# Azure/mmlspark

Measured on NVIDIA H100. Metric: boosting_iters_per_sec, higher is better.
Workload: dtype int64 fixed-point histograms over u8 bins (fp32 gradients, fp64 split gains)

## Files before the change

### mmlspark_b200/csrc/engine.cu

```cuda
#include "engine.h"
#include "objective.h"
#include "renew_kernel.cuh"
#include "metric_kernels.cuh"

#include <nvtx3/nvToolsExt.h>

#include <arpa/inet.h>
#include <netdb.h>
#include <netinet/in.h>
#include <netinet/tcp.h>
#include <sys/select.h>
#include <sys/socket.h>
#include <unistd.h>
#include <sys/types.h>

#include <algorithm>
#include <chrono>
#include <functional>
#include <mutex>
#include <omp.h>
#include <cstring>
#include <numeric>
#include <thread>

// ... 365 lines not shown
  UploadMeta();
  rows_stride = static_cast<size_t>(num_data);
  bins.Alloc(static_cast<size_t>(num_tiles) * rows_stride * 32);
  if (nw > 0) bins16.Alloc(static_cast<size_t>(nw) * rows_stride);
}

template <typename T>
static void LaunchBin(const T* X, long long nrow, int ncol, int row_major, long long ld, const Dataset& d, long long row_offset, cudaStream_t s) {
  B200_CUDA(cudaFuncSetAttribute(k_bin_rows<T>, cudaFuncAttributeMaxDynamicSharedMemorySize, 65536));
  const int sms = DeviceSMs();
  dim3 grid(static_cast<unsigned>(std::min<long long>((nrow + 7) / 8, sms * 8)), d.num_tiles);
  if (grid.x == 0) grid.x = 1;
  k_bin_rows<T><<<grid, 256, 65536, s>>>(X, nrow, ncol, row_major, ld, d.meta.p, d.ub.p, d.catbin.p, d.nfn, d.bins.p, static_cast<long long>(d.rows_stride), row_offset);
  if (d.nw > 0)
    k_bin_wide<T><<<sms * 8, 256, 0, s>>>(X, nrow, row_major, ld, d.wide_meta.p, d.nw, d.wide_cats.p, d.wide_catbin.p, d.wide_ub.p, d.bins16.p, d.rows_stride, row_offset);
  B200_CUDA(cudaGetLastError());
}

void Dataset::BinBlock(const void* data, bool on_device, int data_type, int is_row_major, long long n, long long start_row) {
  NvtxRange nvtx("b200gbm:K0 bin rows (H2D + value->bin)");
  const int F = num_total_features;
  const size_t esz = data_type == 0 ? 4 : 8;
  if (start_row < 0 || start_row + n > num_data) Fatal("row block out of range");
  if (on_device) {
    const long long ld = is_row_major ? F : n;
    if (data_type == 0) LaunchBin<float>(static_cast<const float*>(data), n, F, is_row_major, ld, *this, start_row, stream);
    else LaunchBin<double>(static_cast<const double*>(data), n, F, is_row_major, ld, *this, start_row, stream);
    B200_CUDA(cudaStreamSynchronize(stream));
    return;
  }
  const size_t kStageBytes = 256u << 20;
  long long chunk = std::max<long long>(1, std::min<long long>(n, static_cast<long long>(kStageBytes) / (static_cast<long long>(F) * esz)));
  const size_t need = static_cast<size_t>(chunk) * F * esz;
  if (!ingest_copy_stream_) {
    B200_CUDA(cudaStreamCreateWithFlags(&ingest_copy_stream_, cudaStreamNonBlocking));
    for (int i = 0; i < 2; ++i) {
      B200_CUDA(cudaEventCreateWithFlags(&ingest_copied_[i], cudaEventDisableTiming));
      B200_CUDA(cudaEventCreateWithFlags(&ingest_binned_[i], cudaEventDisableTiming));
    }
  }
  for (int i = 0; i < 2; ++i) if (ingest_buf_[i].n < need) ingest_buf_[i].Alloc(std::max(need, std::min(kStageBytes, static_cast<size_t>(num_data) * F * esz)));
  cudaStream_t copy_stream = ingest_copy_stream_;
  int it = 0;
  for (long long r0 = 0; r0 < n; r0 += chunk, ++it) {
    const int b = it & 1;
    const long long rows = std::min(chunk, n - r0);
    if (it >= 2) B200_CUDA(cudaStreamWaitEvent(copy_stream, ingest_binned_[b], 0));
    if (is_row_major) {
      B200_CUDA(cudaMemcpyAsync(ingest_buf_[b].p, static_cast<const unsigned char*>(data) + static_cast<size_t>(r0) * F * esz, static_cast<size_t>(rows) * F * esz,
                                cudaMemcpyHostToDevice, copy_stream));
    } else {
      B200_CUDA(cudaMemcpy2DAsync(ingest_buf_[b].p, static_cast<size_t>(rows) * esz, static_cast<const unsigned char*>(data) + static_cast<size_t>(r0) * esz,
                                  static_cast<size_t>(n) * esz, static_cast<size_t>(rows) * esz, F, cudaMemcpyHostToDevice, copy_stream));
    }
    B200_CUDA(cudaEventRecord(ingest_copied_[b], copy_stream));
    B200_CUDA(cudaStreamWaitEvent(stream, ingest_copied_[b], 0));
    const long long ld = is_row_major ? F : rows;
    if (data_type == 0) LaunchBin<float>(reinterpret_cast<const float*>(ingest_buf_[b].p), rows, F, is_row_major, ld, *this, start_row + r0, stream);
    else LaunchBin<double>(reinterpret_cast<const double*>(ingest_buf_[b].p), rows, F, is_row_major, ld, *this, start_row + r0, stream);
    B200_CUDA(cudaEventRecord(ingest_binned_[b], stream));
  }
  B200_CUDA(cudaStreamSynchronize(stream));
  ingest_rows_done_ += n;
  if (ingest_rows_done_ >= num_data) ReleaseIngestStaging();
}

void Dataset::ReleaseIngestStaging() {
  for (int i = 0; i < 2; ++i) {
    ingest_buf_[i].Free();
    if (ingest_copied_[i]) { cudaEventDestroy(ingest_copied_[i]); ingest_copied_[i] = nullptr; }
    if (ingest_binned_[i]) { cudaEventDestroy(ingest_binned_[i]); ingest_binned_[i] = nullptr; }
  }
  if (ingest_copy_stream_) { cudaStreamDestroy(ingest_copy_stream_); ingest_copy_stream_ = nullptr; }
}

Dataset* Dataset::CreateFromSampledColumn(double** sample_data, int** sample_indices, int ncol, const int* num_per_col, int num_sample_row,
                                          int num_total_row, const char* params) {
  (void)sample_indices;
  EnsureDevice();
  if (num_total_row <= 0 || ncol <= 0) Fatal("Dataset should have at least one row and one column");
  std::unique_ptr<Dataset> d = NewShell(num_total_row, ncol, params);
  d->SetMappers(nullptr, [&](std::vector<std::vector<double>>* nz, int, int) {
    for (int f = 0; f < ncol; ++f) (*nz)[f].assign(sample_data[f], sample_data[f] + num_per_col[f]);
    return num_sample_row;
  });
  d->AllocBins();
  return d.release();
}

void Dataset::PushRows(const void* data, int data_type, int nrow, int ncol, int start_row) {
  EnsureDevice();
  if (ncol != num_total_features) Fatal("PushRows: wrong number of columns");
  if (data_type != 0 && data_type != 1) Fatal("PushRows: unknown data type");
  StreamTimer timer(stream);
  BinBlock(data, IsDevicePointer(data), data_type, 1, nrow, start_row);
  ingest_ms += timer.Ms();
}

template <typename T>
void Dataset::UnpackTiles(T* out) const {
  std::vector<uint8_t> h(bins.n);
  B200_CUDA(cudaMemcpy(h.data(), bins.p, bins.n, cudaMemcpyDeviceToHost));
  std::memset(out, 0, static_cast<size_t>(num_data) * num_total_features * sizeof(T));
  for (int u = 0; u < nfn; ++u) {
    const int f = used[u];
    const uint8_t* src = h.data() + (static_cast<size_t>(u >> 5) * rows_stride) * 32 + (u & 31);
    for (int i = 0; i < num_data; ++i) out[static_cast<size_t>(i) * num_total_features + f] = src[static_cast<size_t>(i) * 32];
  }
}
void Dataset::GetBinsRowMajor(uint8_t* out) const {
  if (nw > 0) Fatal("this dataset has features with more than 256 bins: use B200GBM_DatasetGetBins16");
  UnpackTiles(out);
}
void Dataset::GetBinsRowMajor16(uint16_t* out) const {
  UnpackTiles(out);
  if (nw > 0) {
    std::vector<uint16_t> hw(bins16.n);
    B200_CUDA(cudaMemcpy(hw.data(), bins16.p, bins16.n * sizeof(uint16_t), cudaMemcpyDeviceToHost));
    for (int w = 0; w < nw; ++w) {
      const int f = used[nfn + w];
      const uint16_t* src = hw.data() + static_cast<size_t>(w) * rows_stride;
      for (int i = 0; i < num_data; ++i) out[static_cast<size_t>(i) * num_total_features + f] = src[i];
    }
  }
}

__global__ void k_gather_bin_rows(BinView bv, int nf, const FeatMeta* __restrict__ meta, const int* __restrict__ rows, int nrows, int F,
                                  uint16_t* __restrict__ out) {
  for (long long e = blockIdx.x * static_cast<long long>(blockDim.x) + threadIdx.x; e < static_cast<long long>(nrows) * nf;
       e += static_cast<long long>(gridDim.x) * blockDim.x) {
    const int i = static_cast<int>(e / nf), u = static_cast<int>(e % nf);
    out[static_cast<size_t>(i) * F + meta[u].real_index] = static_cast<uint16_t>(bv.at(u, static_cast<size_t>(rows[i])));
  }
}
void Dataset::GetBinsOfRows(const int32_t* rows, int nrows, uint16_t* out) const {
  if (nrows <= 0) return;
  for (int i = 0; i < nrows; ++i) if (rows[i] < 0 || rows[i] >= num_data) Fatal("GetBinsOfRows: row index out of range");
  DevBuf<int> dr; dr.Alloc(nrows);
  DevBuf<uint16_t> dout; dout.Alloc(static_cast<size_t>(nrows) * num_total_features);
  dr.Upload(rows, nrows, stream);
  dout.Zero(stream);
  if (nf > 0) k_gather_bin_rows<<<DeviceSMs() * 4, 256, 0, stream>>>(View(), nf, meta.p, dr.p, nrows, num_total_features, dout.p);
  B200_CUDA(cudaGetLastError());
  dout.Download(out, dout.n, stream);
  B200_CUDA(cudaStreamSynchronize(stream));
}

void Dataset::Histogram(const float* grad, const float* hess, const int32_t* idx, int cnt, double* out) const {
  EnsureDevice();
  B200_CUDA(set_k4_smem_limit());
  const int n = num_data;
  DevBuf<float> g, h; g.Alloc(n); h.Alloc(n);
  g.Upload(grad, n, stream); h.Upload(hess, n, stream);
  DevBuf<int4> q; q.Alloc(n);
  DevBuf<TreeCtrl> ctrl; ctrl.Alloc(1); ctrl.Zero(stream);
  DevBuf<int> didx; didx.Alloc(std::max(cnt, 1));
  if (idx) didx.Upload(idx, cnt, stream);
  const size_t elems = static_cast<size_t>(num_tiles) * 32 * 512;
  DevBuf<long long> H; H.Alloc(elems); H.Zero(stream);
  DevBuf<double> D; D.Alloc(elems);
  int sms = 0;
  B200_CUDA(cudaDeviceGetAttribute(&sms, cudaDevAttrMultiProcessorCount, device));
  k_absmax<<<sms * 4, 256, 0, stream>>>(g.p, h.p, n, ctrl.p);
  k_set_scale<<<1, 1, 0, stream>>>(ctrl.p, 0, 1.0);
  k_quantize<<<sms * 4, 256, 0, stream>>>(g.p, h.p, n, q.p, ctrl.p, 0, nullptr, 0);
  HistWork w{0, cnt, idx ? 1 : 0, 0};
  B200_CUDA(cudaMemcpyAsync(&ctrl.p->hist_work, &w, sizeof(w), cudaMemcpyHostToDevice, stream));
  DevBuf<int4> qo; qo.Alloc(std::max(cnt, 1));
  k_gather_q<<<sms * 4, 256, 0, stream>>>(&ctrl.p->hist_work, didx.p, didx.p, q.p, qo.p);
  launch_k4(false, bins.p, rows_stride, num_tiles, q.p, qo.p, didx.p, didx.p, &ctrl.p->hist_work,
            reinterpret_cast<unsigned long long*>(H.p), sms, stream);
  k_hist_to_double<<<sms * 4, 256, 0, stream>>>(H.p, D.p, elems, ctrl.p);
  B200_CUDA(cudaGetLastError());
  std::vector<double> hd(elems);
  D.Download(hd.data(), elems, stream);
  B200_CUDA(cudaStreamSynchronize(stream));
  std::memset(out, 0, sizeof(double) * static_cast<size_t>(num_total_features) * 512);
  for (int u = 0; u < nfn; ++u) std::memcpy(out + static_cast<size_t>(used[u]) * 512, hd.data() + static_cast<size_t>(u) * 512, sizeof(double) * 512);
}

Dataset* Dataset::CreateFromMat(const void* data, int data_type, int nrow, int ncol, int is_row_major, const char* params,
                                const Dataset* reference) {
  EnsureDevice();
  if (data_type != 0 && data_type != 1) Fatal("Unknown data type in CreateFromMat (expect C_API_DTYPE_FLOAT32 or FLOAT64)");
  if (nrow <= 0 || ncol <= 0) Fatal("Dataset should have at least one row and one column");
  std::unique_ptr<Dataset> d = NewShell(nrow, ncol, params);
  StreamTimer timer(d->stream);
  const bool on_device = IsDevicePointer(data);
  d->SetMappers(reference, [&](std::vector<std::vector<double>>* nz, int f0, int f1) {
    const int n = nrow, F = ncol;
    const std::vector<int> rows = d->SampleRows();
    const int sample_cnt = static_cast<int>(rows.size());
    std::vector<double> S(static_cast<size_t>(sample_cnt) * F);
    if (on_device) {
      DevBuf<int> d_rows; d_rows.Alloc(sample_cnt);
      DevBuf<double> d_S; d_S.Alloc(S.size());
      d_rows.Upload(rows.data(), sample_cnt, d->stream);
      int grid = static_cast<int>(std::min<size_t>((S.size() + 255) / 256, static_cast<size_t>(DeviceSMs()) * 32));
      if (data_type == 0) k_gather_rows<float><<<grid, 256, 0, d->stream>>>(static_cast<const float*>(data), n, F, is_row_major, d_rows.p, sample_cnt, d_S.p);
      else k_gather_rows<double><<<grid, 256, 0, d->stream>>>(static_cast<const double*>(data), n, F, is_row_major, d_rows.p, sample_cnt, d_S.p);
      B200_CUDA(cudaGetLastError());
      d_S.Download(S.data(), S.size(), d->stream);
      B200_CUDA(cudaStreamSynchronize(d->stream));
    } else {
#pragma omp parallel for schedule(static)
      for (int s = 0; s < sample_cnt; ++s) {
        const long long r = rows[s];
        for (int f = 0; f < F; ++f) {
          double v;
          if (data_type == 0) v = is_row_major ? static_cast<const float*>(data)[r * F + f] : static_cast<const float*>(data)[static_cast<long long>(f) * n + r];
          else v = is_row_major ? static_cast<const double*>(data)[r * F + f] : static_cast<const double*>(data)[static_cast<long long>(f) * n + r];
          S[static_cast<size_t>(s) * F + f] = v;
        }
      }
    }
#pragma omp parallel for schedule(dynamic)
    for (int f = f0; f < f1; ++f) {
      (*nz)[f].reserve(sample_cnt);
      for (int s = 0; s < sample_cnt; ++s) {
        double v = S[static_cast<size_t>(s) * F + f];
        if (std::fabs(v) > kZeroThr || std::isnan(v)) (*nz)[f].push_back(v);
      }
    }
    return sample_cnt;
  });
  d->AllocBins();
  d->BinBlock(data, on_device, data_type, is_row_major, nrow, 0);
  d->ingest_ms = timer.Ms();
  return d.release();
}

__global__ void k_fill_default_wide(const WideMeta* __restrict__ wm, int nw, uint16_t* __restrict__ bins16, size_t rows_stride, long long nrow) {
  for (long long e = blockIdx.x * static_cast<long long>(blockDim.x) + threadIdx.x; e < nrow * nw; e += static_cast<long long>(gridDim.x) * blockDim.x) {
    const int w = static_cast<int>(e / nrow);
    bins16[static_cast<size_t>(w) * rows_stride + (e - static_cast<long long>(w) * nrow)] = static_cast<uint16_t>(wm[w].default_bin);
  }
}
__global__ void k_fill_default_bins(const FeatMeta* __restrict__ meta, int nf, uint8_t* __restrict__ bins, size_t rows_stride, long long nrow, int num_tiles) {
  const long long total = nrow * num_tiles * 32;
  for (long long e = blockIdx.x * static_cast<long long>(blockDim.x) + threadIdx.x; e < total; e += static_cast<long long>(gridDim.x) * blockDim.x) {
    const int lane = static_cast<int>(e & 31);
    const long long rt = e >> 5;
    const int tile = static_cast<int>(rt / nrow);
    const long long r = rt - static_cast<long long>(tile) * nrow;
    const int u = tile * 32 + lane;
    bins[(static_cast<size_t>(tile) * rows_stride + r) * 32 + lane] = u < nf ? static_cast<uint8_t>(meta[u].default_bin) : 0;
  }
}
template <typename TI, typename TV>
__global__ void k_bin_csr(const TI* __restrict__ indptr, const int* __restrict__ indices, const TV* __restrict__ vals, long long nrow, const int* __restrict__ inner_of,
                          const FeatMeta* __restrict__ meta, const double* __restrict__ ub, const uint8_t* __restrict__ catbin, uint8_t* __restrict__ bins,
                          size_t rows_stride, long long elem_base, int nfn, const WideMeta* __restrict__ wm, const int* __restrict__ wcats,
                          const unsigned short* __restrict__ wcatbin, const double* __restrict__ wub, uint16_t* __restrict__ bins16) {
  const int lane = threadIdx.x & 31;
  const long long warp = (blockIdx.x * static_cast<long long>(blockDim.x) + threadIdx.x) >> 5, nwarps = (static_cast<long long>(gridDim.x) * blockDim.x) >> 5;
  for (long long r = warp; r < nrow; r += nwarps) {
    const long long a = static_cast<long long>(indptr[r]) - elem_base, b = static_cast<long long>(indptr[r + 1]) - elem_base;
    for (long long k = a + lane; k < b; k += 32) {
      const int u = inner_of[indices[k]];
      if (u < 0) continue;
      const FeatMeta m = meta[u];
      double v = static_cast<double>(vals[k]);
      if (u >= nfn) {
        bins16[static_cast<size_t>(u - nfn) * rows_stride + r] = static_cast<uint16_t>(d_wide_bin(v, wm[u - nfn], wcats, wcatbin, wub));
        continue;
      }
      const double* myub = ub + static_cast<size_t>(u) * 256;
      unsigned bin = 0;
      if (m.is_categorical) {
        if (!isnan(v)) {
          const int iv = static_cast<int>(v);
          if (iv >= 0) {
            int lo = 0, hi = m.num_sorted_cats;
            while (lo < hi) { int mid = (lo + hi) >> 1; if (static_cast<int>(myub[mid]) < iv) lo = mid + 1; else hi = mid; }
            if (lo < m.num_sorted_cats && static_cast<int>(myub[lo]) == iv) bin = catbin[static_cast<size_t>(u) * 256 + lo];
          }
        }
      } else {
        if (isnan(v)) { if (m.missing_type == 2) bin = m.num_bin - 1; else v = 0.0; }
        if (!isnan(v)) {
          int lo = 0, hi = m.num_bin - 1 - (m.missing_type == 2 ? 1 : 0);
          while (lo < hi) { int mid = (hi + lo - 1) / 2; if (v <= myub[mid]) hi = mid; else lo = mid + 1; }
          bin = lo;
        }
      }
      bins[(static_cast<size_t>(u >> 5) * rows_stride + r) * 32 + (u & 31)] = static_cast<uint8_t>(bin);
    }
  }
}

Dataset* Dataset::CreateFromCSR(const void* indptr, int indptr_type, const int32_t* indices, const void* data, int data_type,
                                int64_t nindptr, int64_t nelem, int64_t num_col, const char* params, const Dataset* reference) {
  EnsureDevice();
  if (num_col <= 0) Fatal("CreateFromCSR: num_col must be given");
  if (num_col > std::numeric_limits<int>::max()) Fatal("CreateFromCSR: too many columns");
  if (indptr_type != 2 && indptr_type != 3) Fatal("CreateFromCSR: indptr must be int32 or int64");
  if (data_type != 0 && data_type != 1) Fatal("Unknown data type in CreateFromCSR (expect C_API_DTYPE_FLOAT32 or FLOAT64)");
  const int64_t nrow = nindptr - 1;
  if (nrow <= 0) Fatal("Dataset should have at least one row and one column");
  if (nrow > std::numeric_limits<int>::max()) Fatal("CreateFromCSR: too many rows for one partition");
  auto ip = [&](int64_t r) -> int64_t { return indptr_type == 2 ? static_cast<const int32_t*>(indptr)[r] : static_cast<const int64_t*>(indptr)[r]; };
  auto val = [&](int64_t k) -> double { return data_type == 0 ? static_cast<double>(static_cast<const float*>(data)[k]) : static_cast<const double*>(data)[k]; };
  if (ip(0) < 0 || ip(nrow) > nelem) Fatal("CreateFromCSR: indptr does not match the number of elements");
  {
    int bad = 0;
#pragma omp parallel for schedule(static) reduction(| : bad)
    for (int64_t r = 0; r < nrow; ++r) {
      if (ip(r) > ip(r + 1)) bad |= 1;
      else for (int64_t k = ip(r); k < ip(r + 1); ++k) if (indices[k] < 0 || indices[k] >= num_col) bad |= 2;
    }
    if (bad & 1) Fatal("CreateFromCSR: indptr is not non-decreasing");
    if (bad & 2) Fatal("CreateFromCSR: a column index is negative or >= num_col");
  }
  std::unique_ptr<Dataset> d = NewShell(static_cast<int>(nrow), static_cast<int>(num_col), params);
  StreamTimer timer(d->stream);
  const int F = d->num_total_features;
  d->SetMappers(reference, [&](std::vector<std::vector<double>>* nz, int, int) {
    const std::vector<int> rows = d->SampleRows();
    for (int r : rows)
      for (int64_t k = ip(r); k < ip(r + 1); ++k) {
        const double v = val(k);
        if (std::fabs(v) > kZeroThr || std::isnan(v)) (*nz)[indices[k]].push_back(v);
      }
// ... 63 lines not shown
  } else if (s == "weight" || s == "weights") {
    if (n == 0 || data == nullptr) { weight.clear(); d_weight.Free(); return; }
    if (n != num_data) Fatal("Length of weights is not same with #data");
    to_f32(&weight);
    d_weight.Alloc(n); d_weight.Upload(weight.data(), n, stream);
  } else if (s == "init_score") {
    if (n == 0 || data == nullptr) { init_score.clear(); return; }
    if (n % num_data != 0) Fatal("Initial score size doesn't match data size");
    init_score.resize(n);
    if (type == 1) std::memcpy(init_score.data(), data, sizeof(double) * n);
    else if (type == 0) for (int i = 0; i < n; ++i) init_score[i] = static_cast<const float*>(data)[i];
    else Fatal("Input type error for init_score (expect float64)");
  } else if (s == "group" || s == "query") {
    if (type != 2) Fatal("Input type error for group (expect int32)");
    const int32_t* g = static_cast<const int32_t*>(data);
    group_sizes.assign(g, g + n);
    query_boundaries.assign(1, 0);
    for (int i = 0; i < n; ++i) query_boundaries.push_back(query_boundaries.back() + g[i]);
    if (query_boundaries.back() != num_data) Fatal("Sum of query counts is not same with #data");
    d_qb.Alloc(query_boundaries.size()); d_qb.Upload(query_boundaries.data(), query_boundaries.size(), stream);
  } else {
    Fatal("Unknown field name: " + s);
  }
  B200_CUDA(cudaStreamSynchronize(stream));
}

void Dataset::GetField(const char* name, int* out_len, const void** out_ptr, int* out_type) const {
  std::string s(name);
  if (s == "label" || s == "target") { *out_len = static_cast<int>(label.size()); *out_ptr = label.data(); *out_type = 0; }
  else if (s == "weight" || s == "weights") { *out_len = static_cast<int>(weight.size()); *out_ptr = weight.empty() ? nullptr : weight.data(); *out_type = 0; }
  else if (s == "init_score") { *out_len = static_cast<int>(init_score.size()); *out_ptr = init_score.empty() ? nullptr : init_score.data(); *out_type = 1; }
  else if (s == "group" || s == "query") { *out_len = static_cast<int>(query_boundaries.size()); *out_ptr = query_boundaries.empty() ? nullptr : query_boundaries.data(); *out_type = 2; }
  else Fatal("Unknown field name: " + s);
}

void Dataset::SetFeatureNames(const char** names, int n) {
  if (n != num_total_features) Fatal("Size of feature_names error, should equal with total number of features");
  feature_names.assign(n, "");
  for (int i = 0; i < n; ++i) {
    feature_names[i] = names[i];
    for (auto& c : feature_names[i]) if (c == ' ') c = '_';
  }
}

static size_t Align16(size_t x) { return (x + 15) & ~static_cast<size_t>(15); }
constexpr int kScanSmem = (768 + 64) * 8;

Booster::Booster(const std::string& model_text) {
  std::unique_ptr<HostModel> m = HostModel::FromString(model_text);
  model = std::move(*m);
  K = model.num_tree_per_iteration;
  num_init_iteration = model.NumIterations();
}

Booster::Booster(const Dataset* tr, const char* params) : train(tr) {
  EnsureDevice();
  device_ = CurrentDevice();
  cfg.Parse(params);
  if (cfg.boosting != "gbdt" && cfg.boosting != "rf" && cfg.boosting != "goss" && cfg.boosting != "dart")
    Fatal("Unknown boosting type " + cfg.boosting);
  is_rf_ = cfg.boosting == "rf"; is_goss_ = cfg.boosting == "goss"; is_dart_ = cfg.boosting == "dart";
  drop_rand_ = LcgRandom(cfg.drop_seed);
  obj_.reset(new Objective(cfg, *train));
  balanced_bagging_ = cfg.bagging_freq > 0 && (cfg.pos_bagging_fraction < 1.0 || cfg.neg_bagging_fraction < 1.0) && obj_->kind() == ObjectiveKind::kBinary;
  bagging_ = cfg.bagging_freq > 0 && (cfg.bagging_fraction < 1.0 || balanced_bagging_);
  if (bagging_ && !(cfg.bagging_fraction > 0.0)) Fatal("bagging_fraction should be in (0, 1]");
  if (is_goss_) {
    if (!(cfg.top_rate + cfg.other_rate <= 1.0)) Fatal("Check failed: (config_->top_rate + config_->other_rate) <= (1.0f)");
    if (!(cfg.top_rate > 0.0 && cfg.other_rate > 0.0)) Fatal("Check failed: config_->top_rate > 0.0f && config_->other_rate > 0.0f");
    if (bagging_) Fatal("Cannot use bagging in GOSS");
  }
  if (is_rf_) {
    const bool ff = cfg.feature_fraction < 1.0 && cfg.feature_fraction > 0.0;
    if (!(bagging_ || ff)) Fatal("Check failed: (config->bagging_freq > 0 && config->bagging_fraction < 1.0f && config->bagging_fraction > 0.0f) || (config->feature_fraction < 1.0f && config->feature_fraction > 0.0f)");
  }
  if (cfg.num_leaves < 2) Fatal("num_leaves should be >= 2");
  ValidateMetrics();
  if (train->label.empty()) Fatal("label should not be empty for training");
  K = obj_->NumTreePerIteration();
  parallel_ = Net().active && Net().world > 1;
  cfg.num_machines = parallel_ ? Net().world : 1;
  if (balanced_bagging_) {
    double npos = static_cast<double>(std::count_if(train->label.begin(), train->label.end(), [](float v) { return v > 0; }));
    if (parallel_) {
      cudaStream_t ts;
      B200_CUDA(cudaStreamCreateWithFlags(&ts, cudaStreamNonBlocking));
      AllReduceHost(&npos, 1, ncclSum, ts);
      B200_CUDA(cudaStreamDestroy(ts));
    }
    if (!(npos > 0)) { balanced_bagging_ = false; bagging_ = cfg.bagging_freq > 0 && cfg.bagging_fraction < 1.0; }
  }
  shrinkage_ = is_rf_ ? 1.0 : cfg.learning_rate;
  model.average_output = is_rf_;
  model.num_class = K;
  model.num_tree_per_iteration = K;
  model.label_index = 0;
  model.max_feature_idx = train->num_total_features - 1;
  model.feature_names = train->feature_names;
  for (int f = 0; f < train->num_total_features; ++f) model.feature_infos.push_back(train->mappers[f].InfoString());
  InitTraining();
  model.objective_str = obj_->ToString();
}

Booster::~Booster() {
  if (split_op_trees_ > 0) {
    double tot = 0; for (auto& kv : split_op_ms_) tot += kv.second;
    fprintf(stderr, "[b200gbm split timing] %d trees, %.3f ms per tree in split operations:", split_op_trees_, tot / split_op_trees_);
    for (auto& kv : split_op_ms_) fprintf(stderr, " %s=%.1fus", kv.first.c_str(), 1000.0 * kv.second / split_op_trees_ / std::max(cfg.num_leaves - 1, 1));
    fprintf(stderr, " (per split)\n");
  }
  for (auto* v : valids_) delete v;
  for (void* p : ipc_opened_) cudaIpcCloseMemHandle(p);
  if (tree_host_) cudaFreeHost(tree_host_);
  if (ctrl_host_) cudaFreeHost(ctrl_host_);
  if (leaves_host_) cudaFreeHost(leaves_host_);
  if (ev_a_) cudaEventDestroy(ev_a_);
  if (ev_b_) cudaEventDestroy(ev_b_);
  if (stream_) cudaStreamDestroy(stream_);
}

void Booster::InitTraining() {
  const int n = train->num_data;
  const int L = cfg.num_leaves;
  cudaDeviceProp prop;
  B200_CUDA(cudaGetDeviceProperties(&prop, device_));
  num_sms_ = prop.multiProcessorCount;
  B200_CUDA(cudaStreamCreateWithFlags(&stream_, cudaStreamNonBlocking));
  B200_CUDA(cudaEventCreate(&ev_a_)); B200_CUDA(cudaEventCreate(&ev_b_));
  cudaDeviceSetLimit(cudaLimitMaxL2FetchGranularity, 32);
  cudaGetLastError();
  B200_CUDA(set_k4_smem_limit());
  B200_CUDA(cudaFuncSetAttribute(k_scan, cudaFuncAttributeMaxDynamicSharedMemorySize, kScanSmem));

  sp_.l1 = cfg.lambda_l1; sp_.l2 = cfg.lambda_l2; sp_.max_delta_step = cfg.max_delta_step;
  sp_.min_gain_to_split = cfg.min_gain_to_split; sp_.min_sum_hessian = cfg.min_sum_hessian_in_leaf;
  sp_.min_data_in_leaf = cfg.min_data_in_leaf; sp_.max_depth = cfg.max_depth; sp_.num_leaves = L; sp_.parallel = parallel_ ? 1 : 0;
  sp_.nf = train->nf; sp_.nf_pad = train->nf_pad; sp_.num_tiles = train->num_tiles; sp_.nfn = train->nfn;
  {
    auto gd = [&](const char* k, double d) { auto it = cfg.raw.find(k); return (it != cfg.raw.end() && !it->second.empty()) ? std::atof(it->second.c_str()) : d; };
    sp_.cat_l2 = gd("cat_l2", 10.0); sp_.cat_smooth = gd("cat_smooth", 10.0);
    sp_.max_cat_threshold = static_cast<int>(gd("max_cat_threshold", 32)); sp_.max_cat_to_onehot = static_cast<int>(gd("max_cat_to_onehot", 4));
    sp_.min_data_per_group = static_cast<int>(gd("min_data_per_group", 100)); sp_.pad3 = 0;
    if (train->nw > 0) {
      if (sp_.max_cat_threshold > kCatListMax) Fatal("max_cat_threshold > " + std::to_string(kCatListMax) + " is not supported together with categorical features of more than 256 bins");
      if (sp_.max_cat_to_onehot > 256) Fatal("max_cat_to_onehot > 256 is not supported together with categorical features of more than 256 bins");
      B200_CUDA(cudaFuncSetAttribute(k4_hist_wide<4>, cudaFuncAttributeMaxDynamicSharedMemorySize, 4 * kWideHistSeg * 4));
      B200_CUDA(cudaFuncSetAttribute(k4_hist_wide<3>, cudaFuncAttributeMaxDynamicSharedMemorySize, 4 * kWideHistSeg * 4));
      B200_CUDA(cudaFuncSetAttribute(k_scan_wide, cudaFuncAttributeMaxDynamicSharedMemorySize, kWideMaxBins * 8));
    }
  }

  score_.Alloc(static_cast<size_t>(K) * n); score_.Zero(stream_);
  grad_.Alloc(static_cast<size_t>(K) * n); hess_.Alloc(static_cast<size_t>(K) * n);
  qgh_.Alloc(n); qord_.Alloc(n); idx0_.Alloc(n); idx1_.Alloc(n);
  slot_elems_ = train->hist_pairs * 2;
  H_.Alloc(slot_elems_); H_.Zero(stream_); pool_.Alloc(slot_elems_ * L);
  {
    int per_sm = 0;
    B200_CUDA(cudaOccupancyMaxActiveBlocksPerMultiprocessor(&per_sm, k_partition, 256, 0));
    int coop = 0;
    cudaDeviceGetAttribute(&coop, cudaDevAttrCooperativeLaunch, device_);
    if (!coop || per_sm < 1) Fatal("this device cannot launch the cooperative partition kernel");
    part_max_blocks_ = per_sm * num_sms_;
  }
  flags_.Alloc(static_cast<size_t>(L) * train->nf_pad);
  cands_.Alloc(2 * static_cast<size_t>(train->nf_pad));
  leaves_.Alloc(L); ctrl_.Alloc(1); ctrl_.Zero(stream_);
  const int chunks = n / kPartChunk + 2;
  part_bits_.Alloc(static_cast<size_t>(chunks) * (kPartChunk / 32)); part_chunks_.Alloc(static_cast<size_t>(chunks) + chunks / kPartLocalScan + 8); part_chunks_.Zero(stream_);
  {
    size_t off = 0;
    auto take = [&](size_t bytes) { size_t o = off; off += Align16(bytes); return o; };
    size_t o_lc = take(4 * (L - 1)), o_rc = take(4 * (L - 1)), o_sf = take(4 * (L - 1)), o_tb = take(4 * (L - 1)), o_dt = take(4 * (L - 1));
    size_t o_sg = take(4 * (L - 1)), o_lv = take(8 * L), o_lw = take(8 * L), o_lcn = take(4 * L), o_iv = take(8 * (L - 1)), o_iw = take(8 * (L - 1));
    size_t o_ic = take(4 * (L - 1)), o_lp = take(4 * L), o_ld = take(4 * L), o_nl = take(16), o_cb = take(32 * (L - 1));
    size_t o_cl = take(2 * kCatListMax * (L - 1)), o_cn = take(4 * (L - 1));
    tree_blob_bytes_ = off;
    tree_blob_.Alloc(off);
    unsigned char* b = tree_blob_.p;
    tree_dev_.left_child = reinterpret_cast<int*>(b + o_lc); tree_dev_.right_child = reinterpret_cast<int*>(b + o_rc);
    tree_dev_.split_feature_inner = reinterpret_cast<int*>(b + o_sf); tree_dev_.threshold_bin = reinterpret_cast<int*>(b + o_tb);
    tree_dev_.decision_type = reinterpret_cast<int*>(b + o_dt); tree_dev_.split_gain = reinterpret_cast<float*>(b + o_sg);
    tree_dev_.leaf_value = reinterpret_cast<double*>(b + o_lv); tree_dev_.leaf_weight = reinterpret_cast<double*>(b + o_lw);
    tree_dev_.leaf_count = reinterpret_cast<int*>(b + o_lcn); tree_dev_.internal_value = reinterpret_cast<double*>(b + o_iv);
    tree_dev_.internal_weight = reinterpret_cast<double*>(b + o_iw); tree_dev_.internal_count = reinterpret_cast<int*>(b + o_ic);
    tree_dev_.leaf_parent = reinterpret_cast<int*>(b + o_lp); tree_dev_.leaf_depth = reinterpret_cast<int*>(b + o_ld);
    tree_dev_.num_leaves = reinterpret_cast<int*>(b + o_nl);
    tree_dev_.cat_bits = reinterpret_cast<unsigned*>(b + o_cb);
    tree_dev_.cat_list = reinterpret_cast<unsigned short*>(b + o_cl);
    tree_dev_.cat_list_len = reinterpret_cast<int*>(b + o_cn);
    B200_CUDA(cudaMemsetAsync(b, 0, off, stream_));
    B200_CUDA(cudaMallocHost(reinterpret_cast<void**>(&tree_host_), off));
    B200_CUDA(cudaMallocHost(reinterpret_cast<void**>(&ctrl_host_), sizeof(TreeCtrl)));
    B200_CUDA(cudaMallocHost(reinterpret_cast<void**>(&leaves_host_), sizeof(LeafState) * L));
  }
  if (!train->init_score.empty()) {
    if (train->init_score.size() != static_cast<size_t>(K) * n) Fatal("Initial score size doesn't match data size");
    has_init_score_ = true;
    score_.Upload(train->init_score.data(), train->init_score.size(), stream_);
  }
  obj_->Init(stream_);
  const_hessian_ = obj_->ConstHessian() && !is_goss_;
  if (obj_->RenewsLeaves()) {
    rn_keys_a_.Alloc(n); rn_keys_b_.Alloc(n); rn_pos_a_.Alloc(n); rn_pos_b_.Alloc(n); rn_leaf_of_pos_.Alloc(n); rn_leaf_a_.Alloc(n); rn_leaf_b_.Alloc(n);
    rn_res_.Alloc(n); rn_row_.Alloc(n); rn_seg_.Alloc(L + 1); rn_out_.Alloc(2 * static_cast<size_t>(L));
    if (obj_->RenewWeights()) rn_cdf_.Alloc(n);
    size_t t1 = 0, t2 = 0;
    cub::DeviceRadixSort::SortPairs(nullptr, t1, rn_keys_a_.p, rn_keys_b_.p, rn_pos_a_.p, rn_pos_b_.p, n, 0, 64, stream_);
    cub::DeviceRadixSort::SortPairs(nullptr, t2, rn_leaf_a_.p, rn_leaf_b_.p, rn_pos_b_.p, rn_pos_a_.p, n, 0, 32, stream_);
    rn_tmp_bytes_ = std::max(t1, t2);
    rn_tmp_.Alloc(rn_tmp_bytes_ + 16);
  }
  if (parallel_) SetupPeerReduce();
  col_rand_ = LcgRandom(cfg.feature_fraction_seed);
  feature_used_host_.assign(train->nf_pad, 0);
  for (int u = 0; u < train->nf; ++u) feature_used_host_[u] = 1;
  feature_used_.Alloc(train->nf_pad);
  feature_used_.Upload(feature_used_host_.data(), train->nf_pad, stream_);
  ResetFeaturesByTree();
  if (bagging_ || is_goss_) {
    bag_blocks_ = (n + kBagBlock - 1) / kBagBlock;
    std::vector<unsigned> st(bag_blocks_);
    for (int i = 0; i < bag_blocks_; ++i) st[i] = static_cast<unsigned>(cfg.bagging_seed + i);
    bag_lcg_.Alloc(bag_blocks_); bag_lcg_.Upload(st.data(), st.size(), stream_);
    std::unique_ptr<LcgJump> jt(new LcgJump());
    unsigned a = 1, c = 0;
    for (int j = 0; j < kBagBlock; ++j) { a = a * 214013u; c = c * 214013u + 2531011u; jt->mul[j] = a; jt->add[j] = c; }
    bag_jump_.Alloc(1); bag_jump_.Upload(jt.get(), 1, stream_);
    in_bag_.Alloc(n); bag_block_cnt_.Alloc(bag_blocks_); bag_idx_.Alloc(n); bag_total_.Alloc(1);
    need_re_bagging_ = bagging_;
    B200_CUDA(cudaStreamSynchronize(stream_));
  }
  if (is_rf_) {
    if (!train->init_score.empty()) Fatal("Check failed: train_data->metadata().init_score() == nullptr");
    rf_init_scores_.assign(K, 0.0);
    DevBuf<double> tmp;
    tmp.Alloc(static_cast<size_t>(K) * n); tmp.Zero(stream_);
    for (int k = 0; k < K; ++k) {
      double init = (cfg.boost_from_average && !has_init_score_) ? obj_->BoostFromScore(k) : 0.0;
      if (!(std::fabs(init) > kEps)) init = 0.0;
      rf_init_scores_[k] = init;
      if (init != 0.0) k_add_const<<<num_sms_ * 4, 256, 0, stream_>>>(tmp.p + static_cast<size_t>(k) * n, n, init);
    }
    ComputeGradientsAt(tmp.p);
    B200_CUDA(cudaStreamSynchronize(stream_));
  }
  B200_CUDA(cudaStreamSynchronize(stream_));
}

TreeDev Booster::RebasedTree(unsigned char* base) const {
  TreeDev t = tree_dev_;
  auto mv = [&](auto*& p) { p = reinterpret_cast<std::remove_reference_t<decltype(p)>>(base + (reinterpret_cast<unsigned char*>(p) - tree_blob_.p)); };
  mv(t.left_child); mv(t.right_child); mv(t.split_feature_inner); mv(t.threshold_bin); mv(t.decision_type); mv(t.split_gain);
  mv(t.leaf_value); mv(t.leaf_weight); mv(t.leaf_count); mv(t.internal_value); mv(t.internal_weight); mv(t.internal_count);
  mv(t.leaf_parent); mv(t.leaf_depth); mv(t.num_leaves); mv(t.cat_bits); mv(t.cat_list); mv(t.cat_list_len);
  return t;
}
void Booster::AddStoredTree(int iter_index, int k, bool to_train, bool to_valid) {
  const size_t ti = static_cast<size_t>(num_init_iteration + iter_index) * K + k;
  const HostTree& ht = *model.trees[ti];
  cudaStream_t s = stream_;
  const int n = train->num_data;
  if (ht.num_leaves <= 1) {
    const double v = ht.leaf_value[0];
    if (v != 0.0) {
      if (to_train) k_add_const<<<num_sms_ * 4, 256, 0, s>>>(score_.p + static_cast<size_t>(k) * n, n, v);
      if (to_valid) for (auto* vs : valids_) k_add_const<<<num_sms_ * 4, 256, 0, s>>>(vs->score.p + static_cast<size_t>(k) * vs->ds->num_data, vs->ds->num_data, v);
    }
    return;
  }
  DevBuf<unsigned char>& blob = *tree_store_.at(static_cast<size_t>(iter_index) * K + k);
  TreeDev td = RebasedTree(blob.p);
  B200_CUDA(cudaMemcpyAsync(td.leaf_value, ht.leaf_value.data(), sizeof(double) * ht.num_leaves, cudaMemcpyHostToDevice, s));
  const int egrid = num_sms_ * 8;
  if (to_train) k_add_tree_binned<<<egrid, 256, 0, s>>>(td, train->meta.p, train->View(), n, score_.p + static_cast<size_t>(k) * n, 1.0);
  if (to_valid)
    for (auto* vs : valids_)
      k_add_tree_binned<<<egrid, 256, 0, s>>>(td, vs->ds->meta.p, vs->ds->View(), vs->ds->num_data,
                                              vs->score.p + static_cast<size_t>(k) * vs->ds->num_data, 1.0);
  B200_CUDA(cudaGetLastError());
  B200_CUDA(cudaStreamSynchronize(s));
  timing.launches += (to_train ? 1 : 0) + (to_valid ? static_cast<long long>(valids_.size()) : 0);
}
void Booster::DroppingTrees() {
  drop_index_.clear();
  const bool is_skip = drop_rand_.NextFloat() < cfg.skip_drop;
  if (!is_skip) {
    double drop_rate = cfg.drop_rate;
    if (!cfg.uniform_drop) {
      const double inv_average_weight = static_cast<double>(tree_weight_.size()) / sum_weight_;
      if (cfg.max_drop > 0) drop_rate = std::min(drop_rate, cfg.max_drop * inv_average_weight / sum_weight_);
      for (int i = 0; i < iter; ++i)
        if (drop_rand_.NextFloat() < drop_rate * tree_weight_[i] * inv_average_weight) {
          drop_index_.push_back(i);
          if (drop_index_.size() >= static_cast<size_t>(cfg.max_drop)) break;
        }
    } else {
      if (cfg.max_drop > 0) drop_rate = std::min(drop_rate, cfg.max_drop / static_cast<double>(iter));
      for (int i = 0; i < iter; ++i)
        if (drop_rand_.NextFloat() < drop_rate) {
          drop_index_.push_back(i);
          if (drop_index_.size() >= static_cast<size_t>(cfg.max_drop)) break;
        }
    }
  }
  for (int i : drop_index_)
    for (int k = 0; k < K; ++k) {
// ... 77 lines not shown
  {
    DevBuf<unsigned char> ds, dr; ds.Alloc(sizeof(PeerInfo)); dr.Alloc(sizeof(PeerInfo) * R);
    B200_CUDA(cudaMemcpyAsync(ds.p, &mine, sizeof(PeerInfo), cudaMemcpyHostToDevice, stream_));
    B200_NCCL(ncclAllGather(ds.p, dr.p, sizeof(PeerInfo), ncclChar, Net().comm, stream_));
    B200_CUDA(cudaMemcpyAsync(all.data(), dr.p, sizeof(PeerInfo) * R, cudaMemcpyDeviceToHost, stream_));
    B200_CUDA(cudaStreamSynchronize(stream_));
  }
  int ok = 1;
  for (int r = 0; r < R; ++r) ok &= all[r].ok;
  PeerTables pt{};
  if (ok) {
    for (int r = 0; r < R && ok; ++r) {
      void* p3[3];
      if (r == me) { for (int i = 0; i < 3; ++i) p3[i] = bufs[i]; }
      else if (all[r].pid == mine.pid) {
        int can = 0;
        cudaDeviceCanAccessPeer(&can, device_, all[r].device);
        if (!can) { ok = 0; break; }
        cudaError_t e = cudaDeviceEnablePeerAccess(all[r].device, 0);
        if (e != cudaSuccess && e != cudaErrorPeerAccessAlreadyEnabled) { cudaGetLastError(); ok = 0; break; }
        cudaGetLastError();
        for (int i = 0; i < 3; ++i) p3[i] = reinterpret_cast<void*>(all[r].ptr[i]);
      } else {
        for (int i = 0; i < 3; ++i) {
          if (cudaIpcOpenMemHandle(&p3[i], all[r].ipc[i], cudaIpcMemLazyEnablePeerAccess) != cudaSuccess) { cudaGetLastError(); ok = 0; break; }
          ipc_opened_.push_back(p3[i]);
        }
        if (!ok) break;
      }
      pt.H[r] = static_cast<const long long*>(p3[0]); pt.mail[r] = static_cast<SplitCand*>(p3[1]); pt.flags[r] = static_cast<unsigned*>(p3[2]);
    }
  }
  double okd = ok ? 1.0 : 0.0;
  AllReduceHost(&okd, 1, ncclMin, stream_);
  const bool peers_ok = okd > 0.5;
  fused_ = peers_ok && mode == 1;
  p2p_allreduce_ = peers_ok && mode == 2;
  if (p2p_allreduce_) { pt.rank = me; pt.world = R; pt.feat0 = 0; pt.feat1 = 0; pt.error = peer_error_.p; peers_ = pt; return; }
  if (!fused_) return;
  const int tiles_per_rank = (train->num_tiles + R - 1) / R;
  pt.rank = me; pt.world = R;
  pt.feat0 = std::min(train->nf_pad, me * tiles_per_rank * 32);
  pt.feat1 = std::min(train->nf_pad, (me + 1) * tiles_per_rank * 32);
  pt.error = peer_error_.p;
  peers_ = pt;
}

void Booster::ResetFeaturesByTree() {
  if (cfg.feature_fraction >= 1.0) return;
  const int total = train->nf;
  int cnt = std::max(static_cast<int>(total * cfg.feature_fraction + 0.5), std::min(2, total));
  std::fill(feature_used_host_.begin(), feature_used_host_.end(), 0);
  for (int i : col_rand_.Sample(total, cnt)) feature_used_host_[train->sample_order[i]] = 1;
  feature_used_.Upload(feature_used_host_.data(), train->nf_pad, stream_);
}

double Booster::BoostFromAverage(int k) {
  if (model.trees.empty() && !has_init_score_ && cfg.boost_from_average) {
    double init = obj_->BoostFromScore(k);
    if (std::fabs(init) > kEps) {
      const int n = train->num_data;
      k_add_const<<<num_sms_ * 4, 256, 0, stream_>>>(score_.p + static_cast<size_t>(k) * n, n, init);
      for (auto* v : valids_) k_add_const<<<num_sms_ * 4, 256, 0, stream_>>>(v->score.p + static_cast<size_t>(k) * v->ds->num_data, v->ds->num_data, init);
      B200_CUDA(cudaGetLastError());
      return init;
    }
  }
  return 0.0;
}

void Booster::ComputeGradientsAt(const double* score_p) {
  NvtxRange nvtx("b200gbm:K1/K2 gradients");
  obj_->LaunchGradients(score_p, grad_.p, hess_.p, num_sms_);
  B200_CUDA(cudaGetLastError());
  timing.launches += 1;
}

void Booster::RenewTreeOutput(int k, double rf_pred) {
  const int n = train->num_data;
  const int total = use_bag_ ? bag_count_ : n;
  const int L = cfg.num_leaves;
  cudaStream_t s = stream_;
  TreeCtrl* ctrl = ctrl_.p;
  const int egrid = num_sms_ * 8;
  const float* wptr = obj_->RenewWeights();
  k_renew_gather<<<egrid, 256, 0, s>>>(ctrl, leaves_.p, idx0_.p, idx1_.p, train->d_label.p, is_rf_ ? nullptr : score_.p + static_cast<size_t>(k) * n, rf_pred,
                                       rn_keys_a_.p, rn_pos_a_.p, rn_res_.p, rn_leaf_of_pos_.p, rn_row_.p);
  size_t tb = rn_tmp_bytes_;
  B200_CUDA(cub::DeviceRadixSort::SortPairs(rn_tmp_.p, tb, rn_keys_a_.p, rn_keys_b_.p, rn_pos_a_.p, rn_pos_b_.p, total, 0, 64, s));
  k_renew_leaf_keys<<<egrid, 256, 0, s>>>(rn_pos_b_.p, rn_leaf_of_pos_.p, total, rn_leaf_a_.p);
  int leaf_bits = 1;
  while ((1 << leaf_bits) < L) ++leaf_bits;
  tb = rn_tmp_bytes_;
  B200_CUDA(cub::DeviceRadixSort::SortPairs(rn_tmp_.p, tb, rn_leaf_a_.p, rn_leaf_b_.p, rn_pos_b_.p, rn_pos_a_.p, total, 0, leaf_bits, s));
  k_renew_offsets<<<1, 32, 0, s>>>(ctrl, leaves_.p, rn_seg_.p);
  double* out = rn_out_.p;
  double* has = rn_out_.p + L;
  const int lgrid = (L + 127) / 128;
  if (!wptr) {
    k_renew_unweighted<<<lgrid, 128, 0, s>>>(ctrl, rn_seg_.p, rn_pos_a_.p, rn_res_.p, obj_->RenewAlpha(), out, has);
  } else {
    k_renew_cdf<<<L, 1024, 0, s>>>(ctrl, rn_seg_.p, rn_pos_a_.p, rn_row_.p, wptr, rn_cdf_.p);
    k_renew_weighted<<<lgrid, 128, 0, s>>>(ctrl, rn_seg_.p, rn_pos_a_.p, rn_res_.p, rn_cdf_.p, obj_->RenewAlpha(), out, has);
  }
  if (parallel_) B200_NCCL(ncclAllReduce(out, out, 2 * static_cast<size_t>(L), ncclDouble, ncclSum, Net().comm, s));
  k_renew_apply<<<lgrid, 128, 0, s>>>(ctrl, tree_dev_, out, has, parallel_ ? 1 : 0);
  B200_CUDA(cudaGetLastError());
  timing.launches += wptr ? 7 : 6;
}

void Booster::EnsureColumnCopy() {
  if (cols_tried_) return;
  cols_tried_ = true;
  const Dataset& d = *train;
  const char* env = std::getenv("B200GBM_COLUMN_COPY");
  if ((env && std::atoi(env) == 0) || d.nfn == 0 || d.num_data == 0) return;
  const size_t stride = (static_cast<size_t>(d.num_data) + 255) & ~static_cast<size_t>(255);
  const size_t need = static_cast<size_t>(d.num_tiles) * 32 * stride;
  size_t free_b = 0, total_b = 0;
  if (cudaMemGetInfo(&free_b, &total_b) != cudaSuccess) { cudaGetLastError(); return; }
  const size_t reserve = std::max<size_t>(static_cast<size_t>(8) << 30, total_b / 10);
  if (free_b < need + reserve) return;
  uint8_t* p = nullptr;
  if (cudaMalloc(reinterpret_cast<void**>(&p), need) != cudaSuccess) { cudaGetLastError(); return; }
  bins_cols_.p = p; bins_cols_.n = need;
  cols_stride_ = stride;
  const long long work = ((static_cast<long long>(d.num_data) + 255) / 256) * d.num_tiles;
  k_tiles_to_columns<<<static_cast<unsigned>(std::min<long long>(work, static_cast<long long>(num_sms_) * 16)), 256, 0, stream_>>>(
      d.bins.p, d.rows_stride, d.num_tiles, d.num_data, bins_cols_.p, stride);
  B200_CUDA(cudaGetLastError());
}

void Booster::GetMemoryInfo(int64_t* out2) {
  EnsureDevice();
  size_t free_b = 0, total_b = 0;
  if (cudaMemGetInfo(&free_b, &total_b) != cudaSuccess) { cudaGetLastError(); free_b = 0; }
  out2[0] = static_cast<int64_t>(bins_cols_.n);
  out2[1] = static_cast<int64_t>(free_b);
}

void Booster::LaunchPartition(int grid, int last) {
  const Dataset& d = *train;
  TreeCtrl* ctrl = ctrl_.p;
  LeafState* leaves = leaves_.p;
  TreeDev tree = tree_dev_;
  uint8_t* flags = flags_.p;
  const FeatMeta* meta = d.meta.p;
  SplitParams sp = sp_;
  const uint8_t* bins = d.bins.p;
  size_t rows_stride = d.rows_stride;
  int* i0 = idx0_.p; int* i1 = idx1_.p;
  unsigned* bits = part_bits_.p;
  int* chunks = part_chunks_.p;
  const int4* qgh = qgh_.p;
  int4* qord = qord_.p;
  long long* H = H_.p;
  size_t h_elems = slot_elems_;
  const uint16_t* bins16 = d.bins16.p;
  static const int tickets = [] { const char* e = std::getenv("B200GBM_PART_TICKETS"); return e ? std::atoi(e) : 8; }();
  int tickets_per_block = tickets;
  const uint8_t* cols = bins_cols_.p;
  size_t cols_stride = cols_stride_;
  int* super_tot = part_chunks_.p + (train->num_data / kPartChunk + 2);
  void* args[] = {&ctrl, &leaves, &tree, &flags, &meta, &sp, &last, &bins, &rows_stride, &i0, &i1, &bits, &chunks, &qgh, &qord, &H, &h_elems, &bins16, &tickets_per_block,
                  &cols, &cols_stride, &super_tot};
  B200_CUDA(cudaLaunchCooperativeKernel(reinterpret_cast<void*>(k_partition), dim3(grid), dim3(256), args, 0, stream_));
}

void Booster::TrainOneTree(int k, HostTree* out) {
  NvtxRange nvtx_tree("b200gbm:tree");
  EnsureColumnCopy();
  const Dataset& d = *train;
  const int n = d.num_data;
  const int L = cfg.num_leaves;
  const float* g = grad_.p + static_cast<size_t>(k) * n;
  const float* h = hess_.p + static_cast<size_t>(k) * n;
  TreeCtrl* ctrl = ctrl_.p;
  cudaStream_t s = stream_;
  const int egrid = num_sms_ * 8;
  nvtxRangePushA("b200gbm:K3 quantize + C1 root sums");
  B200_CUDA(cudaMemsetAsync(&ctrl->absmax_bits[0], 0, 8, s));
  k_absmax<<<egrid, 256, 0, s>>>(g, h, n, ctrl);
  if (parallel_) B200_NCCL(ncclAllReduce(&ctrl->absmax_bits[0], &ctrl->absmax_bits[0], 2, ncclUint32, ncclMax, Net().comm, s));
  k_set_scale<<<1, 1, 0, s>>>(ctrl, const_hessian_ ? 1 : 0, 1.0);
  k_quantize<<<egrid, 256, 0, s>>>(g, h, n, qgh_.p, ctrl, const_hessian_ ? 1 : 0, use_bag_ ? in_bag_.p : nullptr, bag_count_);
  if (parallel_) B200_NCCL(ncclAllReduce(&ctrl->root_q[0], &ctrl->root_q[0], 3, ncclInt64, ncclSum, Net().comm, s));
  ResetFeaturesByTree();
  if (use_bag_)
    B200_CUDA(cudaMemcpyAsync(idx0_.p, bag_idx_.p, static_cast<size_t>(bag_count_) * sizeof(int), cudaMemcpyDeviceToDevice, s));
  k_tree_init<<<1, 256, 0, s>>>(ctrl, leaves_.p, tree_dev_, flags_.p, sp_, use_bag_ ? bag_count_ : n, feature_used_.p, use_bag_ ? 1 : 0);
  nvtxRangePop();
  timing.launches += 4;
  const int pgrid = std::max(1, std::min(n / kPartChunk + 1, part_max_blocks_));
  const dim3 sgrid(std::max(1, d.nfn), 2);
  std::vector<cudaEvent_t> evs;
  static const bool split_timing = getenv("B200GBM_SPLIT_TIMING") != nullptr;
  std::vector<cudaEvent_t> sev;
  auto mark = [&]() { if (split_timing) { cudaEvent_t e; cudaEventCreate(&e); cudaEventRecord(e, s); sev.push_back(e); } };
  k_round_ctl<<<1, 256, 0, s>>>(ctrl, leaves_.p, tree_dev_, flags_.p, d.meta.p, sp_, 0);
  timing.launches += 1;
  for (int split = 0; split < L - 1; ++split) {
    mark();
    if (profile_hist) { cudaEvent_t a, b; B200_CUDA(cudaEventCreate(&a)); B200_CUDA(cudaEventCreate(&b)); evs.push_back(a); evs.push_back(b); B200_CUDA(cudaEventRecord(a, s)); }
    if (split == 0 && use_bag_) k_gather_q<<<egrid, 256, 0, s>>>(&ctrl->hist_work, idx0_.p, idx1_.p, qgh_.p, qord_.p);
    mark();
    nvtxRangePushA("b200gbm:K4 histogram");
    launch_k4(const_hessian_, d.bins.p, d.rows_stride, d.num_tiles, qgh_.p, qord_.p, idx0_.p, idx1_.p, &ctrl->hist_work,
              reinterpret_cast<unsigned long long*>(H_.p), num_sms_, s);
    if (d.nw > 0) {
      int max_nb = 0;
      for (const WideMeta& wm : d.wide_host) max_nb = std::max(max_nb, wm.num_bin);
      const int segs = (max_nb + kWideHistSeg - 1) / kWideHistSeg;
      int units = 0;
      for (const WideMeta& wm : d.wide_host) units += (wm.num_bin + kWideHistSeg - 1) / kWideHistSeg;
      const dim3 wgrid(static_cast<unsigned>(std::max(1, std::min(64, 4 * num_sms_ / std::max(1, units)))), static_cast<unsigned>(d.nw), static_cast<unsigned>(segs));
      if (const_hessian_)
        k4_hist_wide<3><<<wgrid, kWideThreads, 4 * kWideHistSeg * 4, s>>>(d.bins16.p, d.rows_stride, d.wide_meta.p, qgh_.p, qord_.p, idx0_.p, idx1_.p, &ctrl->hist_work,
                                                                         reinterpret_cast<unsigned long long*>(H_.p));
      else
        k4_hist_wide<4><<<wgrid, kWideThreads, 4 * kWideHistSeg * 4, s>>>(d.bins16.p, d.rows_stride, d.wide_meta.p, qgh_.p, qord_.p, idx0_.p, idx1_.p, &ctrl->hist_work,
                                                                         reinterpret_cast<unsigned long long*>(H_.p));
      timing.launches += 1;
    }
    nvtxRangePop();
    if (profile_hist) B200_CUDA(cudaEventRecord(evs.back(), s));
    mark();
    nvtxRangePushA(parallel_ ? "b200gbm:C2 histogram reduce + K5 scan + pick" : "b200gbm:K5 scan + pick");
    if (fused_) {
      ++epoch_;
      const dim3 dgrid(std::max(1, (peers_.feat1 - peers_.feat0 + 7) / 8), 2);
      k_scan_dp<<<dgrid, 256, 0, s>>>(ctrl, leaves_.p, d.meta.p, peers_, pool_.p, slot_elems_, flags_.p, cands_.p, sp_, epoch_);
      k_pick_dp<<<1, 256, 0, s>>>(ctrl, leaves_.p, d.meta.p, cands_.p, sp_, peers_, epoch_);
      mark();
    } else {
      if (p2p_allreduce_) {
        ++epoch_;
        const int agrid = static_cast<int>(std::max<size_t>(1, std::min<size_t>(64, slot_elems_ / 2 / Net().world / 256 + 1)));
        k_allreduce_p2p<<<agrid, 256, 0, s>>>(ctrl, peers_, slot_elems_, epoch_, peer_flags_.p + 48);
        timing.launches += 1;
      } else if (parallel_) {
        B200_NCCL(ncclAllReduce(H_.p, H_.p, slot_elems_, ncclInt64, ncclSum, Net().comm, s));
      }
      mark();
      if (d.nw > 0) {
        k_scan_wide<<<dim3(d.nw, 2), 256, kWideMaxBins * 8, s>>>(ctrl, leaves_.p, d.wide_meta.p, H_.p, pool_.p, slot_elems_, flags_.p, cands_.p, sp_);
        timing.launches += 1;
      }
      k_scan<<<sgrid, 256, d.has_categorical ? kScanSmem : 0, s>>>(ctrl, leaves_.p, d.meta.p, H_.p, pool_.p, slot_elems_, flags_.p, cands_.p, sp_);
    }
    nvtxRangePop();
    mark();
    nvtxRangePushA("b200gbm:K7 partition + controller");
    LaunchPartition(pgrid, split == L - 2 ? 1 : 0);
    nvtxRangePop();
    mark();
    timing.launches += fused_ ? 4 : 3; timing.hist_launches += 1;
  }
  if (obj_->RenewsLeaves()) RenewTreeOutput(k, is_rf_ ? rf_init_scores_[k] : 0.0);
  const double bias = is_rf_ ? rf_init_scores_[k] : 0.0, pre = is_rf_ ? static_cast<double>(iter + num_init_iteration) : 1.0;
  const double post = is_rf_ ? 1.0 / (iter + num_init_iteration + 1) : 1.0;
  if (use_bag_ || is_rf_)
    k_add_tree_binned<<<egrid, 256, 0, s>>>(tree_dev_, d.meta.p, d.View(), n, score_.p + static_cast<size_t>(k) * n, shrinkage_, bias, pre, post);
  else
    k_add_score<<<egrid, 256, 0, s>>>(ctrl, leaves_.p, tree_dev_, idx0_.p, idx1_.p, score_.p + static_cast<size_t>(k) * n, shrinkage_);
  for (auto* v : valids_)
    k_add_tree_binned<<<egrid, 256, 0, s>>>(tree_dev_, v->ds->meta.p, v->ds->View(), v->ds->num_data,
                                            v->score.p + static_cast<size_t>(k) * v->ds->num_data, shrinkage_, bias, pre, post);
  timing.launches += 2 + static_cast<long long>(valids_.size());
  B200_CUDA(cudaGetLastError());
  B200_CUDA(cudaMemcpyAsync(tree_host_, tree_blob_.p, tree_blob_bytes_, cudaMemcpyDeviceToHost, s));
  B200_CUDA(cudaMemcpyAsync(ctrl_host_, ctrl, sizeof(TreeCtrl), cudaMemcpyDeviceToHost, s));
  B200_CUDA(cudaStreamSynchronize(s));
  if (split_timing && !fused_ && !sev.empty()) {
    static const char* kOps[] = {"gather_q(bagged root)", "K4", "allreduce", "scan+pick", "partition+zeroH+ctl"};
    const int per = 6;
    for (size_t b0 = 0; b0 + per <= sev.size(); b0 += per)
      for (int o = 0; o < per - 1; ++o) { float ms = 0; cudaEventElapsedTime(&ms, sev[b0 + o], sev[b0 + o + 1]); split_op_ms_[kOps[o]] += ms; }
    split_op_trees_ += 1;
    for (auto e : sev) cudaEventDestroy(e);
  }
  if (profile_hist) {
    for (size_t i = 0; i + 1 < evs.size(); i += 2) { float ms = 0; cudaEventElapsedTime(&ms, evs[i], evs[i + 1]); timing.hist_ms += ms; }
    for (auto e : evs) cudaEventDestroy(e);
  }
  timing.hist_rows += ctrl_host_->trace_rows;
  if (fused_ || p2p_allreduce_) {
    int err = 0;
    B200_CUDA(cudaMemcpy(&err, peer_error_.p, sizeof(int), cudaMemcpyDeviceToHost));
    if (err) Fatal("data-parallel training: a peer rank stopped responding (peer-memory barrier timed out)");
  }
  const unsigned char* hb = tree_host_;
  auto at = [&](const void* devp) { return hb + (static_cast<const unsigned char*>(devp) - tree_blob_.p); };
  const int nl = *reinterpret_cast<const int*>(at(tree_dev_.num_leaves));
  out->Resize(nl);
  if (nl > 1) {
    const int* lc = reinterpret_cast<const int*>(at(tree_dev_.left_child));
    const int* rc = reinterpret_cast<const int*>(at(tree_dev_.right_child));
    const int* sf = reinterpret_cast<const int*>(at(tree_dev_.split_feature_inner));
    const int* tb = reinterpret_cast<const int*>(at(tree_dev_.threshold_bin));
    const int* dt = reinterpret_cast<const int*>(at(tree_dev_.decision_type));
    const float* sg = reinterpret_cast<const float*>(at(tree_dev_.split_gain));
    const double* lv = reinterpret_cast<const double*>(at(tree_dev_.leaf_value));
    const double* lw = reinterpret_cast<const double*>(at(tree_dev_.leaf_weight));
    const int* lcn = reinterpret_cast<const int*>(at(tree_dev_.leaf_count));
    const double* iv = reinterpret_cast<const double*>(at(tree_dev_.internal_value));
    const double* iw = reinterpret_cast<const double*>(at(tree_dev_.internal_weight));
    const int* ic = reinterpret_cast<const int*>(at(tree_dev_.internal_count));
    const int* ld = reinterpret_cast<const int*>(at(tree_dev_.leaf_depth));
    const unsigned* cb = reinterpret_cast<const unsigned*>(at(tree_dev_.cat_bits));
    const unsigned short* cl = reinterpret_cast<const unsigned short*>(at(tree_dev_.cat_list));
    const int* cln = reinterpret_cast<const int*>(at(tree_dev_.cat_list_len));
    for (int i = 0; i < nl - 1; ++i) {
      out->left_child[i] = lc[i]; out->right_child[i] = rc[i]; out->split_feature_inner[i] = sf[i];
      out->split_feature[i] = d.used[sf[i]]; out->threshold_in_bin[i] = static_cast<uint32_t>(tb[i]);
      out->decision_type[i] = static_cast<int8_t>(dt[i]); out->split_gain[i] = sg[i];
      const FeatureBins& fbm = d.mappers[d.used[sf[i]]];
      if (dt[i] & 1) {
        std::vector<int> cats;
        if (sf[i] >= d.nfn) { for (int k = 0; k < cln[i]; ++k) cats.push_back(fbm.bin_to_cat[cl[i * kCatListMax + k]]); }
        else for (int b = 0; b < fbm.num_bin; ++b) if ((cb[i * 8 + (b >> 5)] >> (b & 31)) & 1u) cats.push_back(fbm.bin_to_cat[b]);
        out->AddCategoricalNode(i, cats);
      } else {
        double thr = fbm.upper[tb[i]];
        if (std::isnan(thr)) thr = 0.0; else if (thr >= 1e300) thr = 1e300; else if (thr <= -1e300) thr = -1e300;
        out->threshold[i] = thr;
      }
      out->internal_value[i] = iv[i]; out->internal_weight[i] = iw[i]; out->internal_count[i] = ic[i];
    }
    for (int i = 0; i < nl; ++i) { out->leaf_value[i] = lv[i]; out->leaf_weight[i] = lw[i]; out->leaf_count[i] = lcn[i]; out->leaf_depth[i] = ld[i]; }
  } else {
    out->leaf_value[0] = 0.0;
  }
}

bool Booster::TrainTrees(const float* custom_g, const float* custom_h) {
  NvtxRange nvtx("b200gbm:iteration (LGBM_BoosterUpdateOneIter)");
  if (!train) Fatal("this booster was loaded from a model string and cannot be trained");
  EnsureDevice();
  cudaStream_t s = stream_;
  const int n = train->num_data;
  B200_CUDA(cudaEventRecord(ev_a_, s));
  std::vector<double> init_scores(K, 0.0);
  bool saved_const = const_hessian_;
  if (is_rf_) {
    if (custom_g) Fatal("RF mode do not support custom objective function, please use built-in objectives.");
    init_scores = rf_init_scores_;
  } else if (!custom_g) {
    for (int k = 0; k < K; ++k) init_scores[k] = BoostFromAverage(k);
    if (is_dart_ && !dart_dropped_this_iter_) DroppingTrees();
    ComputeGradientsAt(score_.p);
  } else {
    grad_.Upload(custom_g, static_cast<size_t>(K) * n, s);
    hess_.Upload(custom_h, static_cast<size_t>(K) * n, s);
    const_hessian_ = false;
  }
  Bagging(iter);
  bool should_continue = is_rf_;
  for (int k = 0; k < K; ++k) {
    std::unique_ptr<HostTree> t(new HostTree());
    t->Resize(1);
    t->leaf_value[0] = 0;
    if (obj_->NeedTrain(k) && train->nf > 0) TrainOneTree(k, t.get());
    if (t->num_leaves > 1) {
      should_continue = true;
      t->Shrink(shrinkage_);
      if (std::fabs(init_scores[k]) > kEps) t->AddBias(init_scores[k]);
    } else if (static_cast<int>(model.trees.size()) < K) {
      double output = obj_->NeedTrain(k) ? init_scores[k] : obj_->BoostFromScore(k);
      t->MakeConstant(output);
      const double pre = is_rf_ ? static_cast<double>(iter + num_init_iteration) : 1.0, post = is_rf_ ? 1.0 / (iter + num_init_iteration + 1) : 1.0;
      k_scale_add<<<num_sms_ * 4, 256, 0, s>>>(score_.p + static_cast<size_t>(k) * n, n, pre, output, post);
      for (auto* v : valids_) k_scale_add<<<num_sms_ * 4, 256, 0, s>>>(v->score.p + static_cast<size_t>(k) * v->ds->num_data, v->ds->num_data, pre, output, post);
    } else {
// ... 407 lines not shown
```

### mmlspark_b200/csrc/engine.h

```cpp
#pragma once
#include <cuda_runtime.h>
#include <nccl.h>

#include <cstdint>
#include <memory>
#include <stdexcept>
#include <map>
#include <string>
#include <vector>

#include "bin_mapper.h"
#include "config.h"
#include "kernels.cuh"
#include "model.h"

namespace b200gbm {

#define B200_CUDA(x)                                                                                      \
  do {                                                                                                    \
    cudaError_t e__ = (x);                                                                                \
    if (e__ != cudaSuccess)                                                                               \
      throw std::runtime_error(std::string("CUDA error: ") + cudaGetErrorString(e__) + " at " + __FILE__ + ":" + std::to_string(__LINE__)); \
  } while (0)
#define B200_NCCL(x)                                                                                      \
// ... 44 lines not shown
  static Dataset* CreateFromMat(const void* data, int data_type, int nrow, int ncol, int is_row_major, const char* params,
                                const Dataset* reference);
  static Dataset* CreateFromCSR(const void* indptr, int indptr_type, const int32_t* indices, const void* data, int data_type,
                                int64_t nindptr, int64_t nelem, int64_t num_col, const char* params, const Dataset* reference);
  static Dataset* CreateFromSampledColumn(double** sample_data, int** sample_indices, int ncol, const int* num_per_col,
                                          int num_sample_row, int num_total_row, const char* params);
  void PushRows(const void* data, int data_type, int nrow, int ncol, int start_row);
  void GetBinsRowMajor(uint8_t* out) const;
  void GetBinsRowMajor16(uint16_t* out) const;
  void GetBinsOfRows(const int32_t* rows, int nrows, uint16_t* out) const;
  void Histogram(const float* grad, const float* hess, const int32_t* idx, int cnt, double* out) const;
  void SetField(const char* name, const void* data, int n, int type);
  void GetField(const char* name, int* out_len, const void** out_ptr, int* out_type) const;
  void SetFeatureNames(const char** names, int n);

  int device = 0;
  int num_data = 0, num_total_features = 0;
  Config cfg;
  std::vector<FeatureBins> mappers;
  std::vector<int> used;
  std::vector<int> inner_of;
  std::vector<FeatMeta> meta_host;
  int nf = 0, nf_pad = 0, num_tiles = 0;
  int nfn = 0, nw = 0;
  size_t hist_pairs = 0;
  std::vector<int> sample_order;
  size_t rows_stride = 0;
  DevBuf<uint8_t> bins;
  DevBuf<uint16_t> bins16;
  std::vector<WideMeta> wide_host;
  DevBuf<WideMeta> wide_meta;
  DevBuf<int> wide_cats;
  DevBuf<unsigned short> wide_catbin;
  DevBuf<double> wide_ub;
  BinView View() const { return BinView{bins.p, rows_stride, bins16.p, nfn}; }
  DevBuf<FeatMeta> meta;
  DevBuf<double> ub;
  DevBuf<uint8_t> catbin;
  bool has_categorical = false;
  std::vector<float> label, weight;
  std::vector<double> init_score;
  std::vector<int32_t> query_boundaries, group_sizes;
  DevBuf<float> d_label, d_weight;
  DevBuf<int> d_qb;
  std::vector<std::string> feature_names;
  cudaStream_t stream = nullptr;
  double ingest_ms = 0.0;

 private:
  static std::unique_ptr<Dataset> NewShell(int nrow, int ncol, const char* params);
  template <typename Sample> void SetMappers(const Dataset* reference, Sample sample);
  std::vector<int> SampleRows() const;
  void AllocBins();
  template <typename T> void UnpackTiles(T* out) const;
  void BinBlock(const void* data, bool on_device, int data_type, int is_row_major, long long nrow, long long start_row);
  DevBuf<unsigned char> ingest_buf_[2];
  cudaStream_t ingest_copy_stream_ = nullptr;
  cudaEvent_t ingest_copied_[2] = {nullptr, nullptr}, ingest_binned_[2] = {nullptr, nullptr};
  long long ingest_rows_done_ = 0;
  void ReleaseIngestStaging();
  void UploadMeta();
};

struct ValidSet {
  const Dataset* ds = nullptr;
  DevBuf<double> score;
};
class Objective;

class Booster {
 public:
  Booster(const Dataset* train, const char* params);
  explicit Booster(const std::string& model_text);
  ~Booster();

  bool UpdateOneIter();
  bool UpdateOneIterCustom(const float* grad, const float* hess);
  void ResetParameter(const char* params);
  void AddValidData(const Dataset* valid);
  void MergeFrom(const Booster* other);
  std::vector<std::string> EvalNames() const;
  std::vector<double> GetEval(int data_idx);
  void ValidateMetrics() const;
  void GetPredict(int data_idx, int64_t* out_len, double* out);
  int64_t NumPredict(int data_idx) const;
  void GetRawScores(int data_idx, double* out);
  int64_t PredictBatch(const void* data, int data_type, int64_t nrow, int ncol, int predict_type, int start_iteration, int num_iteration, double* out);
  double last_predict_ms = 0.0;
  void GetInfo(int* out4) const { out4[0] = parallel_ ? Net().world : 1; out4[1] = parallel_ ? Net().rank : 0; out4[2] = fused_ ? 1 : (p2p_allreduce_ ? 2 : 0); out4[3] = const_hessian_ ? 1 : 0; }
  std::string SaveModelToString(int start_iteration, int num_iteration, int importance_type) const;
  std::string DumpModelJson(int start_iteration, int num_iteration) const;

  struct Timing { double hist_ms = 0, total_ms = 0; long long hist_rows = 0; long long hist_launches = 0, launches = 0; };
  Timing timing;
  std::map<std::string, double> split_op_ms_; int split_op_trees_ = 0;
  bool profile_hist = false;
  std::vector<double> trace;

  Config cfg;
  HostModel model;
  const Dataset* train = nullptr;
  int K = 1;
  int iter = 0;
  int num_init_iteration = 0;

 private:
  void InitTraining();
  bool TrainTrees(const float* custom_g, const float* custom_h);
  void TrainOneTree(int class_id, HostTree* out);
  void LaunchPartition(int grid, int last);
  int part_max_blocks_ = 0;
  double BoostFromAverage(int class_id);

  std::unique_ptr<Objective> obj_;
  int device_ = 0;
  cudaStream_t stream_ = nullptr;
  bool parallel_ = false;
  bool const_hessian_ = false;
  bool has_init_score_ = false;
  double shrinkage_ = 0.1;
  LcgRandom col_rand_{2};
  std::vector<uint8_t> feature_used_host_;
  DevBuf<uint8_t> feature_used_;
  void ResetFeaturesByTree();
  bool is_rf_ = false, is_goss_ = false, bagging_ = false, balanced_bagging_ = false, use_bag_ = false, need_re_bagging_ = false;
  int bag_count_ = 0, bag_blocks_ = 0;
  DevBuf<unsigned> bag_lcg_;
  DevBuf<LcgJump> bag_jump_;
  DevBuf<uint8_t> in_bag_;
  DevBuf<int> bag_block_cnt_, bag_idx_, bag_total_;
  std::vector<double> rf_init_scores_;
  void Bagging(int it);
  void ComputeGradientsAt(const double* score);
  DevBuf<unsigned long long> rn_keys_a_, rn_keys_b_;
  DevBuf<unsigned> rn_pos_a_, rn_pos_b_, rn_leaf_of_pos_, rn_leaf_a_, rn_leaf_b_;
  DevBuf<double> rn_res_, rn_cdf_, rn_out_;
  DevBuf<int> rn_row_, rn_seg_;
  DevBuf<unsigned char> rn_tmp_;
  size_t rn_tmp_bytes_ = 0;
  void RenewTreeOutput(int class_id, double rf_pred);
  bool is_dart_ = false, dart_dropped_this_iter_ = false;
  LcgRandom drop_rand_{4};
  std::vector<int> drop_index_;
  std::vector<double> tree_weight_;
  double sum_weight_ = 0.0;
  std::vector<std::unique_ptr<DevBuf<unsigned char>>> tree_store_;
  void DroppingTrees();
  void DartNormalize();
  void AddStoredTree(int iter_index, int class_id, bool to_train, bool to_valid);
  TreeDev RebasedTree(unsigned char* base) const;
  SplitParams sp_{};
  DevBuf<double> score_;
  DevBuf<float> grad_, hess_;
  DevBuf<int4> qgh_, qord_;
  DevBuf<int> idx0_, idx1_;
  DevBuf<long long> H_;
  DevBuf<long long> pool_;
  size_t slot_elems_ = 0;
  DevBuf<uint8_t> flags_;
  DevBuf<SplitCand> cands_;
  DevBuf<LeafState> leaves_;
  DevBuf<TreeCtrl> ctrl_;
  DevBuf<unsigned char> tree_blob_;
  TreeDev tree_dev_{};
  size_t tree_blob_bytes_ = 0;
  unsigned char* tree_host_ = nullptr;
  TreeCtrl* ctrl_host_ = nullptr;
  LeafState* leaves_host_ = nullptr;
  DevBuf<uint8_t> bins_cols_;
  size_t cols_stride_ = 0;
  bool cols_tried_ = false;
  void EnsureColumnCopy();
 public:
  void GetMemoryInfo(int64_t* out2);
 private:
  DevBuf<unsigned> part_bits_;
  DevBuf<int> part_chunks_;
  bool fused_ = false;
  bool p2p_allreduce_ = false;
  PeerTables peers_{};
  DevBuf<SplitCand> mailbox_;
  DevBuf<unsigned> peer_flags_;
  DevBuf<int> peer_error_;
  std::vector<void*> ipc_opened_;
  unsigned epoch_ = 0;
  void SetupPeerReduce();
  struct ForestBufs { DevBuf<int> tree_offset, leaf_offset, num_leaves, split_feature, decision_type, left_child, right_child, cat_begin, cat_len; DevBuf<double> threshold, leaf_value, node_count, leaf_count, expected; DevBuf<unsigned> cat_words; size_t trees = 0; int max_depth = 0; };
  std::unique_ptr<ForestBufs> forest_;
  void UploadForest();
  std::vector<ValidSet*> valids_;
  DevBuf<double> met_partial_, met_out_, auc_wpos_, auc_wneg_, auc_ppos_, auc_pneg_;
  DevBuf<unsigned long long> auc_keys_a_, auc_keys_b_;
  DevBuf<int> auc_rows_a_, auc_rows_b_, auc_head_, auc_start_;
  DevBuf<unsigned char> auc_tmp_;
  int num_sms_ = 0;
  cudaEvent_t ev_a_ = nullptr, ev_b_ = nullptr;
};

}
```

### mmlspark_b200/csrc/hist_kernel.cuh

```cuda
#pragma once
#include <cstdint>
#include <cuda_runtime.h>

namespace b200gbm {

constexpr int kTileFeat = 32;
constexpr int kBins = 256;
constexpr int kLoBits = 18;
constexpr int kFlushRows = 1 << (32 - kLoBits);
#ifndef B200GBM_K4_EXPERIMENT
#define B200GBM_K4_EXPERIMENT 0
#endif
constexpr int kPlaneWords = kBins * kTileFeat;

struct HistWork {
  int begin;
  int count;
  int use_idx;
  int buf;
};

__global__ void __launch_bounds__(256)
k_gather_q(const HistWork* __restrict__ work, const int* __restrict__ idx0, const int* __restrict__ idx1, const int4* __restrict__ qgh,
           int4* __restrict__ qord) {
  const HistWork w = *work;
  if (!w.use_idx) return;
  const int* __restrict__ idx = w.buf ? idx1 : idx0;
  for (int i = blockIdx.x * blockDim.x + threadIdx.x; i < w.count; i += gridDim.x * blockDim.x) {
    const int p = w.begin + i;
    qord[p] = qgh[idx[p]];
  }
}


__device__ __forceinline__ void cp_async16(void* smem, const void* gmem, bool valid) {
  unsigned s = static_cast<unsigned>(__cvta_generic_to_shared(smem));
  int sz = valid ? 16 : 0;
  asm volatile("cp.async.cg.shared.global [%0], [%1], 16, %2;\n" ::"r"(s), "l"(gmem), "r"(sz));
}
template <int N>
__device__ __forceinline__ void cp_async_wait() {
  asm volatile("cp.async.wait_group %0;\n" ::"n"(N));
}

constexpr int kWsConsumerWarps = 16;
constexpr int kWsProducerWarps = 2;
constexpr int kWsThreads = (kWsConsumerWarps + kWsProducerWarps) * 32;
constexpr int kWsStageRows = 512;
constexpr int kWsStages = 3;
constexpr int kFlushSlabBins = 32;
constexpr int kFlushRowBytes = kFlushSlabBins * 16;
constexpr int kFlushStageBytes = kTileFeat * kFlushRowBytes;
constexpr int kWsSmemBytes = 4 * kPlaneWords * 4 + kWsStages * (kWsStageRows * 32 + kWsStageRows * 16) + kFlushStageBytes + 64;
static_assert(kWsSmemBytes <= 227 * 1024, "K4 shared memory exceeds the 227 KB per block of sm_90");
static_assert(kFlushSlabBins * kTileFeat == 2 * kWsConsumerWarps * 32, "a flush slab is two (g,h) pairs per consumer thread");

__device__ __forceinline__ unsigned smem_u32(const void* p) { return static_cast<unsigned>(__cvta_generic_to_shared(p)); }
__device__ __forceinline__ void mbar_init(unsigned long long* bar, unsigned count) {
  asm volatile("mbarrier.init.shared::cta.b64 [%0], %1;\n" ::"r"(smem_u32(bar)), "r"(count));
}
__device__ __forceinline__ void mbar_arrive(unsigned long long* bar) {
  asm volatile("mbarrier.arrive.shared::cta.b64 _, [%0];\n" ::"r"(smem_u32(bar)) : "memory");
}
__device__ __forceinline__ void mbar_arrive_expect_tx(unsigned long long* bar, unsigned bytes) {
  asm volatile("mbarrier.arrive.expect_tx.shared::cta.b64 _, [%0], %1;\n" ::"r"(smem_u32(bar)), "r"(bytes) : "memory");
}
__device__ __forceinline__ void mbar_expect_tx(unsigned long long* bar, unsigned bytes) {
  asm volatile("mbarrier.expect_tx.relaxed.cta.shared::cta.b64 [%0], %1;\n" ::"r"(smem_u32(bar)), "r"(bytes) : "memory");
}
__device__ __forceinline__ void mbar_wait(unsigned long long* bar, unsigned parity) {
  asm volatile(
      "{\n"
      ".reg .pred p;\n"
      "WAIT_LOOP:\n"
      "mbarrier.try_wait.parity.shared::cta.b64 p, [%0], %1;\n"
      "@p bra DONE;\n"
      "bra WAIT_LOOP;\n"
      "DONE:\n"
      "}\n" ::"r"(smem_u32(bar)), "r"(parity) : "memory");
}
__device__ __forceinline__ void tma_bulk_g2s(void* smem_dst, const void* gmem_src, unsigned bytes, unsigned long long* bar) {
  asm volatile("cp.async.bulk.shared::cluster.global.mbarrier::complete_tx::bytes [%0], [%1], %2, [%3];\n" ::"r"(smem_u32(smem_dst)),
               "l"(gmem_src), "r"(bytes), "r"(smem_u32(bar))
               : "memory");
}
__device__ __forceinline__ void cp_async_mbar_arrive_noinc(unsigned long long* bar) {
  asm volatile("cp.async.mbarrier.arrive.noinc.shared::cta.b64 [%0];\n" ::"r"(smem_u32(bar)) : "memory");
}
__device__ __forceinline__ void bulk_reduce_add_u64(unsigned long long* gmem_dst, const void* smem_src, unsigned bytes) {
  asm volatile("cp.reduce.async.bulk.global.shared::cta.bulk_group.add.u64 [%0], [%1], %2;\n" ::"l"(gmem_dst), "r"(smem_u32(smem_src)),
               "r"(bytes)
               : "memory");
}
__device__ __forceinline__ void bulk_commit() { asm volatile("cp.async.bulk.commit_group;\n" ::: "memory"); }
__device__ __forceinline__ void bulk_wait_read_all() { asm volatile("cp.async.bulk.wait_group.read 0;\n" ::: "memory"); }
__device__ __forceinline__ void bulk_wait_all() { asm volatile("cp.async.bulk.wait_group 0;\n" ::: "memory"); }
__device__ __forceinline__ void fence_proxy_async_smem() { asm volatile("fence.proxy.async.shared::cta;\n" ::: "memory"); }

template <int NATOM>
__global__ void __launch_bounds__(kWsThreads, 1)
k4_hist_build_ws(const uint8_t* __restrict__ bins, size_t rows_stride, int num_tiles, const int4* __restrict__ qgh,
                 const int4* __restrict__ qord, const int* __restrict__ idx0, const int* __restrict__ idx1,
                 const HistWork* __restrict__ work, unsigned long long* __restrict__ hist) {
  extern __shared__ __align__(128) unsigned char smem_raw[];
  unsigned* plane = reinterpret_cast<unsigned*>(smem_raw);
  unsigned char* stage_bins = smem_raw + 4 * kPlaneWords * 4;
  int4* stage_q = reinterpret_cast<int4*>(stage_bins + kWsStages * kWsStageRows * 32);
  unsigned char* flush_stage = reinterpret_cast<unsigned char*>(stage_q) + kWsStages * kWsStageRows * 16;
  unsigned long long* full_bar = reinterpret_cast<unsigned long long*>(flush_stage + kFlushStageBytes);
  unsigned long long* empty_bar = full_bar + kWsStages;

  const HistWork w = *work;
  const int n = w.count;
  if (n <= 0) return;
  const int tid = threadIdx.x, lane = tid & 31, warp = tid >> 5;
  const int* __restrict__ idx = w.buf ? idx1 : idx0;

  long long cells_rows = static_cast<long long>(n) * num_tiles;
  int rpi = static_cast<int>((cells_rows + 4LL * gridDim.x - 1) / (4LL * gridDim.x));
  rpi = (rpi + kWsStageRows - 1) / kWsStageRows * kWsStageRows;
  rpi = max(rpi, kWsStageRows);
  rpi = min(rpi, kFlushRows);
  const int chunks = (n + rpi - 1) / rpi;
  const long long items = static_cast<long long>(chunks) * num_tiles;
  const int i0 = static_cast<int>(items * blockIdx.x / gridDim.x);
  const int i1 = static_cast<int>(items * (blockIdx.x + 1) / gridDim.x);
  if (i0 >= i1) return;

  if (tid == 0) {
    for (int i = 0; i < kWsStages; ++i) { mbar_init(&full_bar[i], kWsProducerWarps * 32); mbar_init(&empty_bar[i], kWsConsumerWarps); }
    asm volatile("fence.mbarrier_init.release.cluster;\n" ::: "memory");
  }
  for (int e = tid; e < 4 * kPlaneWords; e += kWsThreads) plane[e] = 0u;
  __syncthreads();

  unsigned gs = 0;
  if (warp >= kWsConsumerWarps) {
    const int ptid = tid - kWsConsumerWarps * 32;
    constexpr int kPT = kWsProducerWarps * 32;
    constexpr int kPerLane = kWsStageRows / kPT;
    for (int item = i0; item < i1; ++item) {
      const int tile = item / chunks, chunk = item - tile * chunks;
      const int row0 = chunk * rpi;
      const int nrows = min(rpi, n - row0);
      const int nst = (nrows + kWsStageRows - 1) / kWsStageRows;
      const uint8_t* tbins = bins + static_cast<size_t>(tile) * rows_stride * 32;
      for (int s = 0; s < nst; ++s, ++gs) {
        const int slot = gs % kWsStages;
        mbar_wait(&empty_bar[slot], ((gs / kWsStages) & 1u) ^ 1u);
        const int p0 = row0 + s * kWsStageRows;
        const int rows = min(kWsStageRows, row0 + nrows - p0);
        unsigned char* db = stage_bins + slot * kWsStageRows * 32;
        int4* dq = stage_q + slot * kWsStageRows;
        if (!w.use_idx) {
          if (ptid == 0) {
            mbar_arrive_expect_tx(&full_bar[slot], static_cast<unsigned>(rows) * 48u);
            const size_t r = static_cast<size_t>(w.begin + p0);
            tma_bulk_g2s(db, tbins + r * 32, static_cast<unsigned>(rows) * 32u, &full_bar[slot]);
            tma_bulk_g2s(dq, qgh + r, static_cast<unsigned>(rows) * 16u, &full_bar[slot]);
          } else {
            mbar_arrive(&full_bar[slot]);
          }
        } else {
          const int* ip = idx + w.begin + p0;
          if (ptid == 0) {
            mbar_expect_tx(&full_bar[slot], static_cast<unsigned>(rows) * 16u);
            tma_bulk_g2s(dq, qord + static_cast<size_t>(w.begin + p0), static_cast<unsigned>(rows) * 16u, &full_bar[slot]);
          }
          int rr[2 * kPerLane];
#pragma unroll
          for (int k = 0; k < 2 * kPerLane; ++k) { const int j = (ptid + k * kPT) >> 1; rr[k] = j < rows ? ip[j] : -1; }
#pragma unroll
          for (int k = 0; k < 2 * kPerLane; ++k) {
            const int hh = ptid + k * kPT, j = hh >> 1, half = (hh & 1) * 16;
            if (rr[k] >= 0) cp_async16(db + j * 32 + half, tbins + static_cast<size_t>(rr[k]) * 32 + half, true);
          }
          cp_async_mbar_arrive_noinc(&full_bar[slot]);
        }
      }
    }
    cp_async_wait<0>();
  } else {
#if B200GBM_K4_EXPERIMENT >= 1 && B200GBM_K4_EXPERIMENT <= 3
    unsigned exp_sink = 0;
#endif
    const int sub = lane >> 2, rot = lane & 3;
    int acc_rows = 0;
    for (int item = i0; item < i1; ++item) {
      const int tile = item / chunks, chunk = item - tile * chunks;
      const int row0 = chunk * rpi;
      const int nrows = min(rpi, n - row0);
      const int nst = (nrows + kWsStageRows - 1) / kWsStageRows;
      for (int s = 0; s < nst; ++s, ++gs) {
        const int slot = gs % kWsStages;
        mbar_wait(&full_bar[slot], (gs / kWsStages) & 1u);
        const int rows = min(kWsStageRows, nrows - s * kWsStageRows);
        const unsigned* sw = reinterpret_cast<const unsigned*>(stage_bins + slot * kWsStageRows * 32);
        const int4* sq = stage_q + slot * kWsStageRows;
        const int groups = (rows + 31) >> 5;
        for (int g = warp; g < groups; g += kWsConsumerWarps) {
          const int r = g * 32 + lane;
          if (r < rows) {
            const int4 q = sq[r];
            const unsigned* rw = sw + r * 8;
#pragma unroll
            for (int k = 0; k < 8; ++k) {
              const int w8 = (sub + k) & 7;
              const unsigned word = rw[w8];
#pragma unroll
              for (int j = 0; j < 4; ++j) {
                const int kk = (j + rot) & 3;
                const unsigned b = (word >> (8 * kk)) & 0xFFu;
                const unsigned a = b * 32u + static_cast<unsigned>(w8 * 4 + kk);
#if B200GBM_K4_EXPERIMENT == 0 || B200GBM_K4_EXPERIMENT == 4
                atomicAdd(&plane[a], static_cast<unsigned>(q.x));
                atomicAdd(&plane[kPlaneWords + a], static_cast<unsigned>(q.y));
                atomicAdd(&plane[2 * kPlaneWords + a], static_cast<unsigned>(q.z));
                if (NATOM == 4) atomicAdd(&plane[3 * kPlaneWords + a], static_cast<unsigned>(q.w));
#else
                if (B200GBM_K4_EXPERIMENT >= 2) atomicAdd(&plane[a], static_cast<unsigned>(q.x));
                if (B200GBM_K4_EXPERIMENT >= 3) atomicAdd(&plane[kPlaneWords + a], static_cast<unsigned>(q.y));
                if (B200GBM_K4_EXPERIMENT == 1) exp_sink ^= a + static_cast<unsigned>(q.x ^ q.y ^ q.z ^ q.w);
#endif
              }
            }
          }
        }
#if B200GBM_K4_EXPERIMENT >= 1 && B200GBM_K4_EXPERIMENT <= 3
        if (exp_sink == 0x12345679u) plane[lane] = exp_sink;
#endif
        __syncwarp();
        if (lane == 0) mbar_arrive(&empty_bar[slot]);
      }
      acc_rows += nrows;
      bool flush = (item + 1 == i1);
      if (!flush) {
        const int ntile = (item + 1) / chunks, nchunk = (item + 1) - ntile * chunks;
        const int nnext = min(rpi, n - nchunk * rpi);
        flush = (ntile != tile) || (acc_rows + nnext > kFlushRows);
      }
      if (!flush) continue;
      acc_rows = 0;
      asm volatile("bar.sync 1, %0;\n" ::"n"(kWsConsumerWarps * 32) : "memory");
      unsigned long long* htile = hist + static_cast<size_t>(tile) * kTileFeat * kBins * 2;
      int sbin[2];
#pragma unroll
      for (int i = 0; i < 2; ++i) sbin[i] = (warp + i * kWsConsumerWarps + lane) & (kFlushSlabBins - 1);
      for (int b0 = 0; b0 < kBins; b0 += kFlushSlabBins) {
        long long g[2], h[2];
        bool nz = false;
#pragma unroll
        for (int i = 0; i < 2; ++i) {
          const int e = (b0 + sbin[i]) * kTileFeat + lane;
          const unsigned ghi = plane[e], glo = plane[kPlaneWords + e], hhi = plane[2 * kPlaneWords + e];
          const unsigned hlo = (NATOM == 4) ? plane[3 * kPlaneWords + e] : 0u;
          plane[e] = 0u;
          plane[kPlaneWords + e] = 0u;
          plane[2 * kPlaneWords + e] = 0u;
          if (NATOM == 4) plane[3 * kPlaneWords + e] = 0u;
          nz |= (ghi | glo | hhi | hlo) != 0u;
          g[i] = (static_cast<long long>(static_cast<int>(ghi)) << kLoBits) + static_cast<long long>(glo);
          h[i] = (NATOM == 4) ? (static_cast<long long>(static_cast<int>(hhi)) << kLoBits) + static_cast<long long>(hlo)
                              : static_cast<long long>(hhi);
        }
        if (tid == 0) bulk_wait_read_all();
        asm volatile("bar.sync 1, %0;\n" ::"n"(kWsConsumerWarps * 32) : "memory");
#pragma unroll
        for (int i = 0; i < 2; ++i)
          *reinterpret_cast<longlong2*>(flush_stage + lane * kFlushRowBytes + sbin[i] * 16) = make_longlong2(g[i], h[i]);
        fence_proxy_async_smem();
        int any;
        asm volatile(
            "{\n"
            ".reg .pred p, q;\n"
            "setp.ne.u32 p, %1, 0;\n"
            "bar.red.or.pred q, 1, %2, p;\n"
            "selp.s32 %0, 1, 0, q;\n"
            "}\n"
            : "=r"(any)
            : "r"(static_cast<unsigned>(nz)), "n"(kWsConsumerWarps * 32)
            : "memory");
#if B200GBM_K4_EXPERIMENT != 4
        if (tid == 0 && any) {
          for (int f = 0; f < kTileFeat; ++f)
            bulk_reduce_add_u64(htile + (static_cast<size_t>(f) * kBins + b0) * 2, flush_stage + f * kFlushRowBytes, kFlushSlabBins * 16);
          bulk_commit();
        }
#else
        (void)any; (void)htile;
#endif
      }
    }
    if (tid == 0) bulk_wait_all();
  }
}

inline cudaError_t set_k4_smem_limit() {
  const cudaError_t e = cudaFuncSetAttribute(k4_hist_build_ws<4>, cudaFuncAttributeMaxDynamicSharedMemorySize, kWsSmemBytes);
  if (e != cudaSuccess) return e;
  return cudaFuncSetAttribute(k4_hist_build_ws<3>, cudaFuncAttributeMaxDynamicSharedMemorySize, kWsSmemBytes);
}

inline void launch_k4(bool const_hessian, const uint8_t* bins, size_t rows_stride, int num_tiles, const int4* qgh, const int4* qord,
                      const int* idx0, const int* idx1, const HistWork* work, unsigned long long* hist, int grid, cudaStream_t stream) {
  if (const_hessian)
    k4_hist_build_ws<3><<<grid, kWsThreads, kWsSmemBytes, stream>>>(bins, rows_stride, num_tiles, qgh, qord, idx0, idx1, work, hist);
  else
    k4_hist_build_ws<4><<<grid, kWsThreads, kWsSmemBytes, stream>>>(bins, rows_stride, num_tiles, qgh, qord, idx0, idx1, work, hist);
}

}
```

### mmlspark_b200/csrc/kernels.cuh

```cuda
#pragma once
#include <cstdint>
#include <cuda_runtime.h>
#include "hist_kernel.cuh"

namespace b200gbm {

constexpr double kEpsD = 1e-15;
#define kNegInf (-__longlong_as_double(0x7ff0000000000000LL))

struct FeatMeta {
  int num_bin;
  int missing_type;
  int default_bin;
  int offset;
  int real_index;
  int is_categorical;
  int num_sorted_cats;
  int hist_off;
};

constexpr int kWideHistSeg = 8192;
constexpr int kWideMaxBins = 16384;
constexpr int kCatListMax = 64;
struct WideMeta {
  int num_bin, hist_off, cat_off, num_cats;
  int default_bin, missing_type, real_index, is_cat;
  int offset, pad0, pad1, pad2;
};
struct BinView {
  const uint8_t* bins; size_t rows_stride; const uint16_t* bins16; int nfn;
  __device__ __forceinline__ unsigned at(int u, size_t row) const {
    return u < nfn ? bins[(static_cast<size_t>(u >> 5) * rows_stride + row) * 32 + (u & 31)] : bins16[static_cast<size_t>(u - nfn) * rows_stride + row];
  }
};

struct SplitParams {
  double l1, l2, max_delta_step, min_gain_to_split, min_sum_hessian;
  int min_data_in_leaf, max_depth, num_leaves, parallel;
  int nf, nf_pad, num_tiles, nfn;
  double cat_l2, cat_smooth;
  int max_cat_threshold, max_cat_to_onehot, min_data_per_group, pad3;
};

struct SplitCand {
  double gain;
  double left_g, left_h;
  int threshold, left_count, default_left, feature;
  double l2_extra;
  unsigned cat_bits[8];
  int is_cat, cat_list_len;
  unsigned short cat_list[kCatListMax];
};

struct LeafBest {
  double gain;
  double left_g, left_h, right_g, right_h;
  double left_out, right_out;
  int feature, threshold, default_left, left_count, right_count, is_cat;
  unsigned cat_bits[8];
  int cat_list_len, pad;
  unsigned short cat_list[kCatListMax];
};

struct LeafState {
  int begin, count, buf, depth;
  int global_count, identity, hist_slot, parent_node;
  double sum_g, sum_h;
  LeafBest best;
};

struct TreeCtrl {
  int num_leaves, left_leaf, right_leaf, smaller, larger, go, finished, split_leaf;
  int split_feature, split_threshold, split_default_left, split_missing_type, split_num_bin, new_leaf, pending, pad;
  int part_begin, part_count, part_buf, part_identity, part_left_total, smaller_rows, round, split_is_cat;
  unsigned split_cat_bits[8];
  HistWork hist_work;
  unsigned absmax_bits[2];
  int exp_g, exp_h;
  double inv_g, inv_h;
  long long root_q[4];
  long long trace_rows;
  unsigned scan_ticket;
  int q_side;
  unsigned part_barrier;
  unsigned part_ticket;
  unsigned part_next[2];
  int split_wide;
  int split_cat_list_len;
  unsigned short split_cat_list[kCatListMax];
};

struct TreeDev {
  int* left_child; int* right_child; int* split_feature_inner; int* threshold_bin; int* decision_type;
  float* split_gain; double* leaf_value; double* leaf_weight; int* leaf_count; double* internal_value;
  double* internal_weight; int* internal_count; int* leaf_parent; int* leaf_depth; int* num_leaves;
  unsigned* cat_bits;
  unsigned short* cat_list;
  int* cat_list_len;
};

__device__ __forceinline__ double d_sign(double x) { return (x > 0.0) - (x < 0.0); }
__device__ __forceinline__ double d_threshold_l1(double s, double l1) {
  double r = fmax(0.0, fabs(s) - l1);
  return d_sign(s) * r;
}
__device__ __forceinline__ double d_calc_output(double g, double h, const SplitParams& p) {
  double ret = (p.l1 > 0) ? -d_threshold_l1(g, p.l1) / (h + p.l2) : -g / (h + p.l2);
  if (p.max_delta_step > 0 && fabs(ret) > p.max_delta_step) ret = d_sign(ret) * p.max_delta_step;
  return ret;
}
__device__ __noinline__ double d_leaf_gain(double g, double h, const SplitParams& p) {
  if (!(p.max_delta_step > 0)) {
    if (p.l1 > 0) { double sg = d_threshold_l1(g, p.l1); return (sg * sg) / (h + p.l2); }
    return (g * g) / (h + p.l2);
  }
  double out = d_calc_output(g, h, p);
  double sg = (p.l1 > 0) ? d_threshold_l1(g, p.l1) : g;
  return -(2.0 * sg * out + (h + p.l2) * out * out);
}

template <typename T>
__global__ void __launch_bounds__(256)
k_bin_rows(const T* __restrict__ X, long long nrow, int ncol, int row_major, long long ld, const FeatMeta* __restrict__ meta,
           const double* __restrict__ ub, const uint8_t* __restrict__ catbin, int nf, uint8_t* __restrict__ bins, long long rows_stride,
           long long row_offset) {
  extern __shared__ double s_ub[];
  const int tile = blockIdx.y;
  for (int e = threadIdx.x; e < 32 * 256; e += blockDim.x) {
    int f = tile * 32 + (e >> 8);
    s_ub[(e & 255) * 32 + (e >> 8)] = f < nf ? ub[static_cast<size_t>(f) * 256 + (e & 255)] : 0.0;
  }
  __syncthreads();
  const int lane = threadIdx.x & 31, warp = threadIdx.x >> 5;
  const int u = tile * 32 + lane;
  FeatMeta m;
  m.num_bin = 1; m.missing_type = 0; m.real_index = 0; m.is_categorical = 0; m.num_sorted_cats = 0;
  if (u < nf) m = meta[u];
  const double* myub = s_ub + lane;
  for (long long r = blockIdx.x * 8LL + warp; r < nrow; r += gridDim.x * 8LL) {
    unsigned bin = 0;
    if (u < nf) {
      double v = row_major ? static_cast<double>(X[r * ld + m.real_index]) : static_cast<double>(X[static_cast<long long>(m.real_index) * ld + r]);
      if (m.is_categorical) {
        if (!isnan(v)) {
          const int iv = static_cast<int>(v);
          if (iv >= 0) {
            int lo = 0, hi = m.num_sorted_cats;
            while (lo < hi) { int mid = (lo + hi) >> 1; if (static_cast<int>(myub[mid * 32]) < iv) lo = mid + 1; else hi = mid; }
            if (lo < m.num_sorted_cats && static_cast<int>(myub[lo * 32]) == iv) bin = catbin[static_cast<size_t>(u) * 256 + lo];
          }
        }
      } else {
        if (isnan(v)) {
          if (m.missing_type == 2) bin = m.num_bin - 1; else v = 0.0;
        }
        if (!isnan(v)) {
          int lo = 0, hi = m.num_bin - 1 - (m.missing_type == 2 ? 1 : 0);
          while (lo < hi) {
            int mid = (hi + lo - 1) / 2;
            if (v <= myub[mid * 32]) hi = mid; else lo = mid + 1;
          }
          bin = lo;
        }
      }
    }
    bins[(static_cast<size_t>(tile) * rows_stride + row_offset + r) * 32 + lane] = static_cast<uint8_t>(bin);
  }
}

__global__ void k_grad_l2(const double* __restrict__ score, const float* __restrict__ label, const float* __restrict__ weight,
                          float* __restrict__ g, float* __restrict__ h, int n) {
  for (int i = blockIdx.x * blockDim.x + threadIdx.x; i < n; i += gridDim.x * blockDim.x) {
    if (weight) { g[i] = static_cast<float>((score[i] - label[i]) * weight[i]); h[i] = weight[i]; }
    else { g[i] = static_cast<float>(score[i] - label[i]); h[i] = 1.0f; }
  }
}
__global__ void k_grad_regvar(const double* __restrict__ score, const float* __restrict__ label, const float* __restrict__ weight,
                              float* __restrict__ g, float* __restrict__ h, int n, int kind, double alpha, double c, double mds, double rho) {
  for (int i = blockIdx.x * blockDim.x + threadIdx.x; i < n; i += gridDim.x * blockDim.x) {
    const double s = score[i], lab = label[i];
    double gg, hh;
    if (kind == 1) { const double diff = s - lab; gg = fabs(diff) <= alpha ? diff : d_sign(diff) * alpha; hh = 1.0; }
    else if (kind == 2) { const double x = s - lab; gg = c * x / (fabs(x) + c); hh = c * c / ((fabs(x) + c) * (fabs(x) + c)); }
    else if (kind == 3) { gg = exp(s) - lab; hh = exp(s + mds); }
    else if (kind == 4) { gg = 1.0 - lab * exp(-s); hh = lab * exp(-s); }
    else { gg = -lab * exp((1 - rho) * s) + exp((2 - rho) * s); hh = -lab * (1 - rho) * exp((1 - rho) * s) + (2 - rho) * exp((2 - rho) * s); }
    if (weight) { gg *= weight[i]; hh *= weight[i]; }
    g[i] = static_cast<float>(gg); h[i] = static_cast<float>(hh);
  }
}
__global__ void k_grad_percentile(const double* __restrict__ score, const float* __restrict__ label, const float* __restrict__ weight,
                                  const float* __restrict__ label_weight, float* __restrict__ g, float* __restrict__ h, int n, int kind, float alpha) {
  for (int i = blockIdx.x * blockDim.x + threadIdx.x; i < n; i += gridDim.x * blockDim.x) {
    if (kind == 2) {
      const float delta = static_cast<float>(score[i] - label[i]);
      const float gg = delta >= 0 ? (1.0f - alpha) : -alpha;
      g[i] = weight ? __fmul_rn(gg, weight[i]) : gg;
    } else {
      const double diff = score[i] - label[i];
      const int sgn = (diff > 0.0) - (diff < 0.0);
      if (kind == 1) g[i] = weight ? static_cast<float>(sgn * static_cast<double>(weight[i])) : static_cast<float>(sgn);
      else g[i] = static_cast<float>(sgn * static_cast<double>(label_weight[i]));
    }
    h[i] = weight ? weight[i] : 1.0f;
  }
}
__global__ void k_grad_binary(const double* __restrict__ score, const float* __restrict__ label, const float* __restrict__ weight,
                              float* __restrict__ g, float* __restrict__ h, int n, double sigmoid, double w_neg, double w_pos) {
  for (int i = blockIdx.x * blockDim.x + threadIdx.x; i < n; i += gridDim.x * blockDim.x) {
    const int is_pos = label[i] > 0;
    const double lab = is_pos ? 1.0 : -1.0;
    const double lw = is_pos ? w_pos : w_neg;
    const double response = -lab * sigmoid / (1.0 + exp(lab * sigmoid * score[i]));
    const double abs_response = fabs(response);
    double gg = response * lw, hh = abs_response * (sigmoid - abs_response) * lw;
    if (weight) { gg *= weight[i]; hh *= weight[i]; }
    g[i] = static_cast<float>(gg); h[i] = static_cast<float>(hh);
  }
}
__global__ void k_grad_ova(const double* __restrict__ score, const float* __restrict__ label, const float* __restrict__ weight, float* __restrict__ g,
                           float* __restrict__ h, int n, int K, double sigmoid, const double* __restrict__ cw, const uint8_t* __restrict__ need) {
  for (int i = blockIdx.x * blockDim.x + threadIdx.x; i < n; i += gridDim.x * blockDim.x) {
    const int li = static_cast<int>(label[i]);
    for (int k = 0; k < K; ++k) {
      if (!need[k]) continue;
      const size_t id = static_cast<size_t>(n) * k + i;
      const int is_pos = li == k;
      const double lab = is_pos ? 1.0 : -1.0;
      const double lw = cw[2 * k + is_pos];
      const double response = -lab * sigmoid / (1.0 + exp(lab * sigmoid * score[id]));
      const double abs_response = fabs(response);
// ... 5 lines not shown
}
__global__ void k_grad_xent(const double* __restrict__ score, const float* __restrict__ label, const float* __restrict__ weight, float* __restrict__ g,
                            float* __restrict__ h, int n) {
  for (int i = blockIdx.x * blockDim.x + threadIdx.x; i < n; i += gridDim.x * blockDim.x) {
    const double z = 1.0 / (1.0 + exp(-score[i]));
    double gg = z - label[i], hh = z * (1.0 - z);
    if (weight) { gg *= weight[i]; hh *= weight[i]; }
    g[i] = static_cast<float>(gg); h[i] = static_cast<float>(hh);
  }
}
__global__ void k_grad_softmax(const double* __restrict__ score, const float* __restrict__ label, const float* __restrict__ weight,
                               float* __restrict__ g, float* __restrict__ h, int n, int K, double factor) {
  for (int i = blockIdx.x * blockDim.x + threadIdx.x; i < n; i += gridDim.x * blockDim.x) {
    double wmax = score[i];
    for (int k = 1; k < K; ++k) wmax = fmax(wmax, score[static_cast<size_t>(n) * k + i]);
    double wsum = 0;
    for (int k = 0; k < K; ++k) wsum += exp(score[static_cast<size_t>(n) * k + i] - wmax);
    const int lab = static_cast<int>(label[i]);
    const double w = weight ? weight[i] : 1.0;
    for (int k = 0; k < K; ++k) {
      double p = exp(score[static_cast<size_t>(n) * k + i] - wmax) / wsum;
      double gg = (lab == k) ? p - 1.0 : p, hh = factor * p * (1.0 - p);
      if (weight) { gg *= w; hh *= w; }
      g[static_cast<size_t>(n) * k + i] = static_cast<float>(gg);
      h[static_cast<size_t>(n) * k + i] = static_cast<float>(hh);
    }
  }
}

constexpr int kLrThreads = 128;
__host__ __device__ inline int lr_tile(int truncation) {
  int t = (48 * 1024 / 8) / max(truncation, 1) - 1;
  t = min(t, 128);
  return max(t & ~31, 32);
}
__global__ void __launch_bounds__(kLrThreads)
k_grad_lambdarank(const double* __restrict__ score, const float* __restrict__ label, const float* __restrict__ weight,
                  const int* __restrict__ qb, int nq, const double* __restrict__ inv_max_dcg, const double* __restrict__ label_gain,
                  const double* __restrict__ discount, const float* __restrict__ sig_table, int sig_bins, double min_in, double max_in,
                  double idx_factor, double sigmoid, int truncation, int norm, float* __restrict__ g, float* __restrict__ h, int max_q) {
  extern __shared__ unsigned char lr_smem[];
  double* r_score = reinterpret_cast<double*>(lr_smem);
  double* s_score = r_score + max_q;
  int* s_lab = reinterpret_cast<int*>(s_score + max_q);
  int* s_orig = s_lab + max_q;
  float* s_lam = reinterpret_cast<float*>(s_orig + max_q);
  float* s_hes = s_lam + max_q;
  float2* M = reinterpret_cast<float2*>(s_hes + max_q);
  __shared__ double s_part[kLrThreads];
  const int T = lr_tile(truncation), TS = T + 1;
  for (int q = blockIdx.x; q < nq; q += gridDim.x) {
    const int start = qb[q], cnt = qb[q + 1] - start;
    __syncthreads();
    for (int i = threadIdx.x; i < cnt; i += blockDim.x) r_score[i] = score[start + i];
    __syncthreads();
    for (int i = threadIdx.x; i < cnt; i += blockDim.x) {
      const double si = r_score[i];
      int rank = 0;
      for (int j = 0; j < cnt; ++j) {
        const double sj = r_score[j];
        rank += (sj > si) || (sj == si && j < i);
      }
      s_score[rank] = si; s_lab[rank] = static_cast<int>(label[start + i]); s_orig[rank] = i;
      s_lam[rank] = 0.f; s_hes[rank] = 0.f;
    }
    __syncthreads();
    const double imd = inv_max_dcg[q];
    const double best_score = s_score[0];
    int worst_idx = cnt - 1;
    if (worst_idx > 0 && s_score[worst_idx] == kNegInf) worst_idx -= 1;
    const double worst_score = s_score[worst_idx];
    const bool do_div = norm && best_score != worst_score;
    const int teff = min(truncation, cnt - 1);
    double local_sum = 0.0;
    for (int j0 = 0; j0 < cnt; j0 += T) {
      const int tcnt = min(T, cnt - j0);
      for (int e = threadIdx.x; e < teff * tcnt; e += blockDim.x) {
        const int i = e / tcnt, jj = e - i * tcnt, j = j0 + jj;
        float2 m = make_float2(0.f, 0.f);
        if (j > i) {
          const double sci = s_score[i], scj = s_score[j];
          const int li = s_lab[i], lj = s_lab[j];
          if (sci != kNegInf && scj != kNegInf && li != lj) {
            const bool ih = li > lj;
            const int hr = ih ? i : j, lr = ih ? j : i;
            const double delta_score = ih ? sci - scj : scj - sci;
            const double dcg_gap = label_gain[ih ? li : lj] - label_gain[ih ? lj : li];
            const double paired_discount = fabs(discount[hr] - discount[lr]);
            double delta = dcg_gap * paired_discount * imd;
            if (do_div) delta /= (0.01f + fabs(delta_score));
            double pl;
            if (delta_score <= min_in) pl = sig_table[0];
            else if (delta_score >= max_in) pl = sig_table[sig_bins - 1];
            else pl = sig_table[static_cast<size_t>((delta_score - min_in) * idx_factor)];
            double ph = pl * (1.0f - pl);
            pl *= -sigmoid * delta;
            ph *= sigmoid * sigmoid * delta;
            local_sum -= 2 * pl;
            const float fl = static_cast<float>(pl);
            m = make_float2(ih ? fl : -fl, static_cast<float>(ph));
          }
        }
        M[i * TS + jj] = m;
      }
      __syncthreads();
      for (int p = threadIdx.x; p < cnt; p += blockDim.x) {
        const bool as_j = p >= j0 && p < j0 + tcnt, as_i = p < teff && p + 1 < j0 + tcnt;
        if (!as_j && !as_i) continue;
        float lam = s_lam[p], hes = s_hes[p];
        if (as_j) {
          const int ilim = min(p, teff);
          for (int i = 0; i < ilim; ++i) { const float2 m = M[i * TS + (p - j0)]; lam = __fsub_rn(lam, m.x); hes = __fadd_rn(hes, m.y); }
        }
        if (as_i) {
          for (int j = max(j0, p + 1); j < j0 + tcnt; ++j) { const float2 m = M[p * TS + (j - j0)]; lam = __fadd_rn(lam, m.x); hes = __fadd_rn(hes, m.y); }
        }
        s_lam[p] = lam; s_hes[p] = hes;
      }
      __syncthreads();
    }
    s_part[threadIdx.x] = local_sum;
    __syncthreads();
    double sum_lambdas = 0.0;
    if (norm) for (int t = 0; t < static_cast<int>(blockDim.x); ++t) sum_lambdas += s_part[t];
    double nf = 1.0;
    const bool do_norm = norm && sum_lambdas > 0;
    if (do_norm) nf = log2(1 + sum_lambdas) / sum_lambdas;
    for (int r = threadIdx.x; r < cnt; r += blockDim.x) {
      float lam = s_lam[r], hes = s_hes[r];
      if (do_norm) { lam = static_cast<float>(lam * nf); hes = static_cast<float>(hes * nf); }
      const int o = start + s_orig[r];
      if (weight) { lam = static_cast<float>(lam * weight[o]); hes = static_cast<float>(hes * weight[o]); }
      g[o] = lam; h[o] = hes;
    }
  }
}

__global__ void k_absmax(const float* __restrict__ g, const float* __restrict__ h, int n, TreeCtrl* ctrl) {
  float mg = 0.f, mh = 0.f;
  for (int i = blockIdx.x * blockDim.x + threadIdx.x; i < n; i += gridDim.x * blockDim.x) {
    mg = fmaxf(mg, fabsf(g[i])); mh = fmaxf(mh, fabsf(h[i]));
  }
  for (int o = 16; o; o >>= 1) { mg = fmaxf(mg, __shfl_xor_sync(0xffffffffu, mg, o)); mh = fmaxf(mh, __shfl_xor_sync(0xffffffffu, mh, o)); }
  if ((threadIdx.x & 31) == 0) {
    atomicMax(&ctrl->absmax_bits[0], __float_as_uint(mg));
    atomicMax(&ctrl->absmax_bits[1], __float_as_uint(mh));
  }
}
__global__ void k_set_scale(TreeCtrl* ctrl, int const_hessian, double hess_const) {
  float mg = __uint_as_float(ctrl->absmax_bits[0]), mh = __uint_as_float(ctrl->absmax_bits[1]);
  int eg = (mg > 0.f && isfinite(mg)) ? 34 - ilogbf(mg) : 0;
  int eh = (mh > 0.f && isfinite(mh)) ? 34 - ilogbf(mh) : 0;
  eg = max(min(eg, 1000), -1000); eh = max(min(eh, 1000), -1000);
  ctrl->exp_g = eg; ctrl->exp_h = eh;
  ctrl->inv_g = ldexp(1.0, -eg);
  ctrl->inv_h = const_hessian ? hess_const : ldexp(1.0, -eh);
  ctrl->root_q[0] = 0; ctrl->root_q[1] = 0; ctrl->root_q[2] = 0; ctrl->root_q[3] = 0;
}
__global__ void __launch_bounds__(256)
k_quantize(const float* __restrict__ g, const float* __restrict__ h, int n, int4* __restrict__ qgh, TreeCtrl* ctrl, int const_hessian,
           const uint8_t* __restrict__ in_bag, int bag_count) {
  const int eg = ctrl->exp_g, eh = ctrl->exp_h;
  long long sg = 0, sh = 0;
  for (int i = blockIdx.x * blockDim.x + threadIdx.x; i < n; i += gridDim.x * blockDim.x) {
    long long qg = __double2ll_rn(ldexp(static_cast<double>(g[i]), eg));
    int4 q;
    q.x = static_cast<int>(qg >> kLoBits); q.y = static_cast<int>(qg & ((1LL << kLoBits) - 1));
    long long qh;
    if (const_hessian) { qh = 1; q.z = 1; q.w = 0; }
    else { qh = __double2ll_rn(ldexp(static_cast<double>(h[i]), eh)); q.z = static_cast<int>(qh >> kLoBits); q.w = static_cast<int>(qh & ((1LL << kLoBits) - 1)); }
    qgh[i] = q;
    if (!in_bag || in_bag[i]) { sg += qg; sh += qh; }
  }
  for (int o = 16; o; o >>= 1) { sg += __shfl_xor_sync(0xffffffffu, sg, o); sh += __shfl_xor_sync(0xffffffffu, sh, o); }
  __shared__ long long s_g[8], s_h[8];
  int lane = threadIdx.x & 31, warp = threadIdx.x >> 5;
  if (lane == 0) { s_g[warp] = sg; s_h[warp] = sh; }
  __syncthreads();
  if (threadIdx.x == 0) {
    long long a = 0, b = 0;
    for (int w = 0; w < 8; ++w) { a += s_g[w]; b += s_h[w]; }
    atomicAdd(reinterpret_cast<unsigned long long*>(&ctrl->root_q[0]), static_cast<unsigned long long>(a));
    atomicAdd(reinterpret_cast<unsigned long long*>(&ctrl->root_q[1]), static_cast<unsigned long long>(b));
    if (blockIdx.x == 0) atomicAdd(reinterpret_cast<unsigned long long*>(&ctrl->root_q[2]), static_cast<unsigned long long>(in_bag ? bag_count : n));
  }
}

__global__ void __launch_bounds__(256)
k_tree_init(TreeCtrl* ctrl, LeafState* leaves, TreeDev tree, uint8_t* flags, SplitParams p, int n_local, const uint8_t* feature_used,
            int root_is_bag) {
  for (int u = threadIdx.x; u < p.nf_pad; u += blockDim.x) flags[u] = (u < p.nf && (!feature_used || feature_used[u])) ? 1 : 0;
  for (int l = threadIdx.x; l < p.num_leaves; l += blockDim.x) {
    leaves[l].best.gain = kNegInf; leaves[l].best.feature = -1;
    tree.leaf_parent[l] = -1; tree.leaf_depth[l] = 0; tree.leaf_value[l] = 0; tree.leaf_weight[l] = 0; tree.leaf_count[l] = 0;
  }
  if (threadIdx.x == 0) {
    LeafState& r = leaves[0];
    r.begin = 0; r.count = n_local; r.buf = 0; r.depth = 0; r.identity = root_is_bag ? 0 : 1; r.hist_slot = 0; r.parent_node = -1;
    r.global_count = static_cast<int>(ctrl->root_q[2]);
    r.sum_g = static_cast<double>(ctrl->root_q[0]) * ctrl->inv_g;
    r.sum_h = static_cast<double>(ctrl->root_q[1]) * ctrl->inv_h;
    ctrl->num_leaves = 1; ctrl->left_leaf = 0; ctrl->right_leaf = -1; ctrl->smaller = 0; ctrl->larger = -1;
    ctrl->go = 0; ctrl->finished = 0; ctrl->split_leaf = -1; ctrl->pending = 0; ctrl->round = 0; ctrl->trace_rows = 0;
    *tree.num_leaves = 1;
  }
}

__device__ __forceinline__ void
d_round_ctl(TreeCtrl* ctrl, LeafState* leaves, const TreeDev& tree, uint8_t* flags, const FeatMeta* __restrict__ meta, const SplitParams& p, int last,
            int* s_copy) {
  if (threadIdx.x == 0) {
    s_copy[0] = -1; s_copy[1] = -1;
    if (ctrl->pending) {
      ctrl->pending = 0;
      const int leaf = ctrl->split_leaf, nl = ctrl->new_leaf;
      LeafState& L = leaves[leaf];
      LeafState& R = leaves[nl];
      LeafBest b = L.best;
      const int true_left = __ldcg(&ctrl->part_left_total), true_right = ctrl->part_count - true_left;
      if (!p.parallel) { b.left_count = true_left; b.right_count = true_right; }
      const int node = ctrl->num_leaves - 1;
      const int parent = tree.leaf_parent[leaf];
      if (parent >= 0) {
        if (tree.left_child[parent] == ~leaf) tree.left_child[parent] = node; else tree.right_child[parent] = node;
      }
      tree.split_feature_inner[node] = b.feature;
      tree.split_gain[node] = static_cast<float>(b.gain + p.min_gain_to_split);
      tree.left_child[node] = ~leaf; tree.right_child[node] = ~nl;
      tree.leaf_parent[leaf] = node; tree.leaf_parent[nl] = node;
      tree.internal_weight[node] = tree.leaf_weight[leaf];
      tree.internal_value[node] = tree.leaf_value[leaf];
      tree.internal_count[node] = b.left_count + b.right_count;
      tree.leaf_value[leaf] = isnan(b.left_out) ? 0.0 : b.left_out;
      tree.leaf_weight[leaf] = b.left_h; tree.leaf_count[leaf] = b.left_count;
      tree.leaf_value[nl] = isnan(b.right_out) ? 0.0 : b.right_out;
      tree.leaf_weight[nl] = b.right_h; tree.leaf_count[nl] = b.right_count;
      tree.leaf_depth[nl] = tree.leaf_depth[leaf] + 1; tree.leaf_depth[leaf] += 1;
      const FeatMeta fm = meta[b.feature];
      if (b.is_cat) {
        tree.decision_type[node] = 1 | (fm.missing_type << 2);
        tree.threshold_bin[node] = 0;
      } else {
        tree.decision_type[node] = (b.default_left ? 2 : 0) | (fm.missing_type << 2);
        tree.threshold_bin[node] = b.threshold;
      }
      for (int wd = 0; wd < 8; ++wd) tree.cat_bits[node * 8 + wd] = b.is_cat ? b.cat_bits[wd] : 0u;
      tree.cat_list_len[node] = b.is_cat ? b.cat_list_len : 0;
      if (b.is_cat) for (int k = 0; k < b.cat_list_len && k < kCatListMax; ++k) tree.cat_list[node * kCatListMax + k] = b.cat_list[k];
      ctrl->num_leaves += 1; *tree.num_leaves = ctrl->num_leaves;
      const int dst_buf = L.identity ? 0 : (L.buf ^ 1);
      R.begin = L.begin + true_left; R.count = true_right; R.buf = dst_buf; R.identity = 0; R.depth = L.depth + 1;
      L.count = true_left; L.buf = dst_buf; L.identity = 0; L.depth += 1;
      L.global_count = b.left_count; R.global_count = b.right_count;
      L.sum_g = b.left_g; L.sum_h = b.left_h; R.sum_g = b.right_g; R.sum_h = b.right_h;
      R.hist_slot = nl;
      L.best.gain = kNegInf; L.best.feature = -1; R.best.gain = kNegInf; R.best.feature = -1;
      ctrl->left_leaf = leaf; ctrl->right_leaf = nl;
    }
    ctrl->go = 0; ctrl->smaller = -1; ctrl->larger = -1; ctrl->split_leaf = -1;
    ctrl->hist_work.count = 0; ctrl->part_count = 0;
    if (!ctrl->finished && !last && ctrl->num_leaves < p.num_leaves) {
      const int ll = ctrl->left_leaf, rl = ctrl->right_leaf;
      bool go = true;
      if (p.max_depth > 0 && tree.leaf_depth[ll] >= p.max_depth) go = false;
      const int nl_cnt = leaves[ll].global_count, nr_cnt = rl >= 0 ? leaves[rl].global_count : 0;
      if (go && nr_cnt < p.min_data_in_leaf * 2 && nl_cnt < p.min_data_in_leaf * 2) go = false;
      if (!go) {
        leaves[ll].best.gain = kNegInf;
        if (rl >= 0) leaves[rl].best.gain = kNegInf;
      } else {
        int smaller = ll, larger = -1;
        if (rl >= 0) {
          if (nl_cnt < nr_cnt) { smaller = ll; larger = rl; } else { smaller = rl; larger = ll; }
          if (larger == rl) { int t = leaves[ll].hist_slot; leaves[ll].hist_slot = leaves[rl].hist_slot; leaves[rl].hist_slot = t; }
          s_copy[0] = ll; s_copy[1] = rl;
        }
        ctrl->smaller = smaller; ctrl->larger = larger; ctrl->go = 1;
        const LeafState& S = leaves[smaller];
        ctrl->hist_work.begin = S.begin; ctrl->hist_work.count = S.count; ctrl->hist_work.use_idx = S.identity ? 0 : 1;
        ctrl->hist_work.buf = S.buf;
        ctrl->smaller_rows = S.count;
        ctrl->trace_rows += S.count;
      }
    }
    ctrl->round += 1;
  }
  __syncthreads();
  if (s_copy[0] >= 0)
    for (int u = threadIdx.x; u < p.nf_pad; u += blockDim.x) flags[static_cast<size_t>(s_copy[1]) * p.nf_pad + u] = flags[static_cast<size_t>(s_copy[0]) * p.nf_pad + u];
}
__global__ void __launch_bounds__(256)
k_round_ctl(TreeCtrl* ctrl, LeafState* leaves, TreeDev tree, uint8_t* flags, const FeatMeta* __restrict__ meta, SplitParams p,
            int last) {
  __shared__ int s_copy[2];
  d_round_ctl(ctrl, leaves, tree, flags, meta, p, last, s_copy);
}

__device__ __forceinline__ long long warp_suffix_excl(long long v, int lane) {
  long long inc = v;
  for (int o = 1; o < 32; o <<= 1) { long long t = __shfl_down_sync(0xffffffffu, inc, o); if (lane + o < 32) inc += t; }
  return inc - v;
}
__device__ __forceinline__ long long warp_prefix_excl(long long v, int lane) {
  long long inc = v;
  for (int o = 1; o < 32; o <<= 1) { long long t = __shfl_up_sync(0xffffffffu, inc, o); if (lane >= o) inc += t; }
  return inc - v;
}

__device__ __forceinline__ void d_scan_feature(const long long (&qg)[8], const long long (&qh)[8], int lane, const FeatMeta m, const LeafState& L,
                                               double inv_g, double inv_h, const SplitParams& p, uint8_t* flag, SplitCand* outp) {
  SplitCand& out = *outp;
  const double sum_g = L.sum_g, sum_h = L.sum_h + 2 * kEpsD;
  const int num_data = L.global_count;
  const double cnt_factor = num_data / sum_h;
  const double min_gain_shift = d_leaf_gain(sum_g, sum_h, p) + p.min_gain_to_split;
  const bool two_way = (m.num_bin > 2 && m.missing_type == 2);
  const int na = two_way ? 1 : 0;

  int cnt[8];
#pragma unroll 1
  for (int j = 0; j < 8; ++j) cnt[j] = static_cast<int>(static_cast<double>(qh[j]) * inv_h * cnt_factor + 0.5);

  double best_gain = kNegInf, best_lg = 0, best_lh = 0;
  int best_thr = -1, best_lc = 0, best_dl = 1;
  bool any_valid = false;
// ... 425 lines not shown
#pragma unroll
      for (int rr = 0; rr < 4; ++rr) if (r0 + rr < pt.world) { sx += vx[rr]; sy += vy[rr]; }
    }
    for (int r = 0; r < pt.world; ++r)
      asm volatile("st.volatile.global.v2.s64 [%0], {%1, %2};\n" ::"l"(const_cast<long long*>(pt.H[r]) + i * 2), "l"(sx), "l"(sy) : "memory");
  }
  __threadfence_system();
  __syncthreads();
  if (threadIdx.x == 0) s_last = (atomicAdd(ticket, 1u) == gridDim.x - 1) ? 1 : 0;
  __syncthreads();
  if (!s_last) return;
  if (threadIdx.x == 0) *ticket = 0u;
  __threadfence_system();
  if (threadIdx.x < pt.world) *reinterpret_cast<volatile unsigned*>(&pt.flags[threadIdx.x][16 + pt.rank]) = epoch;
  if (threadIdx.x == 0) peer_wait(pt.flags[pt.rank] + 16, pt.world, epoch, pt.error);
  __syncthreads();
}




__global__ void __launch_bounds__(256)
k_pick_dp(TreeCtrl* ctrl, LeafState* leaves, const FeatMeta* __restrict__ meta, const SplitCand* __restrict__ cands, SplitParams p,
          PeerTables pt, unsigned epoch) {
  __shared__ double s_gain[256];
  __shared__ int s_feat[256], s_idx[256];
  const bool go = ctrl->go != 0;
  if (go) {
    for (int which = 0; which < 2; ++which) {
      const int leaf = which ? ctrl->larger : ctrl->smaller;
      double bg = kNegInf; int bf = 0x7fffffff, bi = -1;
      if (leaf >= 0) {
        for (int u = pt.feat0 + threadIdx.x; u < pt.feat1 && u < p.nf; u += blockDim.x) {
          const SplitCand& c = cands[which * p.nf_pad + u];
          const int rf = meta[u].real_index;
          if (c.gain > bg || (c.gain == bg && rf < bf)) { bg = c.gain; bf = rf; bi = u; }
        }
      }
      s_gain[threadIdx.x] = bg; s_feat[threadIdx.x] = bf; s_idx[threadIdx.x] = bi;
      __syncthreads();
      for (int s = 128; s; s >>= 1) {
        if (threadIdx.x < s) {
          double og = s_gain[threadIdx.x + s]; int of = s_feat[threadIdx.x + s];
          if (og > s_gain[threadIdx.x] || (og == s_gain[threadIdx.x] && of < s_feat[threadIdx.x])) {
            s_gain[threadIdx.x] = og; s_feat[threadIdx.x] = of; s_idx[threadIdx.x] = s_idx[threadIdx.x + s];
          }
        }
        __syncthreads();
      }
      if (threadIdx.x < pt.world) {
        SplitCand c;
        c.gain = kNegInf; c.left_g = 0; c.left_h = 0; c.threshold = 0; c.left_count = 0; c.default_left = 1; c.feature = -1;
        if (s_idx[0] >= 0 && s_gain[0] > kNegInf) c = cands[which * p.nf_pad + s_idx[0]];
        SplitCand* dst = pt.mail[threadIdx.x] + pt.rank * 2 + which;
        volatile double* dd = reinterpret_cast<volatile double*>(dst);
        dd[0] = c.gain; dd[1] = c.left_g; dd[2] = c.left_h;
        volatile int* di = reinterpret_cast<volatile int*>(dd + 3);
        di[0] = c.threshold; di[1] = c.left_count; di[2] = c.default_left; di[3] = c.feature;
      }
      __syncthreads();
    }
  }
  __threadfence_system();
  __syncthreads();
  if (threadIdx.x < pt.world) *reinterpret_cast<volatile unsigned*>(&pt.flags[threadIdx.x][16 + pt.rank]) = epoch;
  if (threadIdx.x == 0) peer_wait(pt.flags[pt.rank] + 16, pt.world, epoch, pt.error);
  __syncthreads();
  if (threadIdx.x == 0 && go) {
    for (int which = 0; which < 2; ++which) {
      const int leaf = which ? ctrl->larger : ctrl->smaller;
      if (leaf < 0) continue;
      SplitCand best;
      best.gain = kNegInf; best.feature = -1; best.left_g = best.left_h = 0; best.threshold = 0; best.left_count = 0; best.default_left = 1;
      int best_rf = 0x7fffffff;
      const SplitCand* mb = pt.mail[pt.rank];
      for (int r = 0; r < pt.world; ++r) {
        SplitCand c;
        const volatile double* dd = reinterpret_cast<const volatile double*>(mb + r * 2 + which);
        c.gain = dd[0]; c.left_g = dd[1]; c.left_h = dd[2];
        const volatile int* di = reinterpret_cast<const volatile int*>(dd + 3);
        c.threshold = di[0]; c.left_count = di[1]; c.default_left = di[2]; c.feature = di[3];
        const int rf = c.feature < 0 ? 0x7fffffff : meta[c.feature].real_index;
        if (c.gain > best.gain || (c.gain == best.gain && rf < best_rf)) { best = c; best_rf = rf; }
      }
      LeafState& L = leaves[leaf];
      LeafBest b;
      b.gain = kNegInf; b.feature = -1; b.threshold = 0; b.default_left = 1; b.left_count = 0; b.right_count = 0;
      b.left_g = b.left_h = b.right_g = b.right_h = b.left_out = b.right_out = 0; b.is_cat = 0; b.cat_list_len = 0; b.pad = 0;
      for (int wd = 0; wd < 8; ++wd) b.cat_bits[wd] = 0u;
      if (best.feature >= 0 && best.gain > kNegInf) {
        const double sum_h = L.sum_h + 2 * kEpsD;
        b.gain = best.gain; b.feature = best.feature; b.threshold = best.threshold; b.default_left = best.default_left;
        b.left_count = best.left_count; b.right_count = L.global_count - best.left_count;
        b.left_g = best.left_g; b.left_h = best.left_h - kEpsD;
        b.right_g = L.sum_g - best.left_g; b.right_h = sum_h - best.left_h - kEpsD;
        b.left_out = d_calc_output(best.left_g, best.left_h, p);
        b.right_out = d_calc_output(L.sum_g - best.left_g, sum_h - best.left_h, p);
      }
      L.best = b;
    }
  }
  __syncthreads();
  if (threadIdx.x < 32 && !ctrl->finished) d_choose_leaf(ctrl, leaves, meta, p, threadIdx.x);
}

__global__ void __launch_bounds__(256)
k_tiles_to_columns(const uint8_t* __restrict__ bins, size_t rows_stride, int num_tiles, long long nrow, uint8_t* __restrict__ cols, size_t cols_stride) {
  __shared__ uint4 s_t[256 * 2 + 16];
  const long long per_tile = (nrow + 255) / 256;
  for (long long w = blockIdx.x; w < per_tile * num_tiles; w += gridDim.x) {
    const int tile = static_cast<int>(w / per_tile);
    const long long r0 = (w % per_tile) * 256;
    const int rows = static_cast<int>(min(256LL, nrow - r0));
    const uint4* src = reinterpret_cast<const uint4*>(bins + (static_cast<size_t>(tile) * rows_stride + static_cast<size_t>(r0)) * 32);
    __syncthreads();
    for (int i = threadIdx.x; i < rows * 2; i += 256) s_t[i] = src[i];
    __syncthreads();
    const uint8_t* sb = reinterpret_cast<const uint8_t*>(s_t);
    const int f = threadIdx.x >> 3, g = threadIdx.x & 7;
    unsigned wv[8];
#pragma unroll
    for (int k = 0; k < 8; ++k) {
      unsigned v = 0;
#pragma unroll
      for (int j = 0; j < 4; ++j) { const int r = g * 32 + k * 4 + j; v |= (r < rows ? static_cast<unsigned>(sb[r * 32 + f]) : 0u) << (8 * j); }
      wv[k] = v;
    }
    uint4* dst = reinterpret_cast<uint4*>(cols + (static_cast<size_t>(tile) * 32 + f) * cols_stride + static_cast<size_t>(r0) + g * 32);
    dst[0] = make_uint4(wv[0], wv[1], wv[2], wv[3]);
    dst[1] = make_uint4(wv[4], wv[5], wv[6], wv[7]);
  }
}

constexpr int kPartChunk = 2048;
constexpr int kPartLocalScan = 2048;
__device__ __forceinline__ bool d_goes_left(unsigned bin, const TreeCtrl* c) {
  if (c->split_is_cat) return (c->split_cat_bits[bin >> 5] >> (bin & 31u)) & 1u;
  if (c->split_missing_type == 2 && bin == static_cast<unsigned>(c->split_num_bin - 1)) return c->split_default_left != 0;
  return bin <= static_cast<unsigned>(c->split_threshold);
}
__device__ __forceinline__ void d_grid_barrier(unsigned* counter, unsigned target) {
  __syncthreads();
  if (threadIdx.x == 0) {
    __threadfence();
    atomicAdd(counter, 1u);
    while (*reinterpret_cast<volatile unsigned*>(counter) < target) __nanosleep(32);
    __threadfence();
  }
  __syncthreads();
}
__global__ void __launch_bounds__(256, 3)
k_partition(TreeCtrl* ctrl, LeafState* leaves, TreeDev tree, uint8_t* flags, const FeatMeta* __restrict__ meta, SplitParams p, int last,
            const uint8_t* __restrict__ bins, size_t rows_stride, int* __restrict__ idx0, int* __restrict__ idx1, unsigned* __restrict__ bits,
            int* __restrict__ chunk_left, const int4* __restrict__ qgh, int4* __restrict__ qord, long long* __restrict__ H, size_t h_elems,
            const uint16_t* __restrict__ bins16, int tickets_per_block, const uint8_t* __restrict__ cols, size_t cols_stride, int* __restrict__ super_tot) {
  __shared__ int s_pref[kPartLocalScan + 1];
  __shared__ unsigned short s_list[kCatListMax];
  __shared__ int s_wl[64];
  __shared__ int s_cnt[8];
  __shared__ int s_copy[2];
  __shared__ int s_last;
  __shared__ int s_chunk;
  const int lane = threadIdx.x & 31, warp = threadIdx.x >> 5;
  {
    longlong2* h2 = reinterpret_cast<longlong2*>(H);
    const size_t n2 = h_elems / 2;
    const longlong2 z = make_longlong2(0, 0);
    for (size_t i = blockIdx.x * static_cast<size_t>(blockDim.x) + threadIdx.x; i < n2; i += static_cast<size_t>(gridDim.x) * blockDim.x) h2[i] = z;
  }
  const int n = ctrl->part_count;
  if (n > 0) {
    const int* src = ctrl->part_buf ? idx1 : idx0;
    int* dst = ctrl->part_identity ? idx0 : (ctrl->part_buf ? idx0 : idx1);
    const int begin = ctrl->part_begin, identity = ctrl->part_identity;
    const int f = ctrl->split_feature;
    const int wide = ctrl->split_wide;
    const uint8_t* col = bins + (static_cast<size_t>((wide >= 0 ? 0 : f) >> 5) * rows_stride) * 32 + ((wide >= 0 ? 0 : f) & 31);
    const uint16_t* wcol = wide >= 0 ? bins16 + static_cast<size_t>(wide) * rows_stride : nullptr;
    const uint8_t* ccol = (cols != nullptr && wide < 0) ? cols + static_cast<size_t>(f) * cols_stride : nullptr;
    const bool wide_cat = wide >= 0 && ctrl->split_is_cat;
    const int list_len = wide_cat ? ctrl->split_cat_list_len : 0;
    if (threadIdx.x < list_len) s_list[threadIdx.x] = ctrl->split_cat_list[threadIdx.x];
    __syncthreads();
    const int chunks = (n + kPartChunk - 1) / kPartChunk;
    const int grp = tickets_per_block > 0 ? max(1, chunks / (static_cast<int>(gridDim.x) * tickets_per_block)) : 1;
    for (;;) {
      __syncthreads();
      if (threadIdx.x == 0) s_chunk = static_cast<int>(atomicAdd(&ctrl->part_next[0], 1u));
      __syncthreads();
      const int cbase = s_chunk * grp;
      if (cbase >= chunks) break;
      for (int c = cbase; c < min(cbase + grp, chunks); ++c) {
      int local = 0;
      int rr[8]; unsigned bb[8];
#pragma unroll
      for (int k = 0; k < 8; ++k) {
        const int i = c * kPartChunk + k * 256 + threadIdx.x;
        rr[k] = i < n ? (identity ? (begin + i) : src[begin + i]) : -1;
      }
#pragma unroll
      for (int k = 0; k < 8; ++k) {
        bb[k] = 0u;
        if (rr[k] >= 0)
          bb[k] = wide >= 0 ? static_cast<unsigned>(wcol[rr[k]]) : (ccol ? static_cast<unsigned>(ccol[rr[k]]) : static_cast<unsigned>(col[static_cast<size_t>(rr[k]) * 32]));
      }
#pragma unroll
      for (int k = 0; k < 8; ++k) {
        bool left = false;
        if (rr[k] >= 0) {
          const unsigned bin = bb[k];
          if (wide_cat) { for (int kk = 0; kk < list_len; ++kk) left |= (bin == s_list[kk]); }
          else left = d_goes_left(bin, ctrl);
        }
        const unsigned bal = __ballot_sync(0xffffffffu, left);
        if (lane == 0) { bits[(c * kPartChunk + k * 256 + threadIdx.x) >> 5] = bal; local += __popc(bal); }
      }
      if (lane == 0 && local) atomicAdd(&chunk_left[c], local);
      }
    }
    d_grid_barrier(&ctrl->part_barrier, gridDim.x);
    int total_left;
    const bool local_scan = chunks <= kPartLocalScan;
    if (local_scan) {
      int v[8], sum = 0;
#pragma unroll
      for (int k = 0; k < 8; ++k) { const int i = threadIdx.x * 8 + k; v[k] = i < chunks ? __ldcg(chunk_left + i) : 0; sum += v[k]; }
      int inc = sum;
      for (int o = 1; o < 32; o <<= 1) { const int t = __shfl_up_sync(0xffffffffu, inc, o); if (lane >= o) inc += t; }
      if (lane == 31) s_cnt[warp] = inc;
      __syncthreads();
      int woff = 0;
      for (int w = 0; w < warp; ++w) woff += s_cnt[w];
      int run = woff + inc - sum;
#pragma unroll
      for (int k = 0; k < 8; ++k) { s_pref[threadIdx.x * 8 + k] = run; run += v[k]; }
      if (threadIdx.x == 255) s_pref[kPartLocalScan] = run;
      __syncthreads();
      total_left = s_pref[kPartLocalScan];
    } else {
      const int supers = (chunks + kPartLocalScan - 1) / kPartLocalScan;
      for (int sp = blockIdx.x; sp < supers; sp += gridDim.x) {
        int v[8], sum = 0;
#pragma unroll
        for (int k = 0; k < 8; ++k) { const int i = sp * kPartLocalScan + threadIdx.x * 8 + k; v[k] = i < chunks ? __ldcg(chunk_left + i) : 0; sum += v[k]; }
        int inc = sum;
        for (int o = 1; o < 32; o <<= 1) { const int t = __shfl_up_sync(0xffffffffu, inc, o); if (lane >= o) inc += t; }
        __syncthreads();
        if (lane == 31) s_cnt[warp] = inc;
        __syncthreads();
        int woff = 0;
        for (int w = 0; w < warp; ++w) woff += s_cnt[w];
        int run = woff + inc - sum;
#pragma unroll
        for (int k = 0; k < 8; ++k) { const int i = sp * kPartLocalScan + threadIdx.x * 8 + k; if (i < chunks) chunk_left[i] = run; run += v[k]; }
        if (threadIdx.x == 255) super_tot[sp] = run;
      }
      d_grid_barrier(&ctrl->part_barrier, 2 * gridDim.x);
      {
        int v[8], sum = 0;
#pragma unroll
        for (int k = 0; k < 8; ++k) { const int i = threadIdx.x * 8 + k; v[k] = i < supers ? __ldcg(super_tot + i) : 0; sum += v[k]; }
        int inc = sum;
        for (int o = 1; o < 32; o <<= 1) { const int t = __shfl_up_sync(0xffffffffu, inc, o); if (lane >= o) inc += t; }
        __syncthreads();
        if (lane == 31) s_cnt[warp] = inc;
        __syncthreads();
        int woff = 0;
        for (int w = 0; w < warp; ++w) woff += s_cnt[w];
        int run = woff + inc - sum;
#pragma unroll
        for (int k = 0; k < 8; ++k) { s_pref[threadIdx.x * 8 + k] = run; run += v[k]; }
        if (threadIdx.x == 255) s_pref[kPartLocalScan] = run;
        __syncthreads();
        total_left = s_pref[kPartLocalScan];
      }
    }
    const LeafBest& bsp = leaves[ctrl->split_leaf].best;
    const int lc = p.parallel ? bsp.left_count : total_left, rc = p.parallel ? bsp.right_count : n - total_left;
    const bool q_left = lc < rc;
    for (;;) {
      __syncthreads();
      if (threadIdx.x == 0) s_chunk = static_cast<int>(atomicAdd(&ctrl->part_next[1], 1u));
      __syncthreads();
      const int cbase = s_chunk * grp;
      if (cbase >= chunks) break;
      for (int c = cbase; c < min(cbase + grp, chunks); ++c) {
      const int wbase = c * (kPartChunk / 32);
      if (threadIdx.x < 64) {
        const int i0 = c * kPartChunk + threadIdx.x * 32;
        s_wl[threadIdx.x] = i0 < n ? __popc(__ldcg(bits + wbase + threadIdx.x)) : 0;
      }
      __syncthreads();
      if (warp == 0) {
        const int a = s_wl[lane * 2], b = s_wl[lane * 2 + 1];
        const int sum = a + b;
        int inc = sum;
        for (int o = 1; o < 32; o <<= 1) { const int t = __shfl_up_sync(0xffffffffu, inc, o); if (lane >= o) inc += t; }
        const int ex = inc - sum;
        s_wl[lane * 2] = ex; s_wl[lane * 2 + 1] = ex + a;
      }
      __syncthreads();
      const int left_base = local_scan ? s_pref[c] : s_pref[c / kPartLocalScan] + __ldcg(chunk_left + c);
      const int right_base = c * kPartChunk - left_base;
      int rr[8], pp[8]; bool qq[8]; int4 qv[8];
#pragma unroll
      for (int k = 0; k < 8; ++k) {
        const int w = k * 8 + warp;
        const int i = c * kPartChunk + w * 32 + lane;
        rr[k] = -1; pp[k] = 0; qq[k] = false;
        if (i < n) {
          const unsigned word = __ldcg(bits + wbase + w);
          const bool left = (word >> lane) & 1u;
          const int lefts_before = s_wl[w] + __popc(word & ((1u << lane) - 1u));
          rr[k] = identity ? (begin + i) : src[begin + i];
          pp[k] = left ? begin + left_base + lefts_before : begin + total_left + right_base + (w * 32 + lane - lefts_before);
          qq[k] = (left == q_left);
        }
      }
#pragma unroll
      for (int k = 0; k < 8; ++k) if (qq[k]) qv[k] = qgh[rr[k]];
#pragma unroll
      for (int k = 0; k < 8; ++k) {
        if (rr[k] < 0) continue;
        dst[pp[k]] = rr[k];
        if (qq[k]) qord[pp[k]] = qv[k];
      }
      __syncthreads();
      }
    }
    if (blockIdx.x == 0 && threadIdx.x == 0) ctrl->part_left_total = total_left;
  }
  __syncthreads();
  if (threadIdx.x == 0) {
    __threadfence();
    const unsigned t = atomicAdd(&ctrl->part_ticket, 1u);
    s_last = (t == gridDim.x - 1) ? 1 : 0;
  }
  __syncthreads();
  if (s_last) {
    __threadfence();
    if (threadIdx.x == 0) { ctrl->part_ticket = 0u; ctrl->part_barrier = 0u; ctrl->part_next[0] = 0u; ctrl->part_next[1] = 0u; }
    if (n > 0) for (int c = threadIdx.x; c < (n + kPartChunk - 1) / kPartChunk; c += blockDim.x) chunk_left[c] = 0;
    d_round_ctl(ctrl, leaves, tree, flags, meta, p, last, s_copy);
  }
}

__device__ __forceinline__ unsigned d_wide_bin(double v, const WideMeta& m, const int* __restrict__ cats, const unsigned short* __restrict__ catbin,
                                               const double* __restrict__ wub) {
  unsigned bin = 0;
  if (m.is_cat) {
    if (!isnan(v)) {
      const int iv = static_cast<int>(v);
      if (iv >= 0) {
        const int* c = cats + m.cat_off;
        int lo = 0, hi = m.num_cats;
        while (lo < hi) { const int mid = (lo + hi) >> 1; if (c[mid] < iv) lo = mid + 1; else hi = mid; }
        if (lo < m.num_cats && c[lo] == iv) bin = catbin[m.cat_off + lo];
      }
    }
    return bin;
  }
  if (isnan(v)) { if (m.missing_type == 2) return static_cast<unsigned>(m.num_bin - 1); v = 0.0; }
  const double* ub = wub + m.cat_off;
  int lo = 0, hi = m.num_bin - 1 - (m.missing_type == 2 ? 1 : 0);
  while (lo < hi) { const int mid = (hi + lo - 1) / 2; if (v <= ub[mid]) hi = mid; else lo = mid + 1; }
  return static_cast<unsigned>(lo);
}
template <typename T>
__global__ void k_bin_wide(const T* __restrict__ X, long long nrow, int row_major, long long ld, const WideMeta* __restrict__ wm, int nw,
                           const int* __restrict__ cats, const unsigned short* __restrict__ catbin, const double* __restrict__ wub,
                           uint16_t* __restrict__ bins16, size_t rows_stride, long long row_offset) {
  const long long total = nrow * nw;
  for (long long e = blockIdx.x * static_cast<long long>(blockDim.x) + threadIdx.x; e < total; e += static_cast<long long>(gridDim.x) * blockDim.x) {
    const int w = static_cast<int>(e / nrow);
    const long long r = e - static_cast<long long>(w) * nrow;
    const WideMeta m = wm[w];
    const double v = row_major ? static_cast<double>(X[r * ld + m.real_index]) : static_cast<double>(X[static_cast<long long>(m.real_index) * ld + r]);
    bins16[static_cast<size_t>(w) * rows_stride + row_offset + r] = static_cast<uint16_t>(d_wide_bin(v, m, cats, catbin, wub));
  }
}

constexpr int kWideThreads = 1024;
template <int NATOM>
__global__ void __launch_bounds__(kWideThreads, 1)
k4_hist_wide(const uint16_t* __restrict__ bins16, size_t rows_stride, const WideMeta* __restrict__ wm, const int4* __restrict__ qgh,
             const int4* __restrict__ qord, const int* __restrict__ idx0, const int* __restrict__ idx1, const HistWork* __restrict__ work,
             unsigned long long* __restrict__ hist) {
  extern __shared__ __align__(16) unsigned wplane[];
  const HistWork w = *work;
  const int n = w.count;
  if (n <= 0) return;
  const int active = min(static_cast<int>(gridDim.x), (n + 4095) / 4096);
  if (static_cast<int>(blockIdx.x) >= active) return;
  const WideMeta m = wm[blockIdx.y];
  const unsigned lo = blockIdx.z * kWideHistSeg;
  if (static_cast<int>(lo) >= m.num_bin) return;
  const int nb = min(kWideHistSeg, m.num_bin - static_cast<int>(lo));
  const int p0 = static_cast<int>(static_cast<long long>(n) * blockIdx.x / active), p1 = static_cast<int>(static_cast<long long>(n) * (blockIdx.x + 1) / active);
  const int* __restrict__ idx = w.buf ? idx1 : idx0;
  const uint16_t* __restrict__ col = bins16 + static_cast<size_t>(blockIdx.y) * rows_stride;
  unsigned* pl0 = wplane; unsigned* pl1 = wplane + kWideHistSeg; unsigned* pl2 = wplane + 2 * kWideHistSeg; unsigned* pl3 = wplane + 3 * kWideHistSeg;
  for (int e = threadIdx.x; e < nb; e += kWideThreads) { pl0[e] = 0u; pl1[e] = 0u; pl2[e] = 0u; if (NATOM == 4) pl3[e] = 0u; }
  __syncthreads();
  for (int c0 = p0; c0 < p1; c0 += kFlushRows) {
    const int c1 = min(c0 + kFlushRows, p1);
    for (int p = c0 + threadIdx.x; p < c1; p += 4 * kWideThreads) {
      int4 q[4]; unsigned b[4]; size_t r[4];
#pragma unroll
      for (int j = 0; j < 4; ++j) {
        const int pj = p + j * kWideThreads;
        r[j] = 0;
        if (pj < c1) {
          if (w.use_idx) { r[j] = static_cast<size_t>(idx[w.begin + pj]); q[j] = qord[w.begin + pj]; }
          else { r[j] = static_cast<size_t>(w.begin + pj); q[j] = qgh[r[j]]; }
        }
      }
#pragma unroll
      for (int j = 0; j < 4; ++j) b[j] = (p + j * kWideThreads < c1) ? static_cast<unsigned>(col[r[j]]) - lo : 0xffffffffu;
#pragma unroll
      for (int j = 0; j < 4; ++j) {
        if (b[j] >= static_cast<unsigned>(nb)) continue;
        atomicAdd(&pl0[b[j]], static_cast<unsigned>(q[j].x));
        atomicAdd(&pl1[b[j]], static_cast<unsigned>(q[j].y));
        atomicAdd(&pl2[b[j]], static_cast<unsigned>(q[j].z));
        if (NATOM == 4) atomicAdd(&pl3[b[j]], static_cast<unsigned>(q[j].w));
      }
    }
    __syncthreads();
    for (int e = threadIdx.x; e < nb; e += kWideThreads) {
      const unsigned ghi = pl0[e], glo = pl1[e], hhi = pl2[e], hlo = (NATOM == 4) ? pl3[e] : 0u;
      if (ghi | glo | hhi | hlo) {
        const long long g = (static_cast<long long>(static_cast<int>(ghi)) << kLoBits) + static_cast<long long>(glo);
        const long long h = (NATOM == 4) ? (static_cast<long long>(static_cast<int>(hhi)) << kLoBits) + static_cast<long long>(hlo) : static_cast<long long>(hhi);
        const size_t o = (static_cast<size_t>(m.hist_off) + lo + e) * 2;
        if (g) atomicAdd(&hist[o], static_cast<unsigned long long>(g));
        if (h) atomicAdd(&hist[o + 1], static_cast<unsigned long long>(h));
        pl0[e] = 0u; pl1[e] = 0u; pl2[e] = 0u; if (NATOM == 4) pl3[e] = 0u;
      }
    }
    __syncthreads();
  }
}

__device__ __forceinline__ void d_block_excl3(long long& a, long long& b, long long& c, int reverse, long long* sm) {
  const int lane = threadIdx.x & 31, warp = threadIdx.x >> 5;
  long long ia = a, ib = b, ic = c;
  for (int o = 1; o < 32; o <<= 1) {
    long long ta, tb, tc;
    if (reverse) { ta = __shfl_down_sync(0xffffffffu, ia, o); tb = __shfl_down_sync(0xffffffffu, ib, o); tc = __shfl_down_sync(0xffffffffu, ic, o); if (lane + o < 32) { ia += ta; ib += tb; ic += tc; } }
    else { ta = __shfl_up_sync(0xffffffffu, ia, o); tb = __shfl_up_sync(0xffffffffu, ib, o); tc = __shfl_up_sync(0xffffffffu, ic, o); if (lane >= o) { ia += ta; ib += tb; ic += tc; } }
  }
  __syncthreads();
  if (lane == (reverse ? 0 : 31)) { sm[warp] = ia; sm[8 + warp] = ib; sm[16 + warp] = ic; }
  __syncthreads();
  long long oa = 0, ob = 0, oc = 0;
  for (int w2 = 0; w2 < 8; ++w2) if (reverse ? w2 > warp : w2 < warp) { oa += sm[w2]; ob += sm[8 + w2]; oc += sm[16 + w2]; }
  a = oa + ia - a; b = ob + ib - b; c = oc + ic - c;
  __syncthreads();
}

__device__ __noinline__ void d_scan_wide_numeric(const long long* __restrict__ hist, const WideMeta m, const LeafState& L, double inv_g, double inv_h,
                                                  const SplitParams& p, uint8_t* flag, SplitCand* outp) {
  __shared__ long long s_sc[24];
  __shared__ double s_bg[8], s_blg[8], s_blh[8];
  __shared__ int s_bt[8], s_blc[8], s_any;
  __shared__ long long s_tot[3];
  const int lane = threadIdx.x & 31, warp = threadIdx.x >> 5;
  const double sum_g = L.sum_g, sum_h = L.sum_h + 2 * kEpsD;
  const int num_data = L.global_count;
  const double cnt_factor = num_data / sum_h;
  const double min_gain_shift = d_leaf_gain(sum_g, sum_h, p) + p.min_gain_to_split;
  const bool two_way = (m.num_bin > 2 && m.missing_type == 2);
  const int na = two_way ? 1 : 0;
  const int S = (m.num_bin + 255) / 256;
  const int b0 = threadIdx.x * S, b1 = min(b0 + S, m.num_bin);
  if (threadIdx.x == 0) s_any = 0;
  bool any_valid = false;
  double best_gain = kNegInf, best_lg = 0, best_lh = 0;
  int best_thr = -1, best_lc = 0, best_dl = 1;
  {
    const int hi = m.num_bin - 1 - na;
    long long lg = 0, lh = 0, lc = 0;
    for (int b = b0; b < b1; ++b)
      if (b >= 1 && b <= hi) { const long long qh = hist[b * 2 + 1]; lg += hist[b * 2]; lh += qh; lc += static_cast<int>(static_cast<double>(qh) * inv_h * cnt_factor + 0.5); }
    long long rg = lg, rh = lh, rc = lc;
    d_block_excl3(rg, rh, rc, 1, s_sc);
    for (int b = b1 - 1; b >= b0; --b) {
      if (b < 1 || b > hi) continue;
      const long long qg = hist[b * 2], qh = hist[b * 2 + 1];
      rg += qg; rh += qh; rc += static_cast<int>(static_cast<double>(qh) * inv_h * cnt_factor + 0.5);
      const double srg = static_cast<double>(rg) * inv_g;
      const double srh = kEpsD + static_cast<double>(rh) * inv_h;
      const int right_count = static_cast<int>(rc);
      if (right_count < p.min_data_in_leaf || srh < p.min_sum_hessian) continue;
      const int left_count = num_data - right_count;
      if (left_count < p.min_data_in_leaf) continue;
      const double slh = sum_h - srh;
      if (slh < p.min_sum_hessian) continue;
      const double slg = sum_g - srg;
      const double gain = d_leaf_gain(slg, slh, p) + d_leaf_gain(srg, srh, p);
      if (gain <= min_gain_shift) continue;
      any_valid = true;
      if (gain > best_gain) { best_gain = gain; best_lg = slg; best_lh = slh; best_thr = b - 1; best_lc = left_count; }
    }
    for (int o = 16; o; o >>= 1) {
      const double og = __shfl_xor_sync(0xffffffffu, best_gain, o);
      const int ot = __shfl_xor_sync(0xffffffffu, best_thr, o);
      const double olg = __shfl_xor_sync(0xffffffffu, best_lg, o), olh = __shfl_xor_sync(0xffffffffu, best_lh, o);
      const int olc = __shfl_xor_sync(0xffffffffu, best_lc, o);
      if (og > best_gain || (og == best_gain && ot > best_thr)) { best_gain = og; best_thr = ot; best_lg = olg; best_lh = olh; best_lc = olc; }
    }
    if (lane == 0) { s_bg[warp] = best_gain; s_bt[warp] = best_thr; s_blg[warp] = best_lg; s_blh[warp] = best_lh; s_blc[warp] = best_lc; }
    __syncthreads();
    for (int w2 = 0; w2 < 8; ++w2)
      if (s_bg[w2] > best_gain || (s_bg[w2] == best_gain && s_bt[w2] > best_thr)) { best_gain = s_bg[w2]; best_thr = s_bt[w2]; best_lg = s_blg[w2]; best_lh = s_blh[w2]; best_lc = s_blc[w2]; }
    __syncthreads();
  }
  if (two_way) {
    const int hi = m.num_bin - 2;
    long long ag = 0, ah = 0, ac = 0, lg = 0, lh = 0, lc = 0;
    for (int b = b0; b < b1; ++b) {
      const long long qg = hist[b * 2], qh = hist[b * 2 + 1];
      const int c = static_cast<int>(static_cast<double>(qh) * inv_h * cnt_factor + 0.5);
      if (b >= 1 && b < m.num_bin) { ag += qg; ah += qh; ac += c; }
      if (b >= m.offset && b <= hi) { lg += qg; lh += qh; lc += c; }
    }
    {
      long long ta = ag, tb = ah, tc = ac;
      for (int o = 16; o; o >>= 1) { ta += __shfl_xor_sync(0xffffffffu, ta, o); tb += __shfl_xor_sync(0xffffffffu, tb, o); tc += __shfl_xor_sync(0xffffffffu, tc, o); }
      if (lane == 0) { s_sc[warp] = ta; s_sc[8 + warp] = tb; s_sc[16 + warp] = tc; }
      __syncthreads();
      if (threadIdx.x == 0) { long long x = 0, y = 0, z = 0; for (int w2 = 0; w2 < 8; ++w2) { x += s_sc[w2]; y += s_sc[8 + w2]; z += s_sc[16 + w2]; } s_tot[0] = x; s_tot[1] = y; s_tot[2] = z; }
      __syncthreads();
      ag = s_tot[0]; ah = s_tot[1]; ac = s_tot[2];
    }
    long long pg = lg, ph = lh, pc = lc;
    d_block_excl3(pg, ph, pc, 0, s_sc);
    double base_g = 0.0, base_h = kEpsD; int base_c = 0;
    if (m.offset == 1) {
      base_g = sum_g - static_cast<double>(ag) * inv_g;
      base_h = (sum_h - kEpsD) - static_cast<double>(ah) * inv_h;
      base_c = num_data - static_cast<int>(ac);
    }
    double f_gain = kNegInf, f_lg = 0, f_lh = 0; int f_thr = 1 << 30, f_lc = 0;
    for (int b = b0; b < b1; ++b) {
      if (b > hi) continue;
      if (b >= m.offset) { const long long qh = hist[b * 2 + 1]; pg += hist[b * 2]; ph += qh; pc += static_cast<int>(static_cast<double>(qh) * inv_h * cnt_factor + 0.5); }
      const double slg = base_g + static_cast<double>(pg) * inv_g;
      const double slh = base_h + static_cast<double>(ph) * inv_h;
      const int left_count = base_c + static_cast<int>(pc);
      if (left_count < p.min_data_in_leaf || slh < p.min_sum_hessian) continue;
      const int right_count = num_data - left_count;
      if (right_count < p.min_data_in_leaf) continue;
      const double srh = sum_h - slh;
      if (srh < p.min_sum_hessian) continue;
      const double srg = sum_g - slg;
      const double gain = d_leaf_gain(slg, slh, p) + d_leaf_gain(srg, srh, p);
      if (gain <= min_gain_shift) continue;
      any_valid = true;
      if (gain > f_gain) { f_gain = gain; f_lg = slg; f_lh = slh; f_thr = b; f_lc = left_count; }
    }
    for (int o = 16; o; o >>= 1) {
      const double og = __shfl_xor_sync(0xffffffffu, f_gain, o);
      const int ot = __shfl_xor_sync(0xffffffffu, f_thr, o);
      const double olg = __shfl_xor_sync(0xffffffffu, f_lg, o), olh = __shfl_xor_sync(0xffffffffu, f_lh, o);
      const int olc = __shfl_xor_sync(0xffffffffu, f_lc, o);
      if (og > f_gain || (og == f_gain && ot < f_thr)) { f_gain = og; f_thr = ot; f_lg = olg; f_lh = olh; f_lc = olc; }
    }
    if (lane == 0) { s_bg[warp] = f_gain; s_bt[warp] = f_thr; s_blg[warp] = f_lg; s_blh[warp] = f_lh; s_blc[warp] = f_lc; }
    __syncthreads();
    for (int w2 = 0; w2 < 8; ++w2)
      if (s_bg[w2] > f_gain || (s_bg[w2] == f_gain && s_bt[w2] < f_thr)) { f_gain = s_bg[w2]; f_thr = s_bt[w2]; f_lg = s_blg[w2]; f_lh = s_blh[w2]; f_lc = s_blc[w2]; }
    __syncthreads();
    if (f_gain > best_gain) { best_gain = f_gain; best_thr = f_thr; best_lg = f_lg; best_lh = f_lh; best_lc = f_lc; best_dl = 0; }
  } else if (m.missing_type == 2) {
    best_dl = 0;
  }
  if (any_valid) atomicOr(&s_any, 1);
// ... 662 lines not shown
```

Baseline: 5.598.

## Stream fp32 (g,h) pairs instead of int4 quantized rows into histogram kernels

Gradients and hessians are stored as float2 (8 bytes per row) instead of pre-quantized int4 (16 bytes), and the histogram kernels convert them to fixed-point on the fly using the per-tree exponents. This halves the per-row gradient traffic in the partition gather, the ordered copy and the TMA stage loads, at the cost of double-precision multiply and round work inside the consumer warps. The change also raises the pipeline stages from 3 to 4 and prefetches the next stage's row indices before waiting on the empty barrier.

```diff
diff --git a/mmlspark_b200/csrc/engine.cu b/mmlspark_b200/csrc/engine.cu
--- a/mmlspark_b200/csrc/engine.cu
+++ b/mmlspark_b200/csrc/engine.cu
@@ -541,7 +541,7 @@
   const int n = num_data;
   DevBuf<float> g, h; g.Alloc(n); h.Alloc(n);
   g.Upload(grad, n, stream); h.Upload(hess, n, stream);
-  DevBuf<int4> q; q.Alloc(n);
+  DevBuf<float2> q; q.Alloc(static_cast<size_t>(n) + kGhPad);
   DevBuf<TreeCtrl> ctrl; ctrl.Alloc(1); ctrl.Zero(stream);
   DevBuf<int> didx; didx.Alloc(std::max(cnt, 1));
   if (idx) didx.Upload(idx, cnt, stream);
@@ -552,12 +552,12 @@
   B200_CUDA(cudaDeviceGetAttribute(&sms, cudaDevAttrMultiProcessorCount, device));
   k_absmax<<<sms * 4, 256, 0, stream>>>(g.p, h.p, n, ctrl.p);
   k_set_scale<<<1, 1, 0, stream>>>(ctrl.p, 0, 1.0);
-  k_quantize<<<sms * 4, 256, 0, stream>>>(g.p, h.p, n, q.p, ctrl.p, 0, nullptr, 0);
+  k_pack_gh<<<sms * 4, 256, 0, stream>>>(g.p, h.p, n, q.p, ctrl.p, 0, nullptr, 0);
   HistWork w{0, cnt, idx ? 1 : 0, 0};
   B200_CUDA(cudaMemcpyAsync(&ctrl.p->hist_work, &w, sizeof(w), cudaMemcpyHostToDevice, stream));
-  DevBuf<int4> qo; qo.Alloc(std::max(cnt, 1));
-  k_gather_q<<<sms * 4, 256, 0, stream>>>(&ctrl.p->hist_work, didx.p, didx.p, q.p, qo.p);
-  launch_k4(false, bins.p, rows_stride, num_tiles, q.p, qo.p, didx.p, didx.p, &ctrl.p->hist_work,
+  DevBuf<float2> qo; qo.Alloc(static_cast<size_t>(std::max(cnt, 1)) + kGhPad);
+  k_gather_gh<<<sms * 4, 256, 0, stream>>>(&ctrl.p->hist_work, didx.p, didx.p, q.p, qo.p);
+  launch_k4(false, bins.p, rows_stride, num_tiles, q.p, qo.p, ctrl.p->exp_gh, didx.p, didx.p, &ctrl.p->hist_work,
             reinterpret_cast<unsigned long long*>(H.p), sms, stream);
   k_hist_to_double<<<sms * 4, 256, 0, stream>>>(H.p, D.p, elems, ctrl.p);
   B200_CUDA(cudaGetLastError());
@@ -927,7 +927,7 @@
 
   score_.Alloc(static_cast<size_t>(K) * n); score_.Zero(stream_);
   grad_.Alloc(static_cast<size_t>(K) * n); hess_.Alloc(static_cast<size_t>(K) * n);
-  qgh_.Alloc(n); qord_.Alloc(n); idx0_.Alloc(n); idx1_.Alloc(n);
+  gh_.Alloc(static_cast<size_t>(n) + kGhPad); ghord_.Alloc(static_cast<size_t>(n) + kGhPad); idx0_.Alloc(n); idx1_.Alloc(n);
   slot_elems_ = train->hist_pairs * 2;
   H_.Alloc(slot_elems_); H_.Zero(stream_); pool_.Alloc(slot_elems_ * L);
   {
@@ -1311,8 +1311,8 @@
   int* i0 = idx0_.p; int* i1 = idx1_.p;
   unsigned* bits = part_bits_.p;
   int* chunks = part_chunks_.p;
-  const int4* qgh = qgh_.p;
-  int4* qord = qord_.p;
+  const float2* gh = gh_.p;
+  float2* ghord = ghord_.p;
   long long* H = H_.p;
   size_t h_elems = slot_elems_;
   const uint16_t* bins16 = d.bins16.p;
@@ -1321,7 +1321,7 @@
   const uint8_t* cols = bins_cols_.p;
   size_t cols_stride = cols_stride_;
   int* super_tot = part_chunks_.p + (train->num_data / kPartChunk + 2);
-  void* args[] = {&ctrl, &leaves, &tree, &flags, &meta, &sp, &last, &bins, &rows_stride, &i0, &i1, &bits, &chunks, &qgh, &qord, &H, &h_elems, &bins16, &tickets_per_block,
+  void* args[] = {&ctrl, &leaves, &tree, &flags, &meta, &sp, &last, &bins, &rows_stride, &i0, &i1, &bits, &chunks, &gh, &ghord, &H, &h_elems, &bins16, &tickets_per_block,
                   &cols, &cols_stride, &super_tot};
   B200_CUDA(cudaLaunchCooperativeKernel(reinterpret_cast<void*>(k_partition), dim3(grid), dim3(256), args, 0, stream_));
 }
@@ -1342,7 +1342,7 @@
   k_absmax<<<egrid, 256, 0, s>>>(g, h, n, ctrl);
   if (parallel_) B200_NCCL(ncclAllReduce(&ctrl->absmax_bits[0], &ctrl->absmax_bits[0], 2, ncclUint32, ncclMax, Net().comm, s));
   k_set_scale<<<1, 1, 0, s>>>(ctrl, const_hessian_ ? 1 : 0, 1.0);
-  k_quantize<<<egrid, 256, 0, s>>>(g, h, n, qgh_.p, ctrl, const_hessian_ ? 1 : 0, use_bag_ ? in_bag_.p : nullptr, bag_count_);
+  k_pack_gh<<<egrid, 256, 0, s>>>(g, h, n, gh_.p, ctrl, const_hessian_ ? 1 : 0, use_bag_ ? in_bag_.p : nullptr, bag_count_);
   if (parallel_) B200_NCCL(ncclAllReduce(&ctrl->root_q[0], &ctrl->root_q[0], 3, ncclInt64, ncclSum, Net().comm, s));
   ResetFeaturesByTree();
   if (use_bag_)
@@ -1361,10 +1361,10 @@
   for (int split = 0; split < L - 1; ++split) {
     mark();
     if (profile_hist) { cudaEvent_t a, b; B200_CUDA(cudaEventCreate(&a)); B200_CUDA(cudaEventCreate(&b)); evs.push_back(a); evs.push_back(b); B200_CUDA(cudaEventRecord(a, s)); }
-    if (split == 0 && use_bag_) k_gather_q<<<egrid, 256, 0, s>>>(&ctrl->hist_work, idx0_.p, idx1_.p, qgh_.p, qord_.p);
+    if (split == 0 && use_bag_) k_gather_gh<<<egrid, 256, 0, s>>>(&ctrl->hist_work, idx0_.p, idx1_.p, gh_.p, ghord_.p);
     mark();
     nvtxRangePushA("b200gbm:K4 histogram");
-    launch_k4(const_hessian_, d.bins.p, d.rows_stride, d.num_tiles, qgh_.p, qord_.p, idx0_.p, idx1_.p, &ctrl->hist_work,
+    launch_k4(const_hessian_, d.bins.p, d.rows_stride, d.num_tiles, gh_.p, ghord_.p, ctrl->exp_gh, idx0_.p, idx1_.p, &ctrl->hist_work,
               reinterpret_cast<unsigned long long*>(H_.p), num_sms_, s);
     if (d.nw > 0) {
       int max_nb = 0;
@@ -1374,10 +1374,10 @@
       for (const WideMeta& wm : d.wide_host) units += (wm.num_bin + kWideHistSeg - 1) / kWideHistSeg;
       const dim3 wgrid(static_cast<unsigned>(std::max(1, std::min(64, 4 * num_sms_ / std::max(1, units)))), static_cast<unsigned>(d.nw), static_cast<unsigned>(segs));
       if (const_hessian_)
-        k4_hist_wide<3><<<wgrid, kWideThreads, 4 * kWideHistSeg * 4, s>>>(d.bins16.p, d.rows_stride, d.wide_meta.p, qgh_.p, qord_.p, idx0_.p, idx1_.p, &ctrl->hist_work,
+        k4_hist_wide<3><<<wgrid, kWideThreads, 4 * kWideHistSeg * 4, s>>>(d.bins16.p, d.rows_stride, d.wide_meta.p, gh_.p, ghord_.p, ctrl->exp_gh, idx0_.p, idx1_.p, &ctrl->hist_work,
                                                                          reinterpret_cast<unsigned long long*>(H_.p));
       else
-        k4_hist_wide<4><<<wgrid, kWideThreads, 4 * kWideHistSeg * 4, s>>>(d.bins16.p, d.rows_stride, d.wide_meta.p, qgh_.p, qord_.p, idx0_.p, idx1_.p, &ctrl->hist_work,
+        k4_hist_wide<4><<<wgrid, kWideThreads, 4 * kWideHistSeg * 4, s>>>(d.bins16.p, d.rows_stride, d.wide_meta.p, gh_.p, ghord_.p, ctrl->exp_gh, idx0_.p, idx1_.p, &ctrl->hist_work,
                                                                          reinterpret_cast<unsigned long long*>(H_.p));
       timing.launches += 1;
     }
diff --git a/mmlspark_b200/csrc/engine.h b/mmlspark_b200/csrc/engine.h
--- a/mmlspark_b200/csrc/engine.h
+++ b/mmlspark_b200/csrc/engine.h
@@ -220,7 +220,7 @@
   SplitParams sp_{};
   DevBuf<double> score_;
   DevBuf<float> grad_, hess_;
-  DevBuf<int4> qgh_, qord_;
+  DevBuf<float2> gh_, ghord_;
   DevBuf<int> idx0_, idx1_;
   DevBuf<long long> H_;
   DevBuf<long long> pool_;
diff --git a/mmlspark_b200/csrc/hist_kernel.cuh b/mmlspark_b200/csrc/hist_kernel.cuh
--- a/mmlspark_b200/csrc/hist_kernel.cuh
+++ b/mmlspark_b200/csrc/hist_kernel.cuh
@@ -12,6 +12,14 @@
 #define B200GBM_K4_EXPERIMENT 0
 #endif
 constexpr int kPlaneWords = kBins * kTileFeat;
+constexpr int kGhPad = 2;
+
+__device__ __forceinline__ long long d_fixed(float x, double scale, unsigned& hi, unsigned& lo) {
+  const long long q = __double2ll_rn(static_cast<double>(x) * scale);
+  hi = static_cast<unsigned>(static_cast<int>(q >> kLoBits));
+  lo = static_cast<unsigned>(q & ((1LL << kLoBits) - 1));
+  return q;
+}
 
 struct HistWork {
   int begin;
@@ -21,14 +29,14 @@
 };
 
 __global__ void __launch_bounds__(256)
-k_gather_q(const HistWork* __restrict__ work, const int* __restrict__ idx0, const int* __restrict__ idx1, const int4* __restrict__ qgh,
-           int4* __restrict__ qord) {
+k_gather_gh(const HistWork* __restrict__ work, const int* __restrict__ idx0, const int* __restrict__ idx1, const float2* __restrict__ gh,
+            float2* __restrict__ ghord) {
   const HistWork w = *work;
   if (!w.use_idx) return;
   const int* __restrict__ idx = w.buf ? idx1 : idx0;
   for (int i = blockIdx.x * blockDim.x + threadIdx.x; i < w.count; i += gridDim.x * blockDim.x) {
     const int p = w.begin + i;
-    qord[p] = qgh[idx[p]];
+    ghord[p] = gh[idx[p]];
   }
 }
 
@@ -47,12 +55,16 @@
 constexpr int kWsProducerWarps = 2;
 constexpr int kWsThreads = (kWsConsumerWarps + kWsProducerWarps) * 32;
 constexpr int kWsStageRows = 512;
-constexpr int kWsStages = 3;
+constexpr int kWsStageGhSlots = kWsStageRows + 2;
+constexpr int kWsStages = 4;
 constexpr int kFlushSlabBins = 32;
 constexpr int kFlushRowBytes = kFlushSlabBins * 16;
 constexpr int kFlushStageBytes = kTileFeat * kFlushRowBytes;
-constexpr int kWsSmemBytes = 4 * kPlaneWords * 4 + kWsStages * (kWsStageRows * 32 + kWsStageRows * 16) + kFlushStageBytes + 64;
+constexpr int kWsBarrierBytes = 2 * kWsStages * 8;
+constexpr int kWsSmemBytes =
+    4 * kPlaneWords * 4 + kWsStages * kWsStageRows * 32 + kFlushStageBytes + kWsStages * kWsStageGhSlots * 8 + kWsBarrierBytes;
 static_assert(kWsSmemBytes <= 227 * 1024, "K4 shared memory exceeds the 227 KB per block of sm_90");
+static_assert((kWsStageGhSlots * 8) % 16 == 0, "a stage's (g,h) slots must keep the next stage 16-byte aligned for the bulk copies");
 static_assert(kFlushSlabBins * kTileFeat == 2 * kWsConsumerWarps * 32, "a flush slab is two (g,h) pairs per consumer thread");
 
 __device__ __forceinline__ unsigned smem_u32(const void* p) { return static_cast<unsigned>(__cvta_generic_to_shared(p)); }
@@ -99,15 +111,15 @@
 
 template <int NATOM>
 __global__ void __launch_bounds__(kWsThreads, 1)
-k4_hist_build_ws(const uint8_t* __restrict__ bins, size_t rows_stride, int num_tiles, const int4* __restrict__ qgh,
-                 const int4* __restrict__ qord, const int* __restrict__ idx0, const int* __restrict__ idx1,
+k4_hist_build_ws(const uint8_t* __restrict__ bins, size_t rows_stride, int num_tiles, const float2* __restrict__ gh,
+                 const float2* __restrict__ ghord, const int* __restrict__ exps, const int* __restrict__ idx0, const int* __restrict__ idx1,
                  const HistWork* __restrict__ work, unsigned long long* __restrict__ hist) {
   extern __shared__ __align__(128) unsigned char smem_raw[];
   unsigned* plane = reinterpret_cast<unsigned*>(smem_raw);
   unsigned char* stage_bins = smem_raw + 4 * kPlaneWords * 4;
-  int4* stage_q = reinterpret_cast<int4*>(stage_bins + kWsStages * kWsStageRows * 32);
-  unsigned char* flush_stage = reinterpret_cast<unsigned char*>(stage_q) + kWsStages * kWsStageRows * 16;
-  unsigned long long* full_bar = reinterpret_cast<unsigned long long*>(flush_stage + kFlushStageBytes);
+  unsigned char* flush_stage = stage_bins + kWsStages * kWsStageRows * 32;
+  float2* stage_gh = reinterpret_cast<float2*>(flush_stage + kFlushStageBytes);
+  unsigned long long* full_bar = reinterpret_cast<unsigned long long*>(stage_gh + kWsStages * kWsStageGhSlots);
   unsigned long long* empty_bar = full_bar + kWsStages;
 
   const HistWork w = *work;
@@ -115,6 +127,7 @@
   if (n <= 0) return;
   const int tid = threadIdx.x, lane = tid & 31, warp = tid >> 5;
   const int* __restrict__ idx = w.buf ? idx1 : idx0;
+  const int gh_off = w.begin & 1;
 
   long long cells_rows = static_cast<long long>(n) * num_tiles;
   int rpi = static_cast<int>((cells_rows + 4LL * gridDim.x - 1) / (4LL * gridDim.x));
@@ -139,6 +152,13 @@
     const int ptid = tid - kWsConsumerWarps * 32;
     constexpr int kPT = kWsProducerWarps * 32;
     constexpr int kPerLane = kWsStageRows / kPT;
+    int rr[2 * kPerLane];
+    auto load_idx = [&](int p0, int rows, int (&dst)[2 * kPerLane]) {
+      const int* ip = idx + w.begin + p0;
+#pragma unroll
+      for (int k = 0; k < 2 * kPerLane; ++k) { const int j = (ptid + k * kPT) >> 1; dst[k] = j < rows ? ip[j] : -1; }
+    };
+    if (w.use_idx) { const int row0 = (i0 % chunks) * rpi; load_idx(row0, min(kWsStageRows, n - row0), rr); }
     for (int item = i0; item < i1; ++item) {
       const int tile = item / chunks, chunk = item - tile * chunks;
       const int row0 = chunk * rpi;
@@ -147,35 +167,42 @@
       const uint8_t* tbins = bins + static_cast<size_t>(tile) * rows_stride * 32;
       for (int s = 0; s < nst; ++s, ++gs) {
         const int slot = gs % kWsStages;
-        mbar_wait(&empty_bar[slot], ((gs / kWsStages) & 1u) ^ 1u);
         const int p0 = row0 + s * kWsStageRows;
         const int rows = min(kWsStageRows, row0 + nrows - p0);
+        int rn[2 * kPerLane];
+        if (w.use_idx) {
+          int np0 = 0, nrw = 0;
+          if (s + 1 < nst) { np0 = p0 + kWsStageRows; nrw = min(kWsStageRows, row0 + nrows - np0); }
+          else if (item + 1 < i1) { np0 = ((item + 1) % chunks) * rpi; nrw = min(kWsStageRows, n - np0); }
+          load_idx(np0, nrw, rn);
+        }
+        mbar_wait(&empty_bar[slot], ((gs / kWsStages) & 1u) ^ 1u);
         unsigned char* db = stage_bins + slot * kWsStageRows * 32;
-        int4* dq = stage_q + slot * kWsStageRows;
+        float2* dgh = stage_gh + slot * kWsStageGhSlots;
+        const size_t gpos = static_cast<size_t>(w.begin + p0 - gh_off);
+        const unsigned gh_bytes = static_cast<unsigned>((gh_off + rows + 1) & ~1) * 8u;
         if (!w.use_idx) {
           if (ptid == 0) {
-            mbar_arrive_expect_tx(&full_bar[slot], static_cast<unsigned>(rows) * 48u);
+            mbar_arrive_expect_tx(&full_bar[slot], static_cast<unsigned>(rows) * 32u + gh_bytes);
             const size_t r = static_cast<size_t>(w.begin + p0);
             tma_bulk_g2s(db, tbins + r * 32, static_cast<unsigned>(rows) * 32u, &full_bar[slot]);
-            tma_bulk_g2s(dq, qgh + r, static_cast<unsigned>(rows) * 16u, &full_bar[slot]);
+            tma_bulk_g2s(dgh, gh + gpos, gh_bytes, &full_bar[slot]);
           } else {
             mbar_arrive(&full_bar[slot]);
           }
         } else {
-          const int* ip = idx + w.begin + p0;
           if (ptid == 0) {
-            mbar_expect_tx(&full_bar[slot], static_cast<unsigned>(rows) * 16u);
-            tma_bulk_g2s(dq, qord + static_cast<size_t>(w.begin + p0), static_cast<unsigned>(rows) * 16u, &full_bar[slot]);
+            mbar_expect_tx(&full_bar[slot], gh_bytes);
+            tma_bulk_g2s(dgh, ghord + gpos, gh_bytes, &full_bar[slot]);
           }
-          int rr[2 * kPerLane];
-#pragma unroll
-          for (int k = 0; k < 2 * kPerLane; ++k) { const int j = (ptid + k * kPT) >> 1; rr[k] = j < rows ? ip[j] : -1; }
 #pragma unroll
           for (int k = 0; k < 2 * kPerLane; ++k) {
             const int hh = ptid + k * kPT, j = hh >> 1, half = (hh & 1) * 16;
             if (rr[k] >= 0) cp_async16(db + j * 32 + half, tbins + static_cast<size_t>(rr[k]) * 32 + half, true);
           }
           cp_async_mbar_arrive_noinc(&full_bar[slot]);
+#pragma unroll
+          for (int k = 0; k < 2 * kPerLane; ++k) rr[k] = rn[k];
         }
       }
     }
@@ -185,6 +212,7 @@
     unsigned exp_sink = 0;
 #endif
     const int sub = lane >> 2, rot = lane & 3;
+    const double scale_g = ldexp(1.0, exps[0]), scale_h = ldexp(1.0, exps[1]);
     int acc_rows = 0;
     for (int item = i0; item < i1; ++item) {
       const int tile = item / chunks, chunk = item - tile * chunks;
@@ -196,12 +224,16 @@
         mbar_wait(&full_bar[slot], (gs / kWsStages) & 1u);
         const int rows = min(kWsStageRows, nrows - s * kWsStageRows);
         const unsigned* sw = reinterpret_cast<const unsigned*>(stage_bins + slot * kWsStageRows * 32);
-        const int4* sq = stage_q + slot * kWsStageRows;
+        const float2* sgh = stage_gh + slot * kWsStageGhSlots + gh_off;
         const int groups = (rows + 31) >> 5;
         for (int g = warp; g < groups; g += kWsConsumerWarps) {
           const int r = g * 32 + lane;
           if (r < rows) {
-            const int4 q = sq[r];
+            const float2 v = sgh[r];
+            uint4 q;
+            d_fixed(v.x, scale_g, q.x, q.y);
+            if (NATOM == 4) d_fixed(v.y, scale_h, q.z, q.w);
+            else { q.z = 1u; q.w = 0u; }
             const unsigned* rw = sw + r * 8;
 #pragma unroll
             for (int k = 0; k < 8; ++k) {
@@ -213,14 +245,14 @@
                 const unsigned b = (word >> (8 * kk)) & 0xFFu;
                 const unsigned a = b * 32u + static_cast<unsigned>(w8 * 4 + kk);
 #if B200GBM_K4_EXPERIMENT == 0 || B200GBM_K4_EXPERIMENT == 4
-                atomicAdd(&plane[a], static_cast<unsigned>(q.x));
-                atomicAdd(&plane[kPlaneWords + a], static_cast<unsigned>(q.y));
-                atomicAdd(&plane[2 * kPlaneWords + a], static_cast<unsigned>(q.z));
-                if (NATOM == 4) atomicAdd(&plane[3 * kPlaneWords + a], static_cast<unsigned>(q.w));
+                atomicAdd(&plane[a], q.x);
+                atomicAdd(&plane[kPlaneWords + a], q.y);
+                atomicAdd(&plane[2 * kPlaneWords + a], q.z);
+                if (NATOM == 4) atomicAdd(&plane[3 * kPlaneWords + a], q.w);
 #else
-                if (B200GBM_K4_EXPERIMENT >= 2) atomicAdd(&plane[a], static_cast<unsigned>(q.x));
-                if (B200GBM_K4_EXPERIMENT >= 3) atomicAdd(&plane[kPlaneWords + a], static_cast<unsigned>(q.y));
-                if (B200GBM_K4_EXPERIMENT == 1) exp_sink ^= a + static_cast<unsigned>(q.x ^ q.y ^ q.z ^ q.w);
+                if (B200GBM_K4_EXPERIMENT >= 2) atomicAdd(&plane[a], q.x);
+                if (B200GBM_K4_EXPERIMENT >= 3) atomicAdd(&plane[kPlaneWords + a], q.y);
+                if (B200GBM_K4_EXPERIMENT == 1) exp_sink ^= a + (q.x ^ q.y ^ q.z ^ q.w);
 #endif
               }
             }
@@ -301,12 +333,13 @@
   return cudaFuncSetAttribute(k4_hist_build_ws<3>, cudaFuncAttributeMaxDynamicSharedMemorySize, kWsSmemBytes);
 }
 
-inline void launch_k4(bool const_hessian, const uint8_t* bins, size_t rows_stride, int num_tiles, const int4* qgh, const int4* qord,
-                      const int* idx0, const int* idx1, const HistWork* work, unsigned long long* hist, int grid, cudaStream_t stream) {
+inline void launch_k4(bool const_hessian, const uint8_t* bins, size_t rows_stride, int num_tiles, const float2* gh, const float2* ghord,
+                      const int* exps, const int* idx0, const int* idx1, const HistWork* work, unsigned long long* hist, int grid,
+                      cudaStream_t stream) {
   if (const_hessian)
-    k4_hist_build_ws<3><<<grid, kWsThreads, kWsSmemBytes, stream>>>(bins, rows_stride, num_tiles, qgh, qord, idx0, idx1, work, hist);
+    k4_hist_build_ws<3><<<grid, kWsThreads, kWsSmemBytes, stream>>>(bins, rows_stride, num_tiles, gh, ghord, exps, idx0, idx1, work, hist);
   else
-    k4_hist_build_ws<4><<<grid, kWsThreads, kWsSmemBytes, stream>>>(bins, rows_stride, num_tiles, qgh, qord, idx0, idx1, work, hist);
-}
-
-}
+    k4_hist_build_ws<4><<<grid, kWsThreads, kWsSmemBytes, stream>>>(bins, rows_stride, num_tiles, gh, ghord, exps, idx0, idx1, work, hist);
+}
+
+}
diff --git a/mmlspark_b200/csrc/kernels.cuh b/mmlspark_b200/csrc/kernels.cuh
--- a/mmlspark_b200/csrc/kernels.cuh
+++ b/mmlspark_b200/csrc/kernels.cuh
@@ -76,7 +76,7 @@
   unsigned split_cat_bits[8];
   HistWork hist_work;
   unsigned absmax_bits[2];
-  int exp_g, exp_h;
+  int exp_gh[2];
   double inv_g, inv_h;
   long long root_q[4];
   long long trace_rows;
@@ -388,25 +388,24 @@
   int eg = (mg > 0.f && isfinite(mg)) ? 34 - ilogbf(mg) : 0;
   int eh = (mh > 0.f && isfinite(mh)) ? 34 - ilogbf(mh) : 0;
   eg = max(min(eg, 1000), -1000); eh = max(min(eh, 1000), -1000);
-  ctrl->exp_g = eg; ctrl->exp_h = eh;
+  ctrl->exp_gh[0] = eg; ctrl->exp_gh[1] = eh;
   ctrl->inv_g = ldexp(1.0, -eg);
   ctrl->inv_h = const_hessian ? hess_const : ldexp(1.0, -eh);
   ctrl->root_q[0] = 0; ctrl->root_q[1] = 0; ctrl->root_q[2] = 0; ctrl->root_q[3] = 0;
 }
 __global__ void __launch_bounds__(256)
-k_quantize(const float* __restrict__ g, const float* __restrict__ h, int n, int4* __restrict__ qgh, TreeCtrl* ctrl, int const_hessian,
-           const uint8_t* __restrict__ in_bag, int bag_count) {
-  const int eg = ctrl->exp_g, eh = ctrl->exp_h;
+k_pack_gh(const float* __restrict__ g, const float* __restrict__ h, int n, float2* __restrict__ gh, TreeCtrl* ctrl, int const_hessian,
+          const uint8_t* __restrict__ in_bag, int bag_count) {
+  const double scale_g = ldexp(1.0, ctrl->exp_gh[0]), scale_h = ldexp(1.0, ctrl->exp_gh[1]);
   long long sg = 0, sh = 0;
   for (int i = blockIdx.x * blockDim.x + threadIdx.x; i < n; i += gridDim.x * blockDim.x) {
-    long long qg = __double2ll_rn(ldexp(static_cast<double>(g[i]), eg));
-    int4 q;
-    q.x = static_cast<int>(qg >> kLoBits); q.y = static_cast<int>(qg & ((1LL << kLoBits) - 1));
-    long long qh;
-    if (const_hessian) { qh = 1; q.z = 1; q.w = 0; }
-    else { qh = __double2ll_rn(ldexp(static_cast<double>(h[i]), eh)); q.z = static_cast<int>(qh >> kLoBits); q.w = static_cast<int>(qh & ((1LL << kLoBits) - 1)); }
-    qgh[i] = q;
-    if (!in_bag || in_bag[i]) { sg += qg; sh += qh; }
+    const float gi = g[i], hi = const_hessian ? 1.f : h[i];
+    gh[i] = make_float2(gi, hi);
+    if (!in_bag || in_bag[i]) {
+      unsigned f0, f1;
+      sg += d_fixed(gi, scale_g, f0, f1);
+      sh += const_hessian ? 1LL : d_fixed(hi, scale_h, f0, f1);
+    }
   }
   for (int o = 16; o; o >>= 1) { sg += __shfl_xor_sync(0xffffffffu, sg, o); sh += __shfl_xor_sync(0xffffffffu, sh, o); }
   __shared__ long long s_g[8], s_h[8];
@@ -1138,7 +1137,7 @@
 __global__ void __launch_bounds__(256, 3)
 k_partition(TreeCtrl* ctrl, LeafState* leaves, TreeDev tree, uint8_t* flags, const FeatMeta* __restrict__ meta, SplitParams p, int last,
             const uint8_t* __restrict__ bins, size_t rows_stride, int* __restrict__ idx0, int* __restrict__ idx1, unsigned* __restrict__ bits,
-            int* __restrict__ chunk_left, const int4* __restrict__ qgh, int4* __restrict__ qord, long long* __restrict__ H, size_t h_elems,
+            int* __restrict__ chunk_left, const float2* __restrict__ gh, float2* __restrict__ ghord, long long* __restrict__ H, size_t h_elems,
             const uint16_t* __restrict__ bins16, int tickets_per_block, const uint8_t* __restrict__ cols, size_t cols_stride, int* __restrict__ super_tot) {
   __shared__ int s_pref[kPartLocalScan + 1];
   __shared__ unsigned short s_list[kCatListMax];
@@ -1288,7 +1287,7 @@
       __syncthreads();
       const int left_base = local_scan ? s_pref[c] : s_pref[c / kPartLocalScan] + __ldcg(chunk_left + c);
       const int right_base = c * kPartChunk - left_base;
-      int rr[8], pp[8]; bool qq[8]; int4 qv[8];
+      int rr[8], pp[8]; bool qq[8]; float2 qv[8];
 #pragma unroll
       for (int k = 0; k < 8; ++k) {
         const int w = k * 8 + warp;
@@ -1304,12 +1303,12 @@
         }
       }
 #pragma unroll
-      for (int k = 0; k < 8; ++k) if (qq[k]) qv[k] = qgh[rr[k]];
+      for (int k = 0; k < 8; ++k) if (qq[k]) qv[k] = gh[rr[k]];
 #pragma unroll
       for (int k = 0; k < 8; ++k) {
         if (rr[k] < 0) continue;
         dst[pp[k]] = rr[k];
-        if (qq[k]) qord[pp[k]] = qv[k];
+        if (qq[k]) ghord[pp[k]] = qv[k];
       }
       __syncthreads();
       }
@@ -1369,13 +1368,14 @@
 constexpr int kWideThreads = 1024;
 template <int NATOM>
 __global__ void __launch_bounds__(kWideThreads, 1)
-k4_hist_wide(const uint16_t* __restrict__ bins16, size_t rows_stride, const WideMeta* __restrict__ wm, const int4* __restrict__ qgh,
-             const int4* __restrict__ qord, const int* __restrict__ idx0, const int* __restrict__ idx1, const HistWork* __restrict__ work,
-             unsigned long long* __restrict__ hist) {
+k4_hist_wide(const uint16_t* __restrict__ bins16, size_t rows_stride, const WideMeta* __restrict__ wm, const float2* __restrict__ gh,
+             const float2* __restrict__ ghord, const int* __restrict__ exps, const int* __restrict__ idx0, const int* __restrict__ idx1,
+             const HistWork* __restrict__ work, unsigned long long* __restrict__ hist) {
   extern __shared__ __align__(16) unsigned wplane[];
   const HistWork w = *work;
   const int n = w.count;
   if (n <= 0) return;
+  const double scale_g = ldexp(1.0, exps[0]), scale_h = ldexp(1.0, exps[1]);
   const int active = min(static_cast<int>(gridDim.x), (n + 4095) / 4096);
   if (static_cast<int>(blockIdx.x) >= active) return;
   const WideMeta m = wm[blockIdx.y];
@@ -1391,14 +1391,14 @@
   for (int c0 = p0; c0 < p1; c0 += kFlushRows) {
     const int c1 = min(c0 + kFlushRows, p1);
     for (int p = c0 + threadIdx.x; p < c1; p += 4 * kWideThreads) {
-      int4 q[4]; unsigned b[4]; size_t r[4];
+      float2 v[4]; unsigned b[4]; size_t r[4];
 #pragma unroll
       for (int j = 0; j < 4; ++j) {
         const int pj = p + j * kWideThreads;
         r[j] = 0;
         if (pj < c1) {
-          if (w.use_idx) { r[j] = static_cast<size_t>(idx[w.begin + pj]); q[j] = qord[w.begin + pj]; }
-          else { r[j] = static_cast<size_t>(w.begin + pj); q[j] = qgh[r[j]]; }
+          if (w.use_idx) { r[j] = static_cast<size_t>(idx[w.begin + pj]); v[j] = ghord[w.begin + pj]; }
+          else { r[j] = static_cast<size_t>(w.begin + pj); v[j] = gh[r[j]]; }
         }
       }
 #pragma unroll
@@ -1406,10 +1406,13 @@
 #pragma unroll
       for (int j = 0; j < 4; ++j) {
         if (b[j] >= static_cast<unsigned>(nb)) continue;
-        atomicAdd(&pl0[b[j]], static_cast<unsigned>(q[j].x));
-        atomicAdd(&pl1[b[j]], static_cast<unsigned>(q[j].y));
-        atomicAdd(&pl2[b[j]], static_cast<unsigned>(q[j].z));
-        if (NATOM == 4) atomicAdd(&pl3[b[j]], static_cast<unsigned>(q[j].w));
+        unsigned ghi, glo, hhi = 1u, hlo = 0u;
+        d_fixed(v[j].x, scale_g, ghi, glo);
+        if (NATOM == 4) d_fixed(v[j].y, scale_h, hhi, hlo);
+        atomicAdd(&pl0[b[j]], ghi);
+        atomicAdd(&pl1[b[j]], glo);
+        atomicAdd(&pl2[b[j]], hhi);
+        if (NATOM == 4) atomicAdd(&pl3[b[j]], hlo);
       }
     }
     __syncthreads();
```

Result: faster. 5.747, median of 6 (+2.7%).
